# davnords/octic-vits

Measured on AMD Instinct MI355X. Metric: images/sec Hybrid Octic ViT-H/14 224² bf16 train step @1/2/4/8 MI355X, higher is better.
Workload: dtype bf16; 1 GPU; hybrid_deit_huge_patch14 (16 octic + 16 standard blocks, drop_path 0.5) DeiT-III train step: bf16-autocast fwd + bwd + LAMB + EMA, 224x224, batch 64/GPU (BASELINE configs[1]), data parallel over 1 GPU(s); global_batch=64, per_gpu_batch=64, accum_steps=1, parallelism=dp1, library_gemm_table=True, launch=hipGraph replay (whole step)

## Files before the change

include/octic_hip.h:

```cpp
#ifndef OCTIC_HIP_H
#define OCTIC_HIP_H

#include <stdint.h>

#ifdef __cplusplus
extern "C" {
#endif

#define OCTIC_ABI_VERSION 20

enum { OCTIC_F32 = 0, OCTIC_BF16 = 1, OCTIC_U8 = 2  };

enum {
  OCTIC_OK = 0,
  OCTIC_ESHAPE = -1,
  OCTIC_EALIGN = -2,
  OCTIC_EDTYPE = -3,
  OCTIC_ENULL = -4,
  OCTIC_EWORKSPACE = -5
};

typedef struct {
  void* ptr[5];
  int64_t ld[5];
// ... 129 lines not shown
int octic_attn_unpack_heads(void* const heads[3], const octic_view* y, int64_t B, int64_t T, int H, int c, int n_s,
                            int dtype, void* stream);

int octic_attn_fwd(const void* q, const void* k, const void* v, void* o, float* lse, int64_t B, int H, int T, int hd,
                   int64_t sB, int64_t sH, int64_t sT, int64_t oB, int64_t oH, int64_t oT, float scale, void* stream);

int octic_attn_bwd(const void* q, const void* k, const void* v, const void* o, const void* dout, const float* lse,
                   float* delta, void* dq, void* dk, void* dv, int64_t B, int H, int T, int hd, int64_t sB, int64_t sH,
                   int64_t sT, int64_t oB, int64_t oH, int64_t oT, int64_t gB, int64_t gH, int64_t gT, float scale,
                   int phase, void* stream);

int octic_attn_fwd_f32(const void* q, const void* k, const void* v, void* o, float* lse, int64_t B, int H, int T, int hd,
                       int64_t sB, int64_t sH, int64_t sT, int64_t oB, int64_t oH, int64_t oT, float scale, void* stream);
int octic_attn_bwd_f32(const void* q, const void* k, const void* v, const void* o, const void* dout, const float* lse,
                       float* delta, void* dq, void* dk, void* dv, int64_t B, int H, int T, int hd, int64_t sB, int64_t sH,
                       int64_t sT, int64_t oB, int64_t oH, int64_t oT, int64_t gB, int64_t gH, int64_t gT, float scale,
                       int phase, void* stream);

int octic_attn_fwd_packed(const void* qkv, void* o, float* lse, int64_t B, int H, int T, int c, int64_t ld_qkv,
                          int64_t ld_o, float scale, void* stream);
int octic_attn_bwd_packed(const void* qkv, const void* o, const void* dout, const float* lse, float* delta, void* dqkv,
                          int64_t B, int H, int T, int c, int64_t ld_qkv, int64_t ld_o, int64_t ld_g, float scale,
                          int phase, void* stream);

enum {
  OCTIC_ATTN_FWD_PERSIST = 0,
  OCTIC_ATTN_FWD_A80_ONESHOT = 1,
  OCTIC_ATTN_FWD_A80_ONLINE = 2,
  OCTIC_ATTN_FWD_RESIDENT = 3,
  OCTIC_ATTN_FWD_STREAM = 4,
  OCTIC_ATTN_FWD_F32 = 5
};
enum {
  OCTIC_ATTN_BWD_SINGLE = 0,
  OCTIC_ATTN_BWD_PAIR = 1,
  OCTIC_ATTN_BWD_STREAM = 2,
  OCTIC_ATTN_BWD_F32 = 3
};
int octic_attn_plan(int dtype, int T, int hd, int64_t ld_in, int64_t ld_out, int64_t ld_grad, int out[4]);
int octic_attn_skip_plan(int dtype, int T, int hd, int64_t ld_in, int64_t ld_out, int64_t ld_grad, int out[4]);

int octic_attn_fwd_skip(const void* q, const void* k, const void* v, void* o, float* lse, int64_t B, int H, int T, int hd,
                        int64_t sB, int64_t sH, int64_t sT, int64_t oB, int64_t oH, int64_t oT, float scale,
                        const float* sample_scale, void* stream);
int octic_attn_bwd_skip(const void* q, const void* k, const void* v, const void* o, const void* dout, const float* lse,
                        float* delta, void* dq, void* dk, void* dv, int64_t B, int H, int T, int hd, int64_t sB, int64_t sH,
                        int64_t sT, int64_t oB, int64_t oH, int64_t oT, int64_t gB, int64_t gH, int64_t gT, float scale,
                        int phase, const float* sample_scale, void* stream);
int octic_attn_fwd_packed_skip(const void* qkv, void* o, float* lse, int64_t B, int H, int T, int c, int64_t ld_qkv,
                               int64_t ld_o, float scale, const float* sample_scale, void* stream);
int octic_attn_bwd_packed_skip(const void* qkv, const void* o, const void* dout, const float* lse, float* delta, void* dqkv,
                               int64_t B, int H, int T, int c, int64_t ld_qkv, int64_t ld_o, int64_t ld_g, float scale,
                               int phase, const float* sample_scale, void* stream);

int octic_handoff_cat_fwd(const octic_view* x, void* dense, int64_t M, int c, int out_dtype, void* stream);
int octic_handoff_cat_bwd(const float* ddense, const octic_view* dx, int64_t M, int c, void* stream);
int octic_power_spectrum_fwd(const octic_view* x, void* dense, int64_t M, int c, int out_dtype, void* stream);
int octic_power_spectrum_bwd(const float* ddense, const octic_view* x, const octic_view* dx, int64_t M, int c,
                             void* stream);

int octic_im2col_patches(const float* img, void* patches, int64_t B, int Cin, int Himg, int Wimg, int p,
                         int Kpad, int dtype, void* stream);
int octic_lift_gemm(const void* patches, const void* w, const float* bias, const float* pos, float* out,
                    int64_t B, int64_t n_patches, int tok0, int Kpad, int D, int dtype, void* stream);
int64_t octic_lift_wgrad_workspace_bytes(int Kpad, int D, int splits);
int octic_lift_wgrad(const void* patches, const void* dout, float* dw, float* workspace, int splits, int64_t rows,
                     int Kpad, int D, int dtype, void* stream);

int64_t octic_lamb_workspace_floats(int ntensors, int nchunks);
int octic_lamb_step(void* const* p, void* const* g, void* const* m, void* const* v, void* const* ema, const float* wd,
                    const int* chunk_tensor, const int64_t* chunk_off, const int* chunk_len,
                    const int* tensor_chunk_begin, int ntensors, int nchunks, float* workspace, float lr, float beta1,
                    float beta2, float eps, float max_grad_norm, int step, float ema_decay, void* const* bf16_shadow,
                    void* stream);
int octic_adamw_step(void* const* p, void* const* g, void* const* m, void* const* v, void* const* ema, const float* wd,
                     const int* chunk_tensor, const int64_t* chunk_off, const int* chunk_len,
                     const int* tensor_chunk_begin, int ntensors, int nchunks, float* workspace, float lr, float beta1,
                     float beta2, float eps, float max_grad_norm, int step, float ema_decay, void* const* bf16_shadow,
                     void* stream);
int octic_lamb_step_hp(void* const* p, void* const* g, void* const* m, void* const* v, void* const* ema, const float* wd,
                       const int* chunk_tensor, const int64_t* chunk_off, const int* chunk_len,
                       const int* tensor_chunk_begin, int ntensors, int nchunks, float* workspace, const float* lr,
                       float beta1, float beta2, float eps, float max_grad_norm, int step, const float* ema_decay,
                       void* const* bf16_shadow, void* stream);
int octic_adamw_step_hp(void* const* p, void* const* g, void* const* m, void* const* v, void* const* ema, const float* wd,
                        const int* chunk_tensor, const int64_t* chunk_off, const int* chunk_len,
                        const int* tensor_chunk_begin, int ntensors, int nchunks, float* workspace, const float* lr,
                        float beta1, float beta2, float eps, float max_grad_norm, int step, const float* ema_decay,
                        void* const* bf16_shadow, void* stream);

int octic_dense_blocks(int64_t rows);
int octic_dense_resid_layernorm_fwd(const float* x, const void* yb, int yb_dtype, const float* gamma, const float* rs,
                                    int64_t rows_per_scale, float* xout, void* y, int y_dtype, const float* w,
                                    const float* b, float* stats, int64_t rows, int d, float eps, void* stream);
int octic_dense_layernorm_fwd(const float* x, void* y, int y_dtype, const float* w, const float* b, float* stats,
                              int64_t rows, int d, float eps, void* stream);
int octic_dense_layernorm_bwd(const void* gy, int g_dtype, const float* x, const float* w, const float* stats,
                              const float* dres, float* dx, float* partials, int64_t rows, int d, void* stream);
int octic_dense_finish(const float* partials, int nblocks, int d, float* out0, float* out1, const float* scale1,
                       void* stream);
typedef struct octic_finish_job {
  const float* partials;
  float* out0;
  float* out1;
  const float* scale1;
  int nblocks;
  int d;
} octic_finish_job;
int octic_dense_finish_batch(const octic_finish_job* jobs, int njobs, void* stream);
int octic_dense_layernorm_bwd_tail(const void* gy, const float* x, const float* w, const float* stats, const float* dres,
                                   float* dx, float* partials, const void* yb, const float* gamma, const float* rs,
                                   int64_t rows_per_scale, void* gyb, float* partials2, int64_t rows, int d, void* stream);
int octic_dense_gelu_blocks(void);
int octic_dense_gelu_bwd(const void* h, const void* g, void* dh, float* partials, int64_t rows, int d, void* stream);
int octic_dense_colsum(const void* g, int64_t rows, int d, int64_t ld, float* partials, void* stream);
int octic_scale_residual_fwd(const float* x, const void* y, int y_dtype, const float* gamma, const float* rs,
                             int64_t rows_per_scale, float* out, int64_t rows, int d, void* stream);
int octic_scale_residual_bwd(const float* gout, const void* y, int y_dtype, const float* gamma, const float* rs,
                             int64_t rows_per_scale, void* gy, float* partials, int64_t rows, int d, void* stream);

int octic_dense_layernorm_fwd_rows(const float* x, void* y, int y_dtype, const float* w, const float* b, float* stats,
                                   int64_t rows, int d, float eps, const int* rowmap, float* xcopy, void* stream);
int octic_dense_layernorm_bwd_rows(const void* gy, int g_dtype, const float* x, const float* w, const float* stats,
                                   const float* dres, float* dx, float* partials, int64_t rows, int d, const int* rowmap,
                                   void* stream);
int octic_scale_residual_fwd_rows(const float* x, const void* y, int y_dtype, const float* gamma, const float* rs,
                                  int64_t rows_per_scale, float* out, int64_t rows, int d, const int* rowmap, void* stream);
int octic_scale_residual_bwd_rows(const float* gout, const void* y, int y_dtype, const float* gamma, const float* rs,
                                  int64_t rows_per_scale, void* gy, float* partials, int64_t rows, int d, const int* rowmap,
                                  void* stream);

typedef struct octic_dense_prep_item {
  const void* src;
  void* wb;
  void* wt;
  int32_t N, K;
  int32_t block_begin, pad;
} octic_dense_prep_item;
int octic_dense_prep_batch_blocks(int N, int K);
int octic_dense_prep_batch(const octic_dense_prep_item* items_dev, int n_items, int total_blocks, int src_dtype, void* stream);

int64_t octic_dense_gemm_workspace_bytes(int M, int N, int K);
int octic_dense_gemm_colsum_rows(int M, int N, int K);
int octic_dense_gemm_tile(int M, int N, int K, int mode);
int octic_dense_gemm_nt(const void* A, const void* B, int M, int N, int K, int64_t lda, int64_t ldb, int mode, void* C,
                        void* C2, int64_t ldc, const float* bias, const float* gamma, const float* rs,
                        int64_t rows_per_sample, const float* X, float* OUT, const void* H, float* colsum,
                        void* workspace, void* stream);
int octic_dense_gemm_nt_tokens(const void* A, const void* B, int M, int N, int K, int64_t lda, int64_t ldb, int mode, void* C,
                               void* C2, int64_t ldc, const float* bias, const float* gamma, const float* rs,
                               int64_t rows_per_sample, const float* X, float* OUT, const void* H, float* colsum,
                               void* workspace, int tokens, void* stream);
int octic_dense_gemm_plan(int M, int N, int K, int mode, int tokens, int* out4);

int64_t octic_dense_wgrad_workspace_bytes(int M, int N, int K);
int octic_dense_wgrad_tile(int M, int N, int K);
int octic_dense_wgrad_plan(int M, int N0, int N1, int K, int64_t ld_max, int out[4]);
int octic_dense_wgrad_tn(const void* dY, const void* X, int M, int N, int K, int64_t ldy, int64_t ldx, float* dW,
                         void* workspace, void* stream);
int64_t octic_dense_wgrad_pair_workspace_bytes(int M, int N0, int N1, int K);
int octic_dense_wgrad_tn_pair(const void* dY0, const void* X0, int N0, int64_t ldy0, int64_t ldx0, float* dW0,
                              const void* dY1, const void* X1, int N1, int64_t ldy1, int64_t ldx1, float* dW1, int M, int K,
                              void* workspace, void* stream);
int octic_dense_wgrad_tn_skip(const void* dY, const void* X, int M, int N, int K, int64_t ldy, int64_t ldx, float* dW,
                              const float* sample_scale, int rows_per_sample, void* workspace, void* stream);
int octic_dense_wgrad_tn_pair_skip(const void* dY0, const void* X0, int N0, int64_t ldy0, int64_t ldx0, float* dW0,
                                   const void* dY1, const void* X1, int N1, int64_t ldy1, int64_t ldx1, float* dW1, int M, int K,
                                   const float* sample_scale, int rows_per_sample, void* workspace, void* stream);

int octic_softmax_center(const void* t, int t_dtype, int64_t ldt, const float* center, float inv_temp, float* out,
                         int64_t rows, int K, void* stream);
int octic_soft_ce_fwd(const void* s, int s_dtype, int64_t lds, const float* tprob, int64_t t_rows, float inv_temp,
                      float* loss, float* lse, float* tsum, int64_t rows, int K, void* stream);
int octic_soft_ce_bwd(const void* s, int s_dtype, int64_t lds, const float* tprob, int64_t t_rows, float inv_temp,
                      const float* g, const float* lse, const float* tsum, void* ds, int64_t ldd, int64_t rows, int K,
                      void* stream);

typedef struct {
  float* w;
  float* b;
  float* mw;
  float* mb;
  int32_t col0;
  int32_t K;
  int32_t lr_index;
  int32_t tile0;
} octic_probe_head;
int octic_probe_features(const void* const* cls, const int64_t* cls_ld, int n, const void* patch, int64_t patch_ld_b,
                         int64_t patch_ld_t, int dtype, int64_t B, int P, int D, float* F, int64_t ldf, void* stream);
int octic_probe_forward(const octic_probe_head* heads, int nheads, const float* F, int64_t ldf, int B, int C, float* logits,
                        void* stream);
int octic_probe_ce(const float* logits, const int64_t* labels, int nheads, int B, int C, float* dlogits, float* rowloss,
                   int* rowrank, float* loss_mean, float* loss_sum, int* topk, void* stream);
int octic_probe_sgd(const octic_probe_head* heads, int nheads, int total_ktiles, const float* F, int64_t ldf,
                    const float* dlogits, int B, int C, const float* lr, float momentum, void* stream);

int octic_seg_ldd(int C);
int octic_seg_slabs(int64_t N, int D, int C);
int64_t octic_seg_workspace_bytes(int64_t N, int D, int C);
int octic_seg_value_dlogits(const float* X, int64_t ldx, int64_t N, int D, const float* W, const float* b, int C,
                            const int32_t* y, float* dlogits, double* value, void* workspace, void* stream);
int octic_seg_predict(const float* X, int64_t ldx, int64_t N, int D, const float* W, const float* b, int C, int32_t* pred,
                      void* stream);
int octic_seg_wgrad(const float* X, int64_t ldx, int64_t N, int D, const float* dlogits, int C, const float* W, double scale,
                    double lambda, float* dW, float* db, void* workspace, void* stream);
int64_t octic_seg_colstats_workspace_bytes(int64_t N, int D);
int octic_seg_colstats(const float* X, int64_t ldx, int64_t N, int D, double* mean, double* var, void* workspace, void* stream);
int octic_seg_standardize(float* X, int64_t ldx, int64_t N, int D, const double* mean, const double* scale, void* stream);
int octic_seg_patch_mode(const void* labels, int esize, int64_t R, int L, int32_t* mode, void* stream);
int octic_seg_confusion(const void* labels, int esize, int64_t R, int L, const int32_t* pred, const uint8_t* ignore,
                        int64_t* counts, void* stream);

typedef struct {
  int32_t partner;
  float lam;
  int32_t cut;
  int32_t yl, yh;
  int32_t xl, xh;
  int32_t pad;
} octic_mix_row;
int octic_mix_images(const float* src, float* dst, const octic_mix_row* table, int B, int C, int H, int W, void* stream);
int octic_mix_targets(const int64_t* labels, const octic_mix_row* table, int B, int row0, int rows, int num_classes, float on,
                      float off, int binarize, float* targets, void* stream);
int octic_mix_bce(const void* logits, int dtype, int64_t ldl, const int64_t* labels, const octic_mix_row* table, int B, int row0,
                  int rows, int num_classes, float on, float off, int binarize, float* loss, const float* gscale,
                  void* dlogits, int64_t ldd, void* workspace, void* stream);

typedef struct {
  int32_t flip;
  int32_t op;
  int32_t blur_r, blur_ww, blur_fw;
  int32_t order[4];
  float brightness, contrast, saturation;
  int32_t pad[4];
} octic_aug_row;
int64_t octic_augment_workspace_bytes(int B, int H, int W);
int octic_augment_u8(const uint8_t* src, void* dst, int dtype_out, const octic_aug_row* table, float mean0, float mean1,
                     float mean2, float std0, float std1, float std2, int B, int H, int W, void* workspace, void* stream);

#ifdef __cplusplus
}
#endif
#endif
```

octic_vits_amd/_lib.py:

```python
import ctypes
import os
import re

HERE = os.path.dirname(os.path.abspath(__file__))
LIB_PATH = os.environ.get("OCTIC_LIB") or os.path.join(HERE, "liboctic_hip.so")
HEADER_PATH = os.path.join(HERE, "..", "include", "octic_hip.h")

F32, BF16, U8 = 0, 1, 2
ABI_VERSION = 20
(ROUTE_DENSE_TILE, ROUTE_DENSE_SPLIT, ROUTE_WGRAD_SLABS, ROUTE_WGRAD_TILE, ROUTE_LINEAR_RING, ROUTE_RING_EVEN,
 ROUTE_ATTN_LEGACY, ROUTE_ATTN_ONLINE, ROUTE_ATTN_BWD_PAIR, ROUTE_DENSE_IMAGE, ROUTE_DENSE_CLS2, ROUTE_ATTN_STREAM) = range(12)

(ATTN_FWD_PERSIST, ATTN_FWD_A80_ONESHOT, ATTN_FWD_A80_ONLINE, ATTN_FWD_RESIDENT, ATTN_FWD_STREAM, ATTN_FWD_F32) = range(6)
ATTN_BWD_SINGLE, ATTN_BWD_PAIR, ATTN_BWD_STREAM, ATTN_BWD_F32 = range(4)
LINEAR_WREG, LINEAR_RING, LINEAR_CLASSIC = range(3)
WGRAD_RING, WGRAD_TILED = range(2)

c_i64, c_int, c_float, c_void_p = ctypes.c_int64, ctypes.c_int, ctypes.c_float, ctypes.c_void_p
c_double = ctypes.c_double


class OcticView(ctypes.Structure):
    _fields_ = [("ptr", c_void_p * 5), ("ld", c_i64 * 5)]


PtrArray5 = c_void_p * 5
VP = ctypes.POINTER(OcticView)

_PROTOS = {
    "octic_abi_version": (c_int, []),
    "octic_strerror": (ctypes.c_char_p, [c_int]),
    "octic_route_override": (c_int, [c_int, c_int]),
    "octic_gelu_d8_fwd": (c_int, [VP, VP, c_i64, c_int, c_int, c_void_p]),
    "octic_gelu_d8_bwd": (c_int, [VP, VP, VP, c_i64, c_int, c_int, c_void_p]),
    "octic_gelu_d8_fwd_skip": (c_int, [VP, VP, c_i64, c_int, c_int, c_void_p, c_i64, c_void_p]),
    "octic_gelu_d8_bwd_skip": (c_int, [VP, VP, VP, c_i64, c_int, c_int, c_void_p, c_i64, c_void_p]),
    "octic_layernorm_d8_fwd": (c_int, [VP, VP, c_void_p, c_void_p, c_void_p, c_i64, c_int, c_float, c_int, c_void_p]),
    "octic_layernorm_d8_bwd_blocks": (c_int, [c_i64]),
    "octic_layernorm_d8_bwd": (c_int, [VP, VP, c_void_p, c_void_p, VP, VP, c_void_p, c_i64, c_int, c_int, c_void_p]),
    "octic_layernorm_d8_bwd_cast": (c_int, [VP, VP, c_void_p, c_void_p, VP, VP, c_void_p, c_i64, c_int, c_void_p, c_i64,
                                            c_void_p, c_void_p]),
    "octic_layernorm_d8_bwd_finish": (c_int, [c_void_p, c_int, c_int, c_void_p, c_void_p, c_void_p]),
    "octic_layernorm_d8_bwd_finish_batch": (c_int, [c_void_p, c_int, c_void_p]),
    "octic_sample_blocks": (c_int, [c_void_p, c_void_p, c_void_p, c_i64, c_i64, c_int, c_void_p]),
    "octic_linear_d8_fwd": (c_int, [VP, c_void_p, c_void_p, VP, VP, c_void_p, c_i64, c_void_p, c_i64, c_int, c_int,
                                    c_int, c_int, c_void_p]),
    "octic_linear_d8_fwd_skip": (c_int, [VP, c_void_p, c_void_p, VP, VP, c_void_p, c_i64, c_void_p, c_i64, c_int, c_int,
                                         c_int, c_int, c_void_p, c_i64, c_void_p]),
    "octic_linear_d8_fwd_dropped": (c_int, [VP, c_void_p, c_void_p, VP, VP, c_void_p, c_i64, c_void_p, c_i64, c_int, c_int,
                                            c_int, c_int, c_void_p, c_i64, c_void_p]),
    "octic_linear_d8_tile_n": (c_int, [c_i64, c_int, c_int]),
    "octic_linear_d8_plan": (c_int, [c_i64, c_int, c_int, c_int, c_int, c_int, ctypes.POINTER(c_int)]),
    "octic_linear_d8_ring_order": (c_int, [c_void_p, c_void_p, c_void_p, c_int, c_void_p, c_void_p]),
    "octic_linear_d8_ring_order_dropped": (c_int, [c_int, c_void_p, c_void_p, c_int, c_void_p, c_void_p, c_void_p, c_void_p,
                                                   c_void_p, c_void_p]),
    "octic_linear_d8_wgrad_tile": (c_int, [c_i64, c_int, c_int]),
    "octic_linear_d8_wgrad_workspace_bytes": (c_i64, [c_int, c_int, c_int]),
    "octic_linear_d8_wgrad_splits": (c_int, [c_i64, c_int, c_int]),
    "octic_linear_d8_wgrad": (c_int, [VP, VP, c_i64, c_int, c_int, c_int, c_void_p, c_int, c_void_p]),
    "octic_linear_d8_wgrad_finish": (c_int, [c_void_p, c_int, c_int, c_int, c_void_p, c_void_p, c_void_p, c_void_p,
                                             c_void_p, c_void_p, c_void_p, c_void_p]),
    "octic_linear_d8_wgrad_finish_batch": (c_int, [c_void_p, c_int, c_void_p]),
    "octic_linear_d8_wgrad_has_colsum": (c_int, [c_int, c_int, c_int]),
    "octic_linear_d8_wgrad_plan": (c_int, [c_i64, c_int, c_int, c_int, ctypes.POINTER(c_int)]),
    "octic_lamb_workspace_floats": (c_i64, [c_int, c_int]),
    "octic_lamb_step": (c_int, [c_void_p] * 10 + [c_int, c_int, c_void_p, c_float, c_float, c_float, c_float, c_float,
                                                  c_int, c_float, c_void_p, c_void_p]),
    "octic_adamw_step": (c_int, [c_void_p] * 10 + [c_int, c_int, c_void_p, c_float, c_float, c_float, c_float, c_float,
                                                   c_int, c_float, c_void_p, c_void_p]),
    "octic_lamb_step_hp": (c_int, [c_void_p] * 10 + [c_int, c_int, c_void_p, c_void_p, c_float, c_float, c_float, c_float,
                                                     c_int, c_void_p, c_void_p, c_void_p]),
    "octic_adamw_step_hp": (c_int, [c_void_p] * 10 + [c_int, c_int, c_void_p, c_void_p, c_float, c_float, c_float, c_float,
                                                      c_int, c_void_p, c_void_p, c_void_p]),
    "octic_dense_blocks": (c_int, [c_i64]),
    "octic_dense_layernorm_fwd": (c_int, [c_void_p, c_void_p, c_int, c_void_p, c_void_p, c_void_p, c_i64, c_int,
                                          c_float, c_void_p]),
    "octic_dense_resid_layernorm_fwd": (c_int, [c_void_p, c_void_p, c_int, c_void_p, c_void_p, c_i64, c_void_p, c_void_p, c_int,
                                                c_void_p, c_void_p, c_void_p, c_i64, c_int, c_float, c_void_p]),
    "octic_dense_layernorm_bwd": (c_int, [c_void_p, c_int, c_void_p, c_void_p, c_void_p, c_void_p, c_void_p, c_void_p,
                                          c_i64, c_int, c_void_p]),
    "octic_dense_layernorm_bwd_tail": (c_int, [c_void_p] * 10 + [c_i64, c_void_p, c_void_p, c_i64, c_int, c_void_p]),
    "octic_dense_finish": (c_int, [c_void_p, c_int, c_int, c_void_p, c_void_p, c_void_p, c_void_p]),
    "octic_dense_finish_batch": (c_int, [c_void_p, c_int, c_void_p]),
    "octic_dense_gelu_blocks": (c_int, []),
    "octic_dense_gelu_bwd": (c_int, [c_void_p, c_void_p, c_void_p, c_void_p, c_i64, c_int, c_void_p]),
    "octic_dense_layernorm_fwd_rows": (c_int, [c_void_p, c_void_p, c_int, c_void_p, c_void_p, c_void_p, c_i64, c_int, c_float,
                                               c_void_p, c_void_p, c_void_p]),
    "octic_dense_layernorm_bwd_rows": (c_int, [c_void_p, c_int, c_void_p, c_void_p, c_void_p, c_void_p, c_void_p, c_void_p, c_i64,
                                               c_int, c_void_p, c_void_p]),
    "octic_scale_residual_fwd_rows": (c_int, [c_void_p, c_void_p, c_int, c_void_p, c_void_p, c_i64, c_void_p, c_i64, c_int,
                                              c_void_p, c_void_p]),
    "octic_scale_residual_bwd_rows": (c_int, [c_void_p, c_void_p, c_int, c_void_p, c_void_p, c_i64, c_void_p, c_void_p, c_i64,
                                              c_int, c_void_p, c_void_p]),
    "octic_softmax_center": (c_int, [c_void_p, c_int, c_i64, c_void_p, c_float, c_void_p, c_i64, c_int, c_void_p]),
    "octic_soft_ce_fwd": (c_int, [c_void_p, c_int, c_i64, c_void_p, c_i64, c_float, c_void_p, c_void_p, c_void_p, c_i64, c_int,
                                  c_void_p]),
    "octic_soft_ce_bwd": (c_int, [c_void_p, c_int, c_i64, c_void_p, c_i64, c_float, c_void_p, c_void_p, c_void_p, c_void_p, c_i64,
                                  c_i64, c_int, c_void_p]),
    "octic_scale_residual_fwd": (c_int, [c_void_p, c_void_p, c_int, c_void_p, c_void_p, c_i64, c_void_p, c_i64, c_int,
                                         c_void_p]),
    "octic_scale_residual_bwd": (c_int, [c_void_p, c_void_p, c_int, c_void_p, c_void_p, c_i64, c_void_p, c_void_p,
                                         c_i64, c_int, c_void_p]),
    "octic_colsum_blocks": (c_int, [c_i64]),
    "octic_colsum_a1": (c_int, [VP, c_i64, c_int, c_int, c_void_p, c_void_p, c_void_p]),
    "octic_cast_rowscale": (c_int, [VP, VP, c_void_p, c_i64, c_i64, c_int, c_int, c_void_p]),
    "octic_linear_d8_prep": (c_int, [c_void_p, c_void_p, c_int, c_int, c_void_p, c_void_p, c_int, c_void_p]),
    "octic_linear_d8_prep_batch_blocks": (c_int, [c_int, c_int]),
    "octic_linear_d8_prep_batch": (c_int, [c_void_p, c_int, c_int, c_int, c_void_p]),
    "octic_attn_fwd": (c_int, [c_void_p, c_void_p, c_void_p, c_void_p, c_void_p, c_i64, c_int, c_int, c_int,
                               c_i64, c_i64, c_i64, c_i64, c_i64, c_i64, c_float, c_void_p]),
    "octic_attn_fwd_packed": (c_int, [c_void_p] * 3 + [c_i64, c_int, c_int, c_int, c_i64, c_i64, c_float, c_void_p]),
    "octic_attn_bwd_packed": (c_int, [c_void_p] * 6 + [c_i64, c_int, c_int, c_int, c_i64, c_i64, c_i64, c_float, c_int, c_void_p]),
    "octic_attn_bwd": (c_int, [c_void_p] * 10 + [c_i64, c_int, c_int, c_int] + [c_i64] * 9 + [c_float, c_int, c_void_p]),
    "octic_attn_fwd_skip": (c_int, [c_void_p] * 5 + [c_i64, c_int, c_int, c_int] + [c_i64] * 6 + [c_float, c_void_p, c_void_p]),
    "octic_attn_bwd_skip": (c_int, [c_void_p] * 10 + [c_i64, c_int, c_int, c_int] + [c_i64] * 9 + [c_float, c_int, c_void_p, c_void_p]),
    "octic_attn_fwd_packed_skip": (c_int, [c_void_p] * 3 + [c_i64, c_int, c_int, c_int, c_i64, c_i64, c_float, c_void_p, c_void_p]),
    "octic_attn_bwd_packed_skip": (c_int, [c_void_p] * 6 + [c_i64, c_int, c_int, c_int, c_i64, c_i64, c_i64, c_float, c_int, c_void_p, c_void_p]),
    "octic_attn_fwd_f32": (c_int, [c_void_p] * 5 + [c_i64, c_int, c_int, c_int] + [c_i64] * 6 + [c_float, c_void_p]),
    "octic_attn_bwd_f32": (c_int, [c_void_p] * 10 + [c_i64, c_int, c_int, c_int] + [c_i64] * 9 + [c_float, c_int, c_void_p]),
    "octic_attn_plan": (c_int, [c_int, c_int, c_int, c_i64, c_i64, c_i64, ctypes.POINTER(c_int)]),
    "octic_attn_skip_plan": (c_int, [c_int, c_int, c_int, c_i64, c_i64, c_i64, ctypes.POINTER(c_int)]),
    "octic_attn_pack_heads": (c_int, [VP, c_void_p, c_i64, c_i64, c_int, c_int, c_int, c_int, c_void_p]),
    "octic_attn_unpack_heads": (c_int, [c_void_p, VP, c_i64, c_i64, c_int, c_int, c_int, c_int, c_void_p]),
    "octic_handoff_cat_fwd": (c_int, [VP, c_void_p, c_i64, c_int, c_int, c_void_p]),
    "octic_handoff_cat_bwd": (c_int, [c_void_p, VP, c_i64, c_int, c_void_p]),
    "octic_power_spectrum_fwd": (c_int, [VP, c_void_p, c_i64, c_int, c_int, c_void_p]),
    "octic_power_spectrum_bwd": (c_int, [c_void_p, VP, VP, c_i64, c_int, c_void_p]),
    "octic_im2col_patches": (c_int, [c_void_p, c_void_p, c_i64, c_int, c_int, c_int, c_int, c_int, c_int, c_void_p]),
    "octic_lift_gemm": (c_int, [c_void_p, c_void_p, c_void_p, c_void_p, c_void_p, c_i64, c_i64, c_int, c_int, c_int,
                                c_int, c_void_p]),
    "octic_lift_wgrad_workspace_bytes": (c_i64, [c_int, c_int, c_int]),
    "octic_lift_wgrad": (c_int, [c_void_p, c_void_p, c_void_p, c_void_p, c_int, c_i64, c_int, c_int, c_int, c_void_p]),
    "octic_dense_prep_batch_blocks": (c_int, [c_int, c_int]),
    "octic_dense_prep_batch": (c_int, [c_void_p, c_int, c_int, c_int, c_void_p]),
    "octic_dense_gemm_workspace_bytes": (c_i64, [c_int, c_int, c_int]),
    "octic_dense_gemm_colsum_rows": (c_int, [c_int, c_int, c_int]),
    "octic_dense_gemm_tile": (c_int, [c_int, c_int, c_int, c_int]),
    "octic_dense_gemm_nt": (c_int, [c_void_p, c_void_p, c_int, c_int, c_int, c_i64, c_i64, c_int, c_void_p, c_void_p, c_i64,
                                    c_void_p, c_void_p, c_void_p, c_i64, c_void_p, c_void_p, c_void_p, c_void_p, c_void_p,
                                    c_void_p]),
    "octic_dense_gemm_nt_tokens": (c_int, [c_void_p, c_void_p, c_int, c_int, c_int, c_i64, c_i64, c_int, c_void_p, c_void_p,
                                           c_i64, c_void_p, c_void_p, c_void_p, c_i64, c_void_p, c_void_p, c_void_p, c_void_p,
                                           c_void_p, c_int, c_void_p]),
    "octic_dense_gemm_plan": (c_int, [c_int, c_int, c_int, c_int, c_int, ctypes.POINTER(c_int)]),
    "octic_dense_colsum": (c_int, [c_void_p, c_i64, c_int, c_i64, c_void_p, c_void_p]),
    "octic_dense_wgrad_workspace_bytes": (c_i64, [c_int, c_int, c_int]),
    "octic_dense_wgrad_tile": (c_int, [c_int, c_int, c_int]),
    "octic_dense_wgrad_plan": (c_int, [c_int, c_int, c_int, c_int, c_i64, ctypes.POINTER(c_int)]),
    "octic_dense_wgrad_tn": (c_int, [c_void_p, c_void_p, c_int, c_int, c_int, c_i64, c_i64, c_void_p, c_void_p, c_void_p]),
    "octic_dense_wgrad_pair_workspace_bytes": (c_i64, [c_int, c_int, c_int, c_int]),
    "octic_dense_wgrad_tn_pair": (c_int, [c_void_p, c_void_p, c_int, c_i64, c_i64, c_void_p, c_void_p, c_void_p, c_int, c_i64, c_i64,
                                          c_void_p, c_int, c_int, c_void_p, c_void_p]),
    "octic_dense_wgrad_tn_skip": (c_int, [c_void_p, c_void_p, c_int, c_int, c_int, c_i64, c_i64, c_void_p, c_void_p, c_int, c_void_p,
                                          c_void_p]),
    "octic_dense_wgrad_tn_pair_skip": (c_int, [c_void_p, c_void_p, c_int, c_i64, c_i64, c_void_p, c_void_p, c_void_p, c_int, c_i64,
                                               c_i64, c_void_p, c_int, c_int, c_void_p, c_int, c_void_p, c_void_p]),
    "octic_probe_features": (c_int, [c_void_p, c_void_p, c_int, c_void_p, c_i64, c_i64, c_int, c_i64, c_int, c_int, c_void_p,
                                     c_i64, c_void_p]),
    "octic_probe_forward": (c_int, [c_void_p, c_int, c_void_p, c_i64, c_int, c_int, c_void_p, c_void_p]),
    "octic_probe_ce": (c_int, [c_void_p, c_void_p, c_int, c_int, c_int, c_void_p, c_void_p, c_void_p, c_void_p, c_void_p,
                               c_void_p, c_void_p]),
    "octic_probe_sgd": (c_int, [c_void_p, c_int, c_int, c_void_p, c_i64, c_void_p, c_int, c_int, c_void_p, c_float, c_void_p]),
    "octic_seg_ldd": (c_int, [c_int]),
    "octic_seg_slabs": (c_int, [c_i64, c_int, c_int]),
    "octic_seg_workspace_bytes": (c_i64, [c_i64, c_int, c_int]),
    "octic_seg_value_dlogits": (c_int, [c_void_p, c_i64, c_i64, c_int, c_void_p, c_void_p, c_int, c_void_p, c_void_p, c_void_p,
                                        c_void_p, c_void_p]),
    "octic_seg_predict": (c_int, [c_void_p, c_i64, c_i64, c_int, c_void_p, c_void_p, c_int, c_void_p, c_void_p]),
    "octic_seg_wgrad": (c_int, [c_void_p, c_i64, c_i64, c_int, c_void_p, c_int, c_void_p, c_double, c_double, c_void_p, c_void_p,
                                c_void_p, c_void_p]),
    "octic_seg_colstats_workspace_bytes": (c_i64, [c_i64, c_int]),
    "octic_seg_colstats": (c_int, [c_void_p, c_i64, c_i64, c_int, c_void_p, c_void_p, c_void_p, c_void_p]),
    "octic_seg_standardize": (c_int, [c_void_p, c_i64, c_i64, c_int, c_void_p, c_void_p, c_void_p]),
    "octic_seg_patch_mode": (c_int, [c_void_p, c_int, c_i64, c_int, c_void_p, c_void_p]),
    "octic_seg_confusion": (c_int, [c_void_p, c_int, c_i64, c_int, c_void_p, c_void_p, c_void_p, c_void_p]),
    "octic_mix_images": (c_int, [c_void_p, c_void_p, c_void_p, c_int, c_int, c_int, c_int, c_void_p]),
    "octic_mix_targets": (c_int, [c_void_p, c_void_p, c_int, c_int, c_int, c_int, c_float, c_float, c_int, c_void_p, c_void_p]),
    "octic_mix_bce": (c_int, [c_void_p, c_int, c_i64, c_void_p, c_void_p, c_int, c_int, c_int, c_int, c_float, c_float, c_int,
                              c_void_p, c_void_p, c_void_p, c_i64, c_void_p, c_void_p]),
    "octic_augment_workspace_bytes": (c_i64, [c_int, c_int, c_int]),
    "octic_augment_u8": (c_int, [c_void_p, c_void_p, c_int, c_void_p] + [c_float] * 6 + [c_int, c_int, c_int, c_void_p, c_void_p]),
}


def header_symbols():
    with open(HEADER_PATH) as f:
        text = re.sub(r"/\*.*?\*/", "", f.read(), flags=re.S)
    return sorted(set(re.findall(r"\b(octic_[a-z0-9_]+)\s*\(", text)))


_LIB = None


def lib():
    global _LIB
    if _LIB is None:
        if not os.path.exists(LIB_PATH):
            raise RuntimeError(
                f"octic_vits_amd: HIP library {LIB_PATH} is missing. Build it with "
                "`python -m octic_vits_amd.build` (hipcc, --offload-arch=gfx950). There is no CPU fallback.")
        L = ctypes.CDLL(LIB_PATH)
        for name, (res, args) in _PROTOS.items():
            fn = getattr(L, name)
            fn.restype, fn.argtypes = res, args
        if L.octic_abi_version() != ABI_VERSION:
            raise RuntimeError("octic_vits_amd: ABI version mismatch between _lib.py and liboctic_hip.so")
        _LIB = L
    return _LIB


def route_override(knob: int, value: int) -> int:
    old = lib().octic_route_override(knob, value)
    if old < 0:
        raise ValueError(f"octic_route_override: unknown knob {knob}")
    _PLANS.clear()
    for drop in _ON_OVERRIDE:
        drop()
    return old


_ON_OVERRIDE = []


def on_route_override(drop):
    if drop not in _ON_OVERRIDE:
        _ON_OVERRIDE.append(drop)
    return drop


_PLANS = {}


def plan(query, *args):
    key = (query, args)
    answer = _PLANS.get(key, 0)
    if answer == 0:
        out = (c_int * 4)()
        code = getattr(lib(), query)(*args, out)
        if code not in (0, -1):
            check(code)
        _PLANS[key] = answer = tuple(out) if code == 0 else None
    return answer


def attn_plan(T, hd, dtype=BF16, ld_in=0, ld_out=0, ld_grad=0):
    answer = plan("octic_attn_plan", dtype, T, hd, ld_in, ld_out, ld_grad)
    if answer is None:
        check(-1)
    return answer


def check(code: int):
    if code != 0:
        raise RuntimeError(f"octic HIP call failed ({code}): {lib().octic_strerror(code).decode()}")
```

octic_vits_amd/csrc/dense_gemm.hip:

```cpp
#include <cmath>
#include <type_traits>
#include "octic_common.hpp"

namespace octic {

constexpr int DG_BM = 256, DG_BK = 64;
constexpr int DG_UNIT = 128 * 128;
constexpr int DG_SLOTS = 8;
constexpr int DG_D = 6;
static_assert(DG_D >= 4 && DG_D <= DG_SLOTS - 2, "prefetch distance");
template <int NT> struct DgGeom {
  static constexpr int NA = NT - 2;
  static constexpr int BN = 64 * NT;
  static constexpr int WCOLS = 16 * NT;
  static constexpr int U1 = NA * 8192;
  static constexpr int KT = 3 * DG_UNIT + U1;
  static constexpr int RING = 2 * KT;
  static constexpr int SRS = WCOLS * 2 + 16;
  static constexpr int EPI_PASSES = NT == 4 ? 1 : 2;
  static constexpr int EPI_ROWS = 128 / EPI_PASSES;
  static constexpr int EPI = 8 * EPI_ROWS * SRS;
  static constexpr int LDS = RING > EPI ? RING : EPI;
  static constexpr int INFLIGHT = 2 * (DG_D - 2) + (NA - 2);
  static_assert(DG_D == 6 || NT == 4, "unequal units: the steady vmcnt assumes the 4 youngest units are one of each kind");
  __host__ __device__ static constexpr int unit_off(int kind) { return kind == 0 ? 0 : kind == 1 ? DG_UNIT : kind == 2 ? DG_UNIT + U1 : 2 * DG_UNIT + U1; }
  __host__ __device__ static constexpr int unit_instr(int kind) { return kind == 1 ? NA : 2; }
};

struct DgArgs {
  const bf16* A;
  const bf16* B;
  int64_t lda, ldb;
  int M, N, K;
  bf16* C;
  bf16* C2;
  int64_t ldc;
  const float* bias;
  const float* gamma;
  const float* rs;
  int64_t rps;
  const float* X;
  float* OUT;
  const bf16* H;
  float* colsum;
  int m_stride, m_base;
  int tiles_m, tiles_n;
  int full_tiles;
  int split;
  int tail_pad;
  float* slabs;
  int* tickets;
};

enum DgMode { DG_PLAIN = 0, DG_GELU = 1, DG_RESID = 2, DG_DGELU = 3,
              DG_GELUF = 4,
              DG_DFACT = 5,
              DG_GELUO = 6 };

__device__ inline void dg_wait_vmcnt(int n) {
  switch (n) {
    case 2: asm volatile("s_waitcnt vmcnt(2)" ::: "memory"); break;
    case 4: asm volatile("s_waitcnt vmcnt(4)" ::: "memory"); break;
    case 6: asm volatile("s_waitcnt vmcnt(6)" ::: "memory"); break;
    case 8: asm volatile("s_waitcnt vmcnt(8)" ::: "memory"); break;
    case 10: asm volatile("s_waitcnt vmcnt(10)" ::: "memory"); break;
    case 12: asm volatile("s_waitcnt vmcnt(12)" ::: "memory"); break;
    case 14: asm volatile("s_waitcnt vmcnt(14)" ::: "memory"); break;
    case 16: asm volatile("s_waitcnt vmcnt(16)" ::: "memory"); break;
    case 3: asm volatile("s_waitcnt vmcnt(3)" ::: "memory"); break;
    case 5: asm volatile("s_waitcnt vmcnt(5)" ::: "memory"); break;
    case 7: asm volatile("s_waitcnt vmcnt(7)" ::: "memory"); break;
    case 9: asm volatile("s_waitcnt vmcnt(9)" ::: "memory"); break;
    default: asm volatile("s_waitcnt vmcnt(0)" ::: "memory"); break;
  }
}

#ifdef DG_TRACE
__device__ unsigned long long g_dg_trace[8 * 256];
extern "C" void* octic_dbg_dense_trace(void) {
  void* p = nullptr;
  (void)hipGetSymbolAddress(&p, HIP_SYMBOL(g_dg_trace));
  return p;
}
#define DGT()                                                                                        \
  do {                                                                                               \
    if (blockIdx.x == 0 && lane == 0 && dgt_i < 256) g_dg_trace[wid * 256 + dgt_i++] = __builtin_readcyclecounter(); \
    if (blockIdx.x == 0 && lane == 0 && dgt_i == 200) g_dg_trace[wid * 256 + 255] = __builtin_amdgcn_s_memrealtime(); \
  } while (0)
#else
#define DGT() do {} while (0)
#endif
#ifdef DG_TRACE2
__device__ unsigned long long g_dg_trace2[4096 * 8];
extern "C" void* octic_dbg_dense_trace2(void) {
  void* p = nullptr;
  (void)hipGetSymbolAddress(&p, HIP_SYMBOL(g_dg_trace2));
  return p;
}
#define DGT2(slot)                                                                                            \
  do {                                                                                                        \
    if (wid == 0 && lane == 0 && blockIdx.x < 4096) g_dg_trace2[blockIdx.x * 8 + (slot)] = __builtin_amdgcn_s_memrealtime(); \
  } while (0)
#else
#define DGT2(slot) do {} while (0)
#endif

__device__ inline float dg_erf(float x) {
  const float ax = fabsf(x);
  const float t = __builtin_amdgcn_rcpf(1.0f + 0.3275911f * ax);
  const float poly = t * (0.254829592f + t * (-0.284496736f + t * (1.421413741f + t * (-1.453152027f + t * 1.061405429f))));
  const float r = 1.0f - poly * __expf(-ax * ax);
  return copysignf(r, x);
}
__device__ inline float dg_gelu(float x) { return 0.5f * x * (1.0f + dg_erf(x * kSqrt1Over2)); }
__device__ inline float dg_gelu_grad(float x) {
  return 0.5f * (1.0f + dg_erf(x * kSqrt1Over2)) + x * kInvSqrt2Pi * __expf(-0.5f * x * x);
}
__device__ inline void dg_gelu_both(float x, float& g, float& d) {
  const float ax = fabsf(x) * kSqrt1Over2;
  const float t = __builtin_amdgcn_rcpf(1.0f + 0.3275911f * ax);
  const float poly = t * (0.254829592f + t * (-0.284496736f + t * (1.421413741f + t * (-1.453152027f + t * 1.061405429f))));
  const float e = __expf(-ax * ax);
  const float phi = 0.5f * (1.0f + copysignf(1.0f - poly * e, x));
  g = x * phi;
  d = phi + x * kInvSqrt2Pi * e;
}

template <int N>
__device__ inline void dg_wait_imm() {
  if constexpr (N == 8) asm volatile("s_waitcnt vmcnt(8)" ::: "memory");
  else if constexpr (N == 10) asm volatile("s_waitcnt vmcnt(10)" ::: "memory");
  else if constexpr (N == 12) asm volatile("s_waitcnt vmcnt(12)" ::: "memory");
  else if constexpr (N == 14) asm volatile("s_waitcnt vmcnt(14)" ::: "memory");
  else if constexpr (N == 16) asm volatile("s_waitcnt vmcnt(16)" ::: "memory");
  else if constexpr (N == 6) asm volatile("s_waitcnt vmcnt(6)" ::: "memory");
  else if constexpr (N == 9) asm volatile("s_waitcnt vmcnt(9)" ::: "memory");
  else asm volatile("s_waitcnt vmcnt(0)" ::: "memory");
}

template <int MODE, int NT>
__global__ __launch_bounds__(512, 1) void dense_nt_kernel(DgArgs a) {
  extern __shared__ __attribute__((aligned(16))) char lds[];
  using GE = DgGeom<NT>;
  constexpr int NA = GE::NA, DG_BN = GE::BN;
  static_assert(NT == 4 || MODE == DG_PLAIN, "the fused tails exist for the 256-wide tile only");

  const int lane = threadIdx.x & 63;
  const int wid = __builtin_amdgcn_readfirstlane(threadIdx.x >> 6);
  const int wr = wid >> 2, wc = wid & 3;
  const bool hi = wr != 0;
  const int fr = lane & 15, kg = lane >> 4;
#ifdef DG_TRACE
  int dgt_i = 0;
  if (blockIdx.x == 0 && lane == 0) g_dg_trace[wid * 256 + 254] = __builtin_amdgcn_s_memrealtime();
#endif
  DGT();
  DGT2(0);
#ifdef DG_TRACE2
  if (wid == 0 && lane == 0 && blockIdx.x < 4096) {
    unsigned xcc, hwid;
    asm volatile("s_getreg_b32 %0, hwreg(HW_REG_XCC_ID)" : "=s"(xcc));
    asm volatile("s_getreg_b32 %0, hwreg(HW_REG_HW_ID)" : "=s"(hwid));
    g_dg_trace2[blockIdx.x * 8 + 7] = ((unsigned long long)hwid << 32) | xcc;
  }
#endif

  const int bid = blockIdx.x;
  int tile, kt_begin, kt_end, part = 0, rem_idx = -1;
  const int nkt_all = a.K / DG_BK;
  if (bid >= a.tail_pad) {
    const int j = bid - a.tail_pad;
    const int nf = a.full_tiles;
    const int xcd = j & 7, q8 = nf >> 3, r8 = nf & 7;
    tile = (xcd < r8 ? xcd * (q8 + 1) : r8 * (q8 + 1) + (xcd - r8) * q8) + (j >> 3);
    kt_begin = 0;
    kt_end = nkt_all;
  } else {
    const int r = bid;
    if (r >= (a.tiles_m * a.tiles_n - a.full_tiles) * a.split) return;
    rem_idx = r / a.split;
    part = r - rem_idx * a.split;
    tile = a.full_tiles + rem_idx;
    kt_begin = (int)(((int64_t)nkt_all * part) / a.split);
    kt_end = (int)(((int64_t)nkt_all * (part + 1)) / a.split);
  }
  int tm, tn;
  {
    const int G = 8;
    const int per_group = G * a.tiles_n;
    const int gidx = tile / per_group;
    const int first_m = gidx * G;
    const int gsz = (a.tiles_m - first_m) < G ? (a.tiles_m - first_m) : G;
    const int in_g = tile - gidx * per_group;
    tm = first_m + in_g % gsz;
    tn = in_g / gsz;
  }
  const int m0 = tm * a.m_stride + a.m_base, n0 = tn * DG_BN;
  const int nkt = kt_end - kt_begin;
  const int nunits = 4 * nkt;

  const int drow = lane >> 3;
  const int dch = (lane & 7) ^ drow;
  const __amdgpu_buffer_rsrc_t rsA = __builtin_amdgcn_make_buffer_rsrc((void*)a.A, 0, (int)((int64_t)a.M * a.lda * 2), 0x27000);
  const __amdgpu_buffer_rsrc_t rsB = __builtin_amdgcn_make_buffer_rsrc((void*)a.B, 0, (int)((int64_t)a.N * a.ldb * 2), 0x27000);
  const int r0 = 16 * wid + drow;
  const int am0 = m0, an0 = n0;
  const unsigned voA = (unsigned)(((int64_t)(am0 + (r0 >> 6) * 128 + (r0 & 63)) * a.lda + dch * 8) * 2);
  const int rb1 = 8 * NA * wid + drow;
  const unsigned voB1 = (unsigned)(((int64_t)(an0 + (rb1 / (16 * NA)) * GE::WCOLS + (rb1 % (16 * NA))) * a.ldb + dch * 8) * 2);
  const unsigned voB2 = (unsigned)(((int64_t)(an0 + (r0 >> 5) * GE::WCOLS + 16 * NA + (r0 & 31)) * a.ldb + dch * 8) * 2);
  const int rowA8 = (int)(a.lda * 16), rowB8 = (int)(a.ldb * 16);
  const int halfA = (int)(a.lda * 128);
  const int kbase = kt_begin * (DG_BK * 2);

  int u_issue = 0;
  auto issue_unit = [&](auto kind_c) {
    constexpr int KIND = decltype(kind_c)::value;
    constexpr bool isA = KIND == 0 || KIND == 3;
    char* dst = lds + ((u_issue >> 2) & 1) * GE::KT + GE::unit_off(KIND) + wid * (GE::unit_instr(KIND) * 1024);
    const int so = kbase + (u_issue >> 2) * (DG_BK * 2) + (KIND == 3 ? halfA : 0);
    if constexpr (isA) {
      __builtin_amdgcn_raw_ptr_buffer_load_lds(rsA, (__attribute__((address_space(3))) void*)dst, 16, voA, so, 0, 0);
      __builtin_amdgcn_raw_ptr_buffer_load_lds(rsA, (__attribute__((address_space(3))) void*)(dst + 1024), 16, voA, so + rowA8, 0, 0);
    } else if constexpr (KIND == 1) {
      __builtin_amdgcn_raw_ptr_buffer_load_lds(rsB, (__attribute__((address_space(3))) void*)dst, 16, voB1, so, 0, 0);
      __builtin_amdgcn_raw_ptr_buffer_load_lds(rsB, (__attribute__((address_space(3))) void*)(dst + 1024), 16, voB1, so + rowB8, 0, 0);
      if constexpr (NA == 3)
        __builtin_amdgcn_raw_ptr_buffer_load_lds(rsB, (__attribute__((address_space(3))) void*)(dst + 2048), 16, voB1, so + 2 * rowB8, 0, 0);
    } else {
      __builtin_amdgcn_raw_ptr_buffer_load_lds(rsB, (__attribute__((address_space(3))) void*)dst, 16, voB2, so, 0, 0);
      __builtin_amdgcn_raw_ptr_buffer_load_lds(rsB, (__attribute__((address_space(3))) void*)(dst + 1024), 16, voB2, so + rowB8, 0, 0);
    }
    ++u_issue;
  };
  auto young_instr = [&](int n) {
    const int k1 = ((u_issue + 2) >> 2) - ((u_issue - n + 2) >> 2);
    return 2 * n + (NA - 2) * k1;
  };
#define DG_IC(v) std::integral_constant<int, v>()

  const int sw = lane & 7;
  const int rdo0 = fr * 128 + ((kg ^ sw) << 4);
  const int rdo1 = fr * 128 + (((4 + kg) ^ sw) << 4);
  const int a_row0 = wr * 64;

  bf16x8 Af[1][2][4];
  bf16x8 Bf0[2][NA], Bf1[2][2];
  f32x4 acc0[2][4][NA], acc1[2][4][2];
#pragma unroll
  for (int i = 0; i < 2; ++i)
#pragma unroll
    for (int p = 0; p < 4; ++p) {
#pragma unroll
      for (int q = 0; q < NA; ++q) acc0[i][p][q] = f32x4{0, 0, 0, 0};
#pragma unroll
      for (int q = 0; q < 2; ++q) acc1[i][p][q] = f32x4{0, 0, 0, 0};
    }
  int rt_hi = (a.M - m0 - wr * 128 + 15) >> 4;
  rt_hi = rt_hi < 0 ? 0 : (rt_hi > 8 ? 8 : rt_hi);
  const int live_mask = __builtin_amdgcn_readfirstlane((rt_hi > 0 ? 1 : 0) | (rt_hi > 4 ? 2 : 0));

  auto readA = [&](int mh, int unit) {
    const char* base = lds + ((unit >> 2) & 1) * GE::KT + GE::unit_off(mh ? 3 : 0) + a_row0 * 128;
#pragma unroll
    for (int mi = 0; mi < 4; ++mi) {
      Af[0][0][mi] = *(const bf16x8*)(base + mi * 2048 + rdo0);
      Af[0][1][mi] = *(const bf16x8*)(base + mi * 2048 + rdo1);
    }
  };
  auto readB = [&](int nh, int unit) {
    if (nh == 0) {
      const char* base = lds + ((unit >> 2) & 1) * GE::KT + GE::unit_off(1) + wc * (16 * NA) * 128;
#pragma unroll
      for (int ni = 0; ni < NA; ++ni) {
        Bf0[0][ni] = *(const bf16x8*)(base + ni * 2048 + rdo0);
        Bf0[1][ni] = *(const bf16x8*)(base + ni * 2048 + rdo1);
      }
    } else {
      const char* base = lds + ((unit >> 2) & 1) * GE::KT + GE::unit_off(2) + wc * 32 * 128;
#pragma unroll
      for (int ni = 0; ni < 2; ++ni) {
        Bf1[0][ni] = *(const bf16x8*)(base + ni * 2048 + rdo0);
        Bf1[1][ni] = *(const bf16x8*)(base + ni * 2048 + rdo1);
      }
    }
  };
  auto mma = [&](int mh, int nh, auto kind_c) {
    asm volatile("s_waitcnt lgkmcnt(0)" ::: "memory");
    __builtin_amdgcn_sched_barrier(0);
    if (live_mask & (mh ? 2 : 1)) {
#pragma unroll
    for (int ks = 0; ks < 2; ++ks) {
#pragma unroll
      for (int mi = 0; mi < 4; ++mi) {
        if (nh == 0) {
#pragma unroll
          for (int ni = 0; ni < NA; ++ni)
            acc0[mh][mi][ni] = __builtin_amdgcn_mfma_f32_16x16x32_bf16(Bf0[ks][ni], Af[0][ks][mi], acc0[mh][mi][ni], 0, 0, 0);
        } else {
#pragma unroll
          for (int ni = 0; ni < 2; ++ni)
            acc1[mh][mi][ni] = __builtin_amdgcn_mfma_f32_16x16x32_bf16(Bf1[ks][ni], Af[0][ks][mi], acc1[mh][mi][ni], 0, 0, 0);
        }
      }
    }
    }
    __builtin_amdgcn_sched_barrier(0);
  };

  int g = 0;
  auto wait_landed = [&]() {
    int need = g + 2;
    need = need < nunits - 1 ? need : nunits - 1;
    const int ok = (u_issue - 1) - need;
    if (ok == DG_D - 2) dg_wait_imm<GE::INFLIGHT>();
    else dg_wait_vmcnt(ok > 0 ? young_instr(ok) : 0);
  };

#define DG_PRO(i) if constexpr ((i) < DG_D) { if (u_issue < nunits) issue_unit(DG_IC((i) & 3)); }
  DG_PRO(0) DG_PRO(1) DG_PRO(2) DG_PRO(3) DG_PRO(4) DG_PRO(5) DG_PRO(6) DG_PRO(7) DG_PRO(8) DG_PRO(9)
#undef DG_PRO
  {
    const int ok = (u_issue - 1) - 1;
    dg_wait_vmcnt(ok > 0 ? young_instr(ok) : 0);
  }
  if (hi) __builtin_amdgcn_s_barrier();
  DGT2(1);

  auto ktile = [&](int t, auto steady_c) {
    constexpr bool STEADY = decltype(steady_c)::value != 0;
    const int u0 = 4 * t;
    auto dma = [&](auto kind_c) {
      if (STEADY || u_issue < nunits) issue_unit(kind_c);
    };
    auto landed = [&]() {
      if constexpr (STEADY) dg_wait_imm<GE::INFLIGHT>();
      else wait_landed();
    };
#define DG_RP(x) do { __builtin_amdgcn_s_setprio(x); } while (0)
#define DG_R(q, reads) do { DG_RP(2); dma(DG_IC(((q) + DG_D) & 3)); reads; DG_RP(0); } while (0)
    __builtin_amdgcn_s_barrier();
    DGT();
    DG_R(0, readA(0, u0); readB(0, u0 + 1));
    if (hi) landed();
    DGT();
    __builtin_amdgcn_s_barrier();
    DGT();
    mma(0, 0, DG_IC((0 + DG_D) & 3));
    DGT();
    if (!hi) landed();
// ... 397 lines not shown
inline DgPlan dense_plan_nt(int M, int N, int K, int cus, int nt, int force_split = 0, bool front_unsplit = false) {
  DgPlan p;
  const int bn = 64 * nt;
  const double wf = nt / 4.0;
  p.nt = nt;
  p.tiles_m = (M + DG_BM - 1) / DG_BM;
  p.tiles_n = (N + bn - 1) / bn;
  const int tiles = p.tiles_m * p.tiles_n;
  const int rounds = tiles / cus;
  const int nkt = K / DG_BK;
  p.full = rounds * cus;
  p.rem = tiles - p.full;
  p.split = 1;
  double f = 1.0;
  if (p.rem > 0) {
    int s = cus / p.rem;
    const int smax = nkt / 4 > 0 ? nkt / 4 : 1;
    s = s < 1 ? 1 : (s > smax ? smax : s);
    s = s > 8 ? 8 : s;
    if (p.rem * 10 >= cus * 8) s = 1;
    {
      int64_t rows = 0;
      for (int tile = p.full; tile < tiles; ++tile) {
        const int G = 8, per_group = G * p.tiles_n, gidx = tile / per_group, first_m = gidx * G;
        const int gsz = (p.tiles_m - first_m) < G ? (p.tiles_m - first_m) : G;
        const int tm = first_m + (tile - gidx * per_group) % gsz;
        const int left = M - tm * DG_BM;
        rows += left < DG_BM ? left : DG_BM;
      }
      f = (double)rows / ((double)p.rem * DG_BM);
    }
    if (s > 1 && (double)nkt / s + 17.0 * f * wf + 1.0 >= (double)nkt) s = 1;
    if (force_split > 0) s = force_split > smax ? smax : force_split;
    p.split = s;
    if (s == 1 && !(front_unsplit && f < 0.5 && rounds >= 1)) {
      p.full = tiles;
      p.rem = 0;
    }
  }
  p.tail_pad = (p.rem * p.split + 7) & ~7;
  p.grid = p.tail_pad + p.full;
  const double tile_cost = nkt * wf + 3.0;
  p.cost = (double)((p.full + cus - 1) / cus) * tile_cost;
  if (p.rem > 0) {
    const double kt = (f < 0.5 ? 0.5 : 1.0) * wf;
    p.cost += (double)nkt / p.split * kt + 17.0 * f * wf + 3.0;
  }
  return p;
}

constexpr int DG_TICKET_BYTES = 8192;

static inline int dense_force_nt() { const int v = route(OCTIC_ROUTE_DENSE_TILE); return (v == 4 || v == 5) ? v : 0; }
static inline int dense_force_split() { const int v = route(OCTIC_ROUTE_DENSE_SPLIT); return v > 0 ? v : 0; }

inline DgPlan dense_plan(int M, int N, int K, int cus, int mode) {
  const DgPlan p4 = dense_plan_nt(M, N, K, cus, 4, dense_force_split(), dense_force_split() == 1);
  if (mode != DG_PLAIN || (N % 320) != 0 || dense_force_nt() == 4) return p4;
  const DgPlan p5 = dense_plan_nt(M, N, K, cus, 5, dense_force_split(), dense_force_split() == 1);
  if (dense_force_nt() == 5) return p5;
  return p5.cost < p4.cost ? p5 : p4;
}

inline int dense_cls_waves(int K) {
  if (K % 320 == 0 && K / 320 <= 16) return K / 320;
  for (int w = 16; w > 1; --w)
    if (K % (32 * w) == 0) return w;
  return 1;
}

struct DgTokPlan { DgPlan p; bool image; int images; };
#ifndef DG_CLS2_US
#define DG_CLS2_US 15.0
#endif
inline bool dense_cls_two_launches(int mode, int N, int K) {
  const int v = route(OCTIC_ROUTE_DENSE_CLS2);
  const bool legal = mode == DG_PLAIN && (K % CLS_KSLICE) == 0 && (N % 64) == 0;
  return legal && v != 1 && (v == 2 || K >= 3840);
}
inline double dense_cls_cost(int B, int N, int K, int mode) {
  double us = 7.0 * sqrt((double)N / 1280.0) * pow((double)K / 1280.0, 0.8);
  if (dense_cls_two_launches(mode, N, K)) us = DG_CLS2_US;
  return us * (B <= 64 ? 1.0 : (double)B / 64.0) / 1.54;
}
inline DgTokPlan dense_plan_tokens(int M, int N, int K, int cus, int mode, int tokens) {
  DgTokPlan t;
  t.p = dense_plan(M, N, K, cus, mode);
  t.image = false;
  t.images = 0;
  const int force = route(OCTIC_ROUTE_DENSE_IMAGE);
  if (tokens != 257 || M % tokens != 0 || mode == DG_RESID || (K % 128) != 0 || (N % 16) != 0 || force == 2) return t;
  const int B = M / tokens;
  const DgPlan pi = dense_plan(B * DG_BM, N, K, cus, mode);
  const double margin = 1.0;
  const bool pays = mode != DG_DGELU && mode != DG_DFACT && pi.cost + dense_cls_cost(B, N, K, mode) + margin < t.p.cost;
  if (force == 1 || (force == 0 && pays) || (force == 3 && pays && mode == DG_PLAIN)) {
    t.p = pi;
    t.image = true;
    t.images = B;
  }
  return t;
}

}

using namespace octic;

extern "C" {

static int dense_cus() { return device_cus(); }

int64_t octic_dense_gemm_workspace_bytes(int M, int N, int K) {
  int64_t need = 256;
  if ((M % 257) == 0 && (K % CLS_KSLICE) == 0) {
    const int64_t rows_pad = ((int64_t)(M / 257) + 63) / 64 * 64;
    need = DG_TICKET_BYTES + (int64_t)(K / CLS_KSLICE) * rows_pad * N * 4 + 256;
  }
  const int Ms[2] = {M, (M % 257) == 0 ? M / 257 * DG_BM : 0};
  for (int i = 0; i < 2; ++i) {
    if (Ms[i] <= 0) continue;
    for (int nt = 4; nt <= 5; ++nt) {
      if (nt == 5 && (N % 320) != 0) continue;
      DgPlan p = dense_plan_nt(Ms[i], N, K, dense_cus(), nt);
      if (dense_force_split() > 1) p = dense_plan_nt(Ms[i], N, K, dense_cus(), nt, 8);
      if (p.split <= 1) continue;
      const int64_t b = (int64_t)p.rem * p.split * DG_BM * (64 * nt) * 4 + DG_TICKET_BYTES + 256;
      need = b > need ? b : need;
    }
  }
  return need;
}

int octic_dense_gemm_plan(int M, int N, int K, int mode, int tokens, int* out) {
  if (!out) return OCTIC_ENULL;
  if (M <= 0 || N <= 0 || K < 2 * DG_BK) { out[0] = 256; out[1] = 0; out[2] = 0; out[3] = 0; return OCTIC_OK; }
  const DgTokPlan t = dense_plan_tokens(M, N, K, dense_cus(), mode, tokens);
  out[0] = t.p.nt == 5 ? 320 : 256;
  out[1] = t.image ? 2 * t.images + (t.images + 15) / 16 : 2 * ((M + DG_BM - 1) / DG_BM);
  out[2] = t.image ? 1 : 0;
  out[3] = t.p.grid;
  return OCTIC_OK;
}

int octic_dense_gemm_tile(int M, int N, int K, int mode) {
  if (M <= 0 || N <= 0 || K < 2 * DG_BK) return 256;
  return dense_plan(M, N, K, dense_cus(), mode).nt == 5 ? 320 : 256;
}

int octic_dense_gemm_colsum_rows(int M, int N, int K) {
  (void)N; (void)K;
  return 2 * ((M + DG_BM - 1) / DG_BM);
}

int octic_dense_gemm_nt_tokens(const void* A, const void* B, int M, int N, int K, int64_t lda, int64_t ldb, int mode, void* C,
                               void* C2, int64_t ldc, const float* bias, const float* gamma, const float* rs, int64_t rps,
                               const float* X, float* OUT, const void* H, float* colsum, void* workspace, int tokens,
                               void* stream) {
  if (!A || !B || !C) return OCTIC_ENULL;
  if (M <= 0 || N <= 0 || K <= 0 || (K % DG_BK) || K < 2 * DG_BK || (N % 8) || (lda % 8) || (ldb % 8) || (ldc % 8)) return OCTIC_ESHAPE;
  if ((int64_t)M * lda * 2 >= (1ll << 31) || (int64_t)N * ldb * 2 >= (1ll << 31)) return OCTIC_ESHAPE;
  if ((((uintptr_t)A) | ((uintptr_t)B)) & 15) return OCTIC_EALIGN;
  if ((mode == DG_GELU || mode == DG_GELUF) && !C2) return OCTIC_ENULL;
  if (mode == DG_RESID && (!X || !OUT || (rs && rps <= 0))) return OCTIC_ENULL;
  if ((mode == DG_DGELU || mode == DG_DFACT) && !H) return OCTIC_ENULL;
  DgArgs a = {};
  a.A = (const bf16*)A; a.B = (const bf16*)B; a.lda = lda; a.ldb = ldb; a.M = M; a.N = N; a.K = K;
  a.C = (bf16*)C; a.C2 = (bf16*)C2; a.ldc = ldc; a.bias = bias; a.gamma = gamma; a.rs = rs; a.rps = rs ? rps : 1;
  a.X = X; a.OUT = OUT; a.H = (const bf16*)H; a.colsum = (mode == DG_DGELU || mode == DG_DFACT) ? colsum : nullptr;
  const DgTokPlan tp = dense_plan_tokens(M, N, K, dense_cus(), mode, tokens);
  const DgPlan p = tp.p;
  a.tiles_m = p.tiles_m; a.tiles_n = p.tiles_n; a.full_tiles = p.full; a.split = p.split; a.tail_pad = p.tail_pad;
  a.m_stride = tp.image ? tokens : DG_BM;
  a.m_base = tp.image ? 1 : 0;
  hipStream_t s = (hipStream_t)stream;
  if (p.split > 1) {
    if (!workspace) return OCTIC_ENULL;
    if (p.rem * 4 > DG_TICKET_BYTES) return OCTIC_ESHAPE;
    a.tickets = (int*)workspace;
    a.slabs = (float*)((char*)workspace + DG_TICKET_BYTES);
  }
  const int smem = DgGeom<4>::LDS, smem5 = DgGeom<5>::LDS;
  static DeviceOnce once;
  if (once.first()) {
    (void)hipFuncSetAttribute((const void*)dense_nt_kernel<DG_PLAIN, 4>, hipFuncAttributeMaxDynamicSharedMemorySize, smem);
    (void)hipFuncSetAttribute((const void*)dense_nt_kernel<DG_PLAIN, 5>, hipFuncAttributeMaxDynamicSharedMemorySize, smem5);
    (void)hipFuncSetAttribute((const void*)dense_nt_kernel<DG_GELU, 4>, hipFuncAttributeMaxDynamicSharedMemorySize, smem);
    (void)hipFuncSetAttribute((const void*)dense_nt_kernel<DG_RESID, 4>, hipFuncAttributeMaxDynamicSharedMemorySize, smem);
    (void)hipFuncSetAttribute((const void*)dense_nt_kernel<DG_DGELU, 4>, hipFuncAttributeMaxDynamicSharedMemorySize, smem);
    (void)hipFuncSetAttribute((const void*)dense_nt_kernel<DG_GELUF, 4>, hipFuncAttributeMaxDynamicSharedMemorySize, smem);
    (void)hipFuncSetAttribute((const void*)dense_nt_kernel<DG_DFACT, 4>, hipFuncAttributeMaxDynamicSharedMemorySize, smem);
    (void)hipFuncSetAttribute((const void*)dense_nt_kernel<DG_GELUO, 4>, hipFuncAttributeMaxDynamicSharedMemorySize, smem);
    (void)hipGetLastError();
  }
  switch (mode) {
    case DG_PLAIN:
      if (p.nt == 5) dense_nt_kernel<DG_PLAIN, 5><<<p.grid, 512, smem5, s>>>(a);
      else dense_nt_kernel<DG_PLAIN, 4><<<p.grid, 512, smem, s>>>(a);
      break;
    case DG_GELU: dense_nt_kernel<DG_GELU, 4><<<p.grid, 512, smem, s>>>(a); break;
    case DG_RESID: dense_nt_kernel<DG_RESID, 4><<<p.grid, 512, smem, s>>>(a); break;
    case DG_DGELU: dense_nt_kernel<DG_DGELU, 4><<<p.grid, 512, smem, s>>>(a); break;
    case DG_GELUF: dense_nt_kernel<DG_GELUF, 4><<<p.grid, 512, smem, s>>>(a); break;
    case DG_DFACT: dense_nt_kernel<DG_DFACT, 4><<<p.grid, 512, smem, s>>>(a); break;
    case DG_GELUO: dense_nt_kernel<DG_GELUO, 4><<<p.grid, 512, smem, s>>>(a); break;
    default: return OCTIC_ESHAPE;
  }
  if (tp.image && dense_cls_two_launches(mode, N, K) && workspace && p.split <= 1) {
    const int rows_pad = (tp.images + 63) / 64 * 64;
    float* part = (float*)((char*)workspace + DG_TICKET_BYTES);
    const int cus = dense_cus(), per64 = (N / 64) * (K / CLS_KSLICE) * (rows_pad / 64);
    const int nw = (per64 > cus && (N % 80) == 0 && (N / 80) * (K / CLS_KSLICE) * (rows_pad / 64) <= cus) ? 5 : 4;
    dense_cls_part_kernel<<<(N / (16 * nw)) * (K / CLS_KSLICE) * (rows_pad / 64), 64 * nw, 0, s>>>(a, tokens, tp.images, rows_pad, part);
    dense_cls_sum_kernel<<<(tp.images * (N / 4) + 255) / 256, 256, 0, s>>>(a, tokens, tp.images, rows_pad, part);
  } else if (tp.image) {
    const int grid = (N / 16) * ((tp.images + 15) / 16), cr0 = 2 * tp.images, thr = 64 * dense_cls_waves(K);
    switch (mode) {
      case DG_PLAIN: dense_cls_kernel<DG_PLAIN><<<grid, thr, 0, s>>>(a, tokens, tp.images, cr0); break;
      case DG_GELU: dense_cls_kernel<DG_GELU><<<grid, thr, 0, s>>>(a, tokens, tp.images, cr0); break;
      case DG_DGELU: dense_cls_kernel<DG_DGELU><<<grid, thr, 0, s>>>(a, tokens, tp.images, cr0); break;
      case DG_GELUF: dense_cls_kernel<DG_GELUF><<<grid, thr, 0, s>>>(a, tokens, tp.images, cr0); break;
      case DG_DFACT: dense_cls_kernel<DG_DFACT><<<grid, thr, 0, s>>>(a, tokens, tp.images, cr0); break;
      case DG_GELUO: dense_cls_kernel<DG_GELUO><<<grid, thr, 0, s>>>(a, tokens, tp.images, cr0); break;
      default: return OCTIC_ESHAPE;
    }
  }
  return launch_status();
}

int octic_dense_gemm_nt(const void* A, const void* B, int M, int N, int K, int64_t lda, int64_t ldb, int mode, void* C,
                        void* C2, int64_t ldc, const float* bias, const float* gamma, const float* rs, int64_t rps,
                        const float* X, float* OUT, const void* H, float* colsum, void* workspace, void* stream) {
  return octic_dense_gemm_nt_tokens(A, B, M, N, K, lda, ldb, mode, C, C2, ldc, bias, gamma, rs, rps, X, OUT, H, colsum,
                                    workspace, 0, stream);
}

}
```

octic_vits_amd/functional.py:

```python
import os

import torch

from . import ops


class Octic(tuple):

    def __new__(cls, packed: torch.Tensor, c: int):
        self = super().__new__(cls, ops.split_packed(packed, c))
        self.packed, self.c = packed, c
        return self


def as_packed(xs):
    if isinstance(xs, Octic):
        return xs.packed, xs.c
    if len(xs) != 5:
        raise AssertionError("Input should be a 5-tuple")
    c = xs[0].shape[-1]
    if xs[4].shape[-2:] != (2, 2 * c):
        raise ValueError(f"E irrep must be [..., 2, {2 * c}], got {tuple(xs[4].shape)}")
    return torch.cat([xs[0], xs[1], xs[2], xs[3], xs[4].flatten(-2)], dim=-1), c

# ... 244 lines not shown
        w32 = [_c(w.detach().float()) for w in w5] if has_cs else None
        f32_masters = all(w.dtype == torch.float32 for w in w5)
        dw, dcs, dbias = ops.linear_wgrad(xv, gv, M, cin, cout, dtype, x, w32=w32, cs5=cs32, bias=b32, dysum=dysum,
                                          want_bias=has_bias, may_defer=f32_masters, wparams=w5 if f32_masters else None)
        if not f32_masters:
            dw = [d.to(w.dtype) for d, w in zip(dw, w5)]
        dcs = dcs if has_cs else [None] * 5
        return (dx, *dw, dbias, dy if fused else None, None, *dcs, None, None, None, None, None, None, None, None)


class LinearD8NormFn(torch.autograd.Function):

    @staticmethod
    def forward(ctx, x, wA1, wA2, wB1, wB2, wE, bias, resid, rs, sA1, sA2, sB1, sB2, sE, cin, cout, rps, dtype, prep,
                a1, a2, b1, b2, ae, beta, eps, skip_dx=None):
        w5 = (wA1, wA2, wB1, wB2, wE)
        cs5 = None if sA1 is None else (sA1, sA2, sB1, sB2, sE)
        ops._require_cuda(x)
        x_in_dtype = x.dtype
        if x.dtype != dtype:
            x = ops.cast_rowscale(_c(x.float()), None, 1, dtype, cin)
        x = _c(x)
        wb, wt = prep.get(w5, cs5, dtype, cin, cout)
        M = x.numel() // (8 * cin)
        y = torch.empty(x.shape[:-1] + (8 * cout,), dtype=resid.dtype, device=x.device)
        b32 = None if bias is None else _c(bias.detach().float())
        cs32 = None if cs5 is None else [_c(s.detach().float()) for s in cs5]
        rs32 = None if rs is None else _c(rs.float())
        ops.linear_fwd(ops.pview(x, cin), wb, b32, ops.pview(y, cout), M, cin, cout, dtype, resid.dtype, x,
                       resid_v=ops.pview(_c(resid), cout), rs=rs32, rps=rps, cs5=cs32, dropped=ring_skip_scale(rs32, rps, M),
                       dropped_rps=rps)
        alpha = None if a1 is None else [_c(t.float()) for t in (a1, a2, b1, b2, ae)]
        yn, stats = ops.layernorm_fwd(y, alpha, None if beta is None else _c(beta.float()), eps, dtype, cout)
        ctx.save_for_backward(x, rs32, b32, y, stats, linear_skip_scale(skip_dx, rps, M), *w5, *(cs32 or []), *(alpha or []))
        ctx.meta = (cin, cout, rps, dtype, cs5 is not None, bias is not None, x_in_dtype, wt, alpha is not None,
                    beta is not None)
        ctx.set_materialize_grads(False)
        return y, yn

    @staticmethod
    def backward(ctx, dy, dyn):
        cin, cout, rps, dtype, has_cs, has_bias, x_in_dtype, wt, has_affine, has_beta = ctx.meta
        x, rs32, b32, y, stats, ss_dx, *rest = ctx.saved_tensors
        w5 = rest[:5]
        cs32 = rest[5:10] if has_cs else None
        alpha = rest[(10 if has_cs else 5):] if has_affine else None
        M = x.numel() // (8 * cin)
        dal, dbeta, g = [None] * 5, None, None
        if dyn is not None:
            dres = None if dy is None else _c(dy.float())
            gn = _c(dyn)
            if ops.layernorm_bwd_cast_ok(gn, y, cout) and dtype == torch.bfloat16:
                dy, dal_, dbeta, g = ops.layernorm_bwd_cast(gn, y, stats, alpha, dres, cout, rs32, rps,
                                                            want_param_grads=has_affine)
            else:
                dy, dal_, dbeta = ops.layernorm_bwd(gn, y, stats, alpha, dres, cout, want_param_grads=has_affine)
            dal = dal_ if dal_ is not None else dal
        dy = _c(dy)
        if g is None:
            g = ops.cast_rowscale(_c(dy.float()), rs32, rps, dtype, cout)
        gv, xv = ops.pview(g, cout), ops.pview(x, cin)
        dx = None
        if ctx.needs_input_grad[0]:
            dx = torch.empty(x.shape, dtype=dtype, device=x.device)
            ops.linear_fwd(gv, wt, None, ops.pview(dx, cin), M, cout, cin, dtype, dtype, x, sample_scale=ss_dx, skip_rps=rps)
            if dx.dtype != x_in_dtype:
                dx = dx.to(x_in_dtype)
        dysum = ops.colsum_a1(gv, M, cout, dtype, x) if (has_bias and not ops.wgrad_has_colsum(cin, cout, dtype)) else None
        w32 = [_c(w.detach().float()) for w in w5] if has_cs else None
        f32_masters = all(w.dtype == torch.float32 for w in w5)
        dw, dcs, dbias = ops.linear_wgrad(xv, gv, M, cin, cout, dtype, x, w32=w32, cs5=cs32, bias=b32, dysum=dysum,
                                          want_bias=has_bias, may_defer=f32_masters, wparams=w5 if f32_masters else None)
        if not f32_masters:
            dw = [d.to(w.dtype) for d, w in zip(dw, w5)]
        dcs = dcs if has_cs else [None] * 5
        return (dx, *dw, dbias, dy, None, *dcs, None, None, None, None, None, *dal, dbeta if has_beta else None, None, None)


class PackHeadsFn(torch.autograd.Function):

    @staticmethod
    def forward(ctx, qkv, H, c):
        B, T = qkv.shape[0], qkv.shape[1]
        ctx.meta = (B, T, H, c)
        q, k, v = ops.pack_heads(_c(qkv), B, T, H, c, 3)
        return q, k, v

    @staticmethod
    def backward(ctx, gq, gk, gv):
        B, T, H, c = ctx.meta
        return ops.unpack_heads([gq, gk, gv], B, T, H, c), None, None


class UnpackHeadsFn(torch.autograd.Function):
    @staticmethod
    def forward(ctx, o, c):
        B, H, T, _ = o.shape
        ctx.meta = (B, T, H, c)
        return ops.unpack_heads([o], B, T, H, c)

    @staticmethod
    def backward(ctx, g):
        B, T, H, c = ctx.meta
        return ops.pack_heads(_c(g), B, T, H, c, 1)[0], None


class AttnFn(torch.autograd.Function):

    @staticmethod
    def forward(ctx, q, k, v, scale):
        q, k, v = _c(q), _c(k), _c(v)
        o, lse = ops.attn_fwd(q, k, v, scale)
        ctx.save_for_backward(q, k, v, o, lse)
        ctx.scale = scale
        return o

    @staticmethod
    def backward(ctx, do):
        q, k, v, o, lse = ctx.saved_tensors
        do = _c(do)
        dq, dk, dv = torch.empty_like(q), torch.empty_like(k), torch.empty_like(v)
        ops.attn_bwd(q, k, v, o, do, lse, ctx.scale, dq, dk, dv)
        return dq, dk, dv, None


def _attn_skip_from_env():
    return os.environ.get("OCTIC_ATTN_SKIP", "1").strip() != "0"


ATTN_SKIP_DROPPED = _attn_skip_from_env()


def skip_scale(rs, B):
    if (not ATTN_SKIP_DROPPED or rs is None or not rs.is_cuda or rs.dtype != torch.float32 or rs.dim() != 1
            or rs.numel() != B or not rs.is_contiguous()):
        return None
    return rs.detach()


def _wgrad_skip_from_env():
    return os.environ.get("OCTIC_WGRAD_SKIP", "1").strip() != "0"


WGRAD_SKIP_DROPPED = _wgrad_skip_from_env()


def wgrad_skip_scale(rs, rps, M, rows_to=None):
    if (not WGRAD_SKIP_DROPPED or rs is None or rows_to is not None or torch.compiler.is_compiling() or not rs.is_cuda
            or rs.dtype != torch.float32 or rs.dim() != 1 or not rs.is_contiguous() or rps < 2 or rs.numel() * rps != M):
        return None
    return rs.detach()


def _linear_skip_from_env():
    return os.environ.get("OCTIC_LINEAR_SKIP", "1").strip() != "0"


LINEAR_SKIP_DROPPED = _linear_skip_from_env()


def linear_skip_scale(rs, rps, M, rows_to=None):
    if (not LINEAR_SKIP_DROPPED or rs is None or rows_to is not None or torch.compiler.is_compiling() or not rs.is_cuda
            or rs.dtype != torch.float32 or rs.dim() != 1 or not rs.is_contiguous() or rps < 2 or rs.numel() * rps != M):
        return None
    return rs.detach()


def _ring_skip_from_env():
    return os.environ.get("OCTIC_RING_SKIP", "1").strip() != "0"


RING_SKIP_DROPPED = _ring_skip_from_env()


def ring_skip_scale(rs, rps, M):
    return linear_skip_scale(rs, rps, M) if RING_SKIP_DROPPED else None


class AttnPackedFn(torch.autograd.Function):

    @staticmethod
    def forward(ctx, qkv, H, c, scale, sample_scale=None):
        qkv = _c(qkv)
        ss = skip_scale(sample_scale, qkv.shape[0])
        o, lse = ops.attn_fwd_packed(qkv, H, c, scale, sample_scale=ss)
        ctx.save_for_backward(qkv, o, lse, ss)
        ctx.meta = (H, c, scale)
        return o

    @staticmethod
    def backward(ctx, do):
        qkv, o, lse, ss = ctx.saved_tensors
        H, c, scale = ctx.meta
        return ops.attn_bwd_packed(qkv, o, _c(do), lse, H, c, scale, sample_scale=ss), None, None, None, None


class AttnFusedQKVFn(torch.autograd.Function):

    @staticmethod
    def forward(ctx, qkv, scale, sample_scale=None):
        qkv = _c(qkv)
        B, T, _, H, hd = qkv.shape
        ss = skip_scale(sample_scale, B) if qkv.dtype == torch.bfloat16 else None
        q, k, v = (qkv[:, :, i].permute(0, 2, 1, 3) for i in range(3))
        o = torch.empty((B, T, H, hd), dtype=qkv.dtype, device=qkv.device)
        ov = o.permute(0, 2, 1, 3)
        _, lse = ops.attn_fwd(q, k, v, scale, out=ov, sample_scale=ss)
        ctx.save_for_backward(qkv, o, lse, ss)
        ctx.scale = scale
        return o.view(B, T, H * hd)

    @staticmethod
    def backward(ctx, do):
        qkv, o, lse, ss = ctx.saved_tensors
        B, T, _, H, hd = qkv.shape
        do = _c(do).view(B, T, H, hd)
        dqkv = torch.empty_like(qkv)
        q, k, v = (qkv[:, :, i].permute(0, 2, 1, 3) for i in range(3))
        dq, dk, dv = (dqkv[:, :, i].permute(0, 2, 1, 3) for i in range(3))
        ops.attn_bwd(q, k, v, o.permute(0, 2, 1, 3), do.permute(0, 2, 1, 3), lse, ctx.scale, dq, dk, dv, sample_scale=ss)
        return dqkv, None, None


def attention_core(q, k, v, dropout_p=0.0):
    B, H, T, hd = q.shape
    if dropout_p == 0.0 and q.is_cuda and (ops.attn_supported(T, hd, q.dtype) or ops.attn_f32_supported(T, hd, q.dtype)):
        return AttnFn.apply(q, k, v, hd ** -0.5)
    o = torch.nn.functional.scaled_dot_product_attention(q, k, v, dropout_p=dropout_p)
    return o if o.dtype == q.dtype else o.to(q.dtype)


class DenseWeightCache:

    def __init__(self):
        self.key = None
        self.w = self.b = None
        self.wt = self.wt_key = None
        self.static = False
        self.static_wt = False

    def static_nt(self):
        if self.static and self.w is not None and self.w.dtype == torch.bfloat16:
            return self.w, (self.wt if self.static_wt else None)
        return None, None

    @staticmethod
    def _key(w, b, dtype):
        return (dtype, w.data_ptr(), w._version, None if b is None else (b.data_ptr(), b._version))

    def get(self, w, b, dtype):
        key = self._key(w, b, dtype)
        if key != self.key:
            with torch.no_grad():
                self.w = _c(w.detach().to(dtype))
                self.b = None if b is None else _c(b.detach().to(dtype))
            self.key = key
            self.wt, self.wt_key = None, None
            self.static = self.static_wt = False
        return self.w, self.b

    def adopt(self, w, b, w_copy, b_copy, dtype, wt_copy=None):
        self.w, self.b = w_copy, b_copy
        self.key = self._key(w, b, dtype)
        self.static = True
        self.static_wt = wt_copy is not None
        if wt_copy is not None:
            self.wt, self.wt_key = wt_copy, self.key

    def get_nt(self, w, b, need_wt=True):
        wb, _ = self.get(w, b, torch.bfloat16)
        if not need_wt:
            return wb, None
        if self.wt is None or self.wt_key != self.key:
            with torch.no_grad():
                self.wt = wb.t().contiguous()
            self.wt_key = self.key
        return wb, self.wt


class SoftCrossEntropyFn(torch.autograd.Function):

    @staticmethod
    def forward(ctx, s, tprob, temp):
        tprob = _c(tprob.detach().float())
        loss, lse, tsum = ops.soft_ce_fwd(s, tprob, 1.0 / temp)
        ctx.save_for_backward(s, tprob, lse, tsum)
        ctx.temp = temp
        return loss

    @staticmethod
    def backward(ctx, g):
        s, tprob, lse, tsum = ctx.saved_tensors
        return ops.soft_ce_bwd(s, tprob, 1.0 / ctx.temp, g, lse, tsum), None, None


def loss_rows_ok(t):
    return t.is_cuda and t.dtype in (torch.float32, torch.bfloat16) and t.shape[-1] % 8 == 0 and not torch.compiler.is_compiling()


class DenseLayerNormFn(torch.autograd.Function):

    @staticmethod
    def forward(ctx, x, w, b, eps, out_dtype):
        x = _c(x)
        w32 = None if w is None else _c(w.detach().float())
        b32 = None if b is None else _c(b.detach().float())
# ... 125 lines not shown
    def backward(ctx, gout):
        ab, wb, y, g32, rs32 = ctx.saved_tensors
        rps, has_b, has_gamma, a_dtype = ctx.meta
        gout = _c(gout.float())
        gy, dgamma, colsum = ops.scale_residual_bwd(gout, y, g32, rs32, rps, want_gamma=has_gamma, want_colsum=has_b)
        g2, a2 = gy.reshape(-1, wb.shape[0]), ab.reshape(-1, wb.shape[1])
        ga = _mm_lib(g2, wb).view(ab.shape).to(a_dtype) if ctx.needs_input_grad[1] else None
        gw = _wgrad_lib(g2, a2, ctx.wparam)
        return gout, ga, gw, colsum, dgamma, None, None, None, None


def invalidate_weight_caches(model):
    n = 0
    for m in model.modules():
        for attr in ("_prep", "_c1", "_c2"):
            c = getattr(m, attr, None)
            if isinstance(c, (WeightPrep, DenseWeightCache)):
                c.key = None
                if isinstance(c, DenseWeightCache):
                    c.wt, c.wt_key = None, None
                n += 1
    return n


def track_optimizer(model, optimizer):
    return optimizer.register_step_post_hook(lambda *_a, **_k: invalidate_weight_caches(model))


WGRAD_F32_OUT = False
DENSE_HIP = {"qkv", "dqkv", "proj", "dproj", "fc1", "dfc1", "fc2", "dfc2"}
DENSE_RESID_FUSED = False
NEXT_NORM_FUSED = True
OCTIC_NEXT_NORM = True
LN_TAIL_FUSED = True


def dense_hip_ok(x, w, which=None):
    rows = x.numel() // max(1, x.shape[-1])
    return (which is None or which in DENSE_HIP) and x.is_cuda and ops.dense_gemm_ok(rows, w.shape[0], w.shape[1])


def _f32(t):
    return None if t is None else _c(t.detach().float())


def _timed_lib(kind, fn, M, N, K):
    t = ops.KERNEL_TIMER.start()
    out = fn()
    if t is not None:
        ops.KERNEL_TIMER.stop(t, f"library_gemm<{kind} {N}x{K}>", 2 * (M * K + N * K + M * N), 2.0 * M * N * K)
    return out


WGRAD_SLABS = {(5120, 1280): 4, (1280, 5120): 4, (3840, 1280): 2, (1280, 1280): 2}


def wgrad_slabs(M, N, K):
    if WGRAD_SLABS is False:
        return 1
    S = WGRAD_SLABS.get((N, K))
    if S is None:
        tiles = -(-N // 256) * -(-K // 256)
        S = max(1, min(8, 256 // max(1, tiles)))
    while S > 1 and M % S:
        S -= 1
    return S


WGRAD_HIP = True


def _wgrad_lib(g2, x2, wparam=None, sample_scale=None, rps=0):
    M, N, K = g2.shape[0], g2.shape[1], x2.shape[1]
    if (WGRAD_HIP and g2.is_cuda and g2.dtype == torch.bfloat16 and x2.dtype == torch.bfloat16
            and g2.stride(1) == 1 and x2.stride(1) == 1
            and ops.dense_wgrad_ok(M, N, K, max(g2.stride(0), x2.stride(0)))):
        dest = ops.grad_dest(wparam, (N, K))
        dw = ops.dense_wgrad_tn(g2, x2, out=dest, sample_scale=sample_scale, rows_per_sample=rps if sample_scale is not None else 0)
        if dest is not None:
            ops.grad_written(wparam)
        return dw
    S = wgrad_slabs(M, N, K)
    if S > 1 and g2.is_contiguous() and x2.is_contiguous():
        with torch.autocast("cuda", enabled=False):
            return _timed_lib("wgrad", lambda: torch.bmm(g2.view(S, M // S, N).transpose(1, 2), x2.view(S, M // S, K))
                              .sum(0, dtype=torch.float32), M, N, K)
    with torch.autocast("cuda", enabled=False):
        if WGRAD_F32_OUT:
            return _timed_lib("wgrad", lambda: torch.mm(g2.t(), x2, out_dtype=torch.float32), g2.shape[0], g2.shape[1],
                              x2.shape[1])
        w = _timed_lib("wgrad", lambda: g2.t() @ x2, g2.shape[0], g2.shape[1], x2.shape[1])
        return w.float()


def _mm_lib(a2, b):
    with torch.autocast("cuda", enabled=False):
        return _timed_lib("dgrad", lambda: a2 @ b, a2.shape[0], b.shape[1], b.shape[0])


def _linear_lib(x2, wb, bias):
    with torch.autocast("cuda", enabled=False):
        return _timed_lib("fwd", lambda: torch.nn.functional.linear(x2, wb, bias), x2.shape[0], wb.shape[0], wb.shape[1])


WGRAD_PAIRED = True
GELU_FACTOR = True


class WgradPair:
    __slots__ = ("pending",)

    def __init__(self):
        self.pending = None

    def park(self, g2, x2, wparam=None, sample_scale=None, rps=0):
        shape = (g2.shape[1], x2.shape[1])
        dw = ops.grad_dest(wparam, shape)
        landed = wparam if dw is not None else None
        if dw is None:
            dw = torch.empty(shape, dtype=torch.float32, device=g2.device)
        self.pending = (g2, x2, dw.untyped_storage(), dw.data_ptr(), tuple(dw.shape), dw.storage_offset(), landed,
                        sample_scale, rps)
        ops.DEFERRED_FINISHES.add_pair(self)
        return dw

    def take(self):
        p, self.pending = self.pending, None
        if p is None:
            return None
        g2, x2, storage, ptr, shape, offset, landed, ss, rps = p
        dw = torch.empty(0, dtype=torch.float32, device=g2.device).set_(storage, offset, shape)
        assert dw.data_ptr() == ptr
        return g2, x2, dw, landed, ss, rps

    def flush(self):
        p = self.take()
        if p is not None:
            g2, x2, dw, landed, ss, rps = p
            dw.copy_(_wgrad_lib(g2, x2, sample_scale=ss, rps=rps))
            ops.grad_written(landed)


def _pair_ready(pair, g2, x2):
    return (pair is not None and WGRAD_PAIRED and WGRAD_HIP and ops.DEFERRED_FINISHES.enabled
            and ops.DEFERRED_FINISHES.allow_pairs and ops._in_backward()
            and g2.is_cuda and g2.dtype == torch.bfloat16 and x2.dtype == torch.bfloat16 and g2.stride(1) == 1
            and x2.stride(1) == 1)


def _tok(shape):
    return int(shape[-2]) if len(shape) >= 3 else 0


def _gemm_fwd(tag, x2, wb, b, cache, name, tokens):
    if tag in DENSE_HIP:
        return ops.dense_gemm_nt(x2, wb, 0, bias=_f32(b), name=f"dense_nt_kernel<{name}>", tokens=tokens)
    return _linear_lib(x2, wb, None if b is None else cache.b)


def _gemm_dgrad(g2, wt, wb, shape, dtype):
    gx = (ops.dense_gemm_nt(g2, wt, 0, name="dense_nt_kernel<dgrad>", tokens=_tok(shape)) if wt is not None
          else _mm_lib(g2, wb))
    return gx.view(shape).to(dtype)


def _resid_tail_fwd(ctx, x, tag, a2, wb, b, cache, tokens, g32, rs32, rps, nw, nb, neps, rows_to, stream):
    ctx.rows_to, ctx.x_shape = rows_to, x.shape
    ctx.tail = (neps is not None, rps, b is not None, nw is not None, nb is not None)
    x2 = x.view(-1, wb.shape[0])
    if neps is None and rows_to is None and tag in DENSE_HIP and DENSE_RESID_FUSED:
        br, out = ops.dense_gemm_nt(a2, wb, 2, bias=_f32(b), gamma=g32, rs=rs32, rps=rps, x=x2, name="dense_nt_kernel<resid>")
        return out.view(x.shape), (br, g32, rs32)
    br = _gemm_fwd(tag, a2, wb, b, cache, tag, tokens)
    if neps is not None:
        nw32, nb32 = _f32(nw), _f32(nb)
        out, yn, stats = ops.dense_resid_layernorm_fwd(x2, br, g32, rs32, rps, nw32, nb32, neps, torch.bfloat16)
        ctx.set_materialize_grads(False)
        return (out.view(x.shape), yn.view(x.shape)), (br, g32, rs32, out, stats, nw32)
    if rows_to is not None:
        ops.scale_residual_fwd_rows_(stream, rows_to.rowmap, x2, br, g32, rs32, rps)
        ctx.mark_dirty(stream)
        return stream, (br, g32, rs32, rows_to.rowmap)
    return ops.scale_residual_fwd(x2, br, g32, rs32, rps).view(x.shape), (br, g32, rs32)


def _resid_tail_bwd(ctx, tail, gout, gyn, want_norm):
    norm, rps, has_b, has_nw, has_nb = ctx.tail
    br, g32, rs32, *rest = tail
    has_gamma = g32 is not None
    dnw = dnb = gbr = None
    if norm:
        out, stats, nw32 = rest
        if gyn is not None:
            want = has_nw and want_norm
            dres = None if gout is None else _c(gout.float()).view(out.shape)
            g2 = _c(gyn).view(out.shape)
            if LN_TAIL_FUSED and ops.dense_ln_bwd_tail_ok(g2, br, out.shape[-1]):
                gout, dnw, dnb, gbr, dgamma, colsum = ops.dense_layernorm_bwd_tail(
                    g2, out, nw32, stats, dres, br, g32, rs32, rps, want_param_grads=want, want_gamma=has_gamma,
                    want_colsum=has_b)
            else:
                gout, dnw, dnb = ops.dense_layernorm_bwd(g2, out, nw32, stats, dres, want_param_grads=want)
            dnw, dnb = (dnw if has_nw else None), (dnb if has_nb else None)
    elif ctx.rows_to is not None:
        gout = _c(gout.float())
        ctx.rows_to.link.g = gout
        gbr, dgamma, colsum = ops.scale_residual_bwd(gout, br, g32, rs32, rps, want_gamma=has_gamma, want_colsum=has_b,
                                                     rowmap=rest[0])
    if gbr is None:
        gout = _c(gout.float())
        gbr, dgamma, colsum = ops.scale_residual_bwd(gout.view(br.shape), br, g32, rs32, rps, want_gamma=has_gamma,
                                                     want_colsum=has_b)
    gx = None if ctx.rows_to is not None else gout.view(ctx.x_shape)
    return gx, gbr, dgamma, colsum, dnw, dnb


class DenseLinearNTFn(torch.autograd.Function):

    @staticmethod
    def forward(ctx, x, w, b, cache, tag, pair=None, rs=None, rps=0):
        ctx.pair = pair
        ctx.wparam = w
        xb = _c(x if x.dtype == torch.bfloat16 else x.to(torch.bfloat16))
        wb, wt = cache.get_nt(w, b, ("d" + tag) in DENSE_HIP and ctx.needs_input_grad[0])
        x2 = xb.reshape(-1, wb.shape[1])
        y = _gemm_fwd(tag, x2, wb, b, cache, "plain", _tok(x.shape))
        ss = wgrad_skip_scale(rs, rps, x2.shape[0])
        ctx.rps = rps
        ctx.save_for_backward(x2, wb, wt, ss)
        ctx.meta = (b is not None, x.dtype, x.shape, tag)
        return y.view(*x.shape[:-1], wb.shape[0])

    @staticmethod
    def backward(ctx, gy):
        x2, wb, wt, ss = ctx.saved_tensors
        has_b, x_dtype, x_shape, tag = ctx.meta
        g2 = _c(gy).reshape(-1, wb.shape[0])
        gx = _gemm_dgrad(g2, wt, wb, x_shape, x_dtype) if ctx.needs_input_grad[0] else None
        gb = None
        if has_b:
            gb = (ops.dense_colsum(g2) if g2.is_cuda and g2.dtype == torch.bfloat16 and g2.shape[1] % 8 == 0
                  else g2.sum(0, dtype=torch.float32))
        pair = ctx.pair
        if pair is not None and pair.pending is not None:
            pg, px = pair.pending[0], pair.pending[1]
            if (_pair_ready(pair, g2, x2) and pg.shape[0] == g2.shape[0] and px.shape[1] == x2.shape[1]
                    and ops.dense_wgrad_pair_ok(g2.shape[0], g2.shape[1], pg.shape[1], x2.shape[1])):
                pg, px, pdw, landed, pss, prps = pair.take()
                dest = ops.grad_dest(ctx.wparam, (g2.shape[1], x2.shape[1]))
                both = ss if (ss is not None and pss is not None and prps == ctx.rps and pss.data_ptr() == ss.data_ptr()
                              and pss.numel() == ss.numel()) else None
                dw, _ = ops.dense_wgrad_tn_pair(g2, x2, pg, px, dw1=pdw, dw0=dest, sample_scale=both,
                                                rows_per_sample=ctx.rps if both is not None else 0)
                ops.grad_written(landed, ctx.wparam if dest is not None else None)
                return gx, dw, gb, None, None, None, None, None
            pair.flush()
        return gx, _wgrad_lib(g2, x2, ctx.wparam, ss, ctx.rps), gb, None, None, None, None, None


class DenseProjResidFn(torch.autograd.Function):

    @staticmethod
    def forward(ctx, x, a, w, b, gamma, rs, rps, cache, nw=None, nb=None, neps=None, pair=None, rows_to=None, stream=None):
        ctx.pair = pair
        ctx.wparam = w
        x = _c(x)
        ab = _c(a if a.dtype == torch.bfloat16 else a.to(torch.bfloat16))
        wb, wt = cache.get_nt(w, b, "dproj" in DENSE_HIP and ctx.needs_input_grad[1])
        a2 = ab.reshape(-1, wb.shape[1])
        outs, tail = _resid_tail_fwd(ctx, x, "proj", a2, wb, b, cache, _tok(a.shape), _f32(gamma), _f32(rs), rps,
                                     nw, nb, neps, rows_to, stream)
        ctx.save_for_backward(a2, wb, wt, *tail)
        ctx.meta = (a.dtype, a.shape)
        return outs

    @staticmethod
    def backward(ctx, gout, gyn=None):
        a2, wb, wt, *tail = ctx.saved_tensors
        a_dtype, a_shape = ctx.meta
        gx, gy, dgamma, colsum, dnw, dnb = _resid_tail_bwd(ctx, tail, gout, gyn,
                                                           ctx.needs_input_grad[8] or ctx.needs_input_grad[9])
        ga = _gemm_dgrad(gy, wt, wb, a_shape, a_dtype) if ctx.needs_input_grad[1] else None
        rps = ctx.tail[1]
        ss = wgrad_skip_scale(tail[2], rps, gy.shape[0], ctx.rows_to)
        if _pair_ready(ctx.pair, gy, a2) and ops.dense_wgrad_ok(gy.shape[0], gy.shape[1], a2.shape[1]):
            dw = ctx.pair.park(gy, a2, ctx.wparam, ss, rps)
        else:
            dw = _wgrad_lib(gy, a2, ctx.wparam, ss, rps)
        return gx, ga, dw, colsum, dgamma, None, None, None, dnw, dnb, None, None, None, None


class DenseMlpFn(torch.autograd.Function):

    @staticmethod
    def forward(ctx, y, x, w1, b1, w2, b2, gamma, rs, rps, c1, c2, nw=None, nb=None, neps=None, rows_to=None, stream=None):
        ctx.wparams = (w1, w2)
        x = _c(x)
        yb = _c(y if y.dtype == torch.bfloat16 else y.to(torch.bfloat16))
        need_t = any(ctx.needs_input_grad[:2])
        w1b, w1t = c1.get_nt(w1, b1, "dfc1" in DENSE_HIP and need_t)
        w2b, w2t = c2.get_nt(w2, b2, "dfc2" in DENSE_HIP and need_t)
        y2 = yb.reshape(-1, w1b.shape[1])
        g32, rs32 = _f32(gamma), _f32(rs)
        factor = GELU_FACTOR and "fc1" in DENSE_HIP and w2t is not None
        ctx.factor = factor
        if "fc1" in DENSE_HIP and not any(ctx.needs_input_grad):
            a = ops.dense_gemm_nt(y2, w1b, 6, bias=_f32(b1), name="dense_nt_kernel<gelu-only>", tokens=_tok(y.shape))
            h = a
        elif "fc1" in DENSE_HIP:
            h, a = ops.dense_gemm_nt(y2, w1b, 4 if factor else 1, bias=_f32(b1), name="dense_nt_kernel<gelu>",
                                     tokens=_tok(y.shape))
        else:
            h = _linear_lib(y2, w1b, None if b1 is None else c1.b)
            a = torch.nn.functional.gelu(h)
        outs, tail = _resid_tail_fwd(ctx, x, "fc2", a, w2b, b2, c2, _tok(y.shape), g32, rs32, rps,
                                     nw, nb, neps, rows_to, stream)
        ctx.save_for_backward(y2, h, a, w1b, w1t, w2b, w2t, *tail)
        ctx.meta = (b1 is not None, y.dtype, y.shape)
        return outs

    @staticmethod
    def backward(ctx, gout, gyn=None):
        y2, h, a, w1b, w1t, w2b, w2t, *tail = ctx.saved_tensors
        has_b1, y_dtype, y_shape = ctx.meta
        gx, gbr, dgamma, db2, dnw, dnb = _resid_tail_bwd(ctx, tail, gout, gyn,
                                                         ctx.needs_input_grad[11] or ctx.needs_input_grad[12])
        if w2t is not None:
            md = 5 if ctx.factor else 3
            if has_b1:
                dh, db1 = ops.dense_gemm_nt(gbr, w2t, md, h=h, name="dense_nt_kernel<dgelu>", want_colsum=True,
                                            tokens=_tok(y_shape))
            else:
                dh, db1 = ops.dense_gemm_nt(gbr, w2t, md, h=h, name="dense_nt_kernel<dgelu>", tokens=_tok(y_shape)), None
        else:
            dh, db1 = ops.dense_gelu_bwd(h, _mm_lib(gbr, w2b), want_colsum=has_b1)
        rps = ctx.tail[1]
        ss = wgrad_skip_scale(tail[2], rps, gbr.shape[0], ctx.rows_to)
        gw2 = _wgrad_lib(gbr, a, ctx.wparams[1], ss, rps)
        gw1 = _wgrad_lib(dh, y2, ctx.wparams[0], ss, rps)
        gy = _gemm_dgrad(dh, w1t, w1b, y_shape, y_dtype) if ctx.needs_input_grad[0] else None
        return gy, gx, gw1, db1, gw2, db2, dgamma, None, None, None, None, dnw, dnb, None, None, None


class HandoffCatFn(torch.autograd.Function):
    @staticmethod
    def forward(ctx, x, c, out_dtype):
        ctx.c, ctx.in_dtype = c, x.dtype
        return ops.handoff_cat_fwd(_c(x.float()), c, out_dtype)

    @staticmethod
    def backward(ctx, g):
        return ops.handoff_cat_bwd(g, ctx.c).to(ctx.in_dtype), None, None


class PowerSpectrumFn(torch.autograd.Function):
    @staticmethod
    def forward(ctx, x, c, out_dtype):
        x = _c(x.float())
        ctx.save_for_backward(x)
        ctx.c = c
        return ops.power_spectrum_fwd(x, c, out_dtype)

    @staticmethod
    def backward(ctx, g):
        (x,) = ctx.saved_tensors
        return ops.power_spectrum_bwd(g, x, ctx.c), None, None


class LiftFn(torch.autograd.Function):

    @staticmethod
    def forward(ctx, img, wfull, bias_full, pos, cls_row, p, dtype):
        B, Cin, Hh, Ww = img.shape
        D, K = wfull.shape
        Kpad = (K + 7) // 8 * 8
        n_p = (Hh // p) * (Ww // p)
        tok0 = 0 if cls_row is None else 1
        patches = ops.im2col(img, p, Kpad, dtype)
        wpad = torch.zeros((D, Kpad), dtype=dtype, device=img.device)
        wpad[:, :K] = wfull.detach()
        out = torch.empty((B, tok0 + n_p, D), dtype=torch.float32, device=img.device)
        ops.lift_gemm(patches, wpad, None if bias_full is None else _c(bias_full.detach().float()),
                      None if pos is None else _c(pos.detach().float()), out, B, n_p, tok0, Kpad, D)
        if tok0:
            out[:, 0] = cls_row.detach().float()
        ctx.save_for_backward(patches)
        ctx.meta = (B, n_p, tok0, K, Kpad, D, dtype, bias_full is not None, pos is not None)
        return out

    @staticmethod
    def backward(ctx, dout):
        (patches,) = ctx.saved_tensors
        B, n_p, tok0, K, Kpad, D, dtype, has_bias, has_pos = ctx.meta
        dtok = dout[:, tok0:]
        dcompact = _c(dtok.to(dtype)).reshape(B * n_p, D)
        dw = ops.lift_wgrad(patches, dcompact, Kpad, D)[:, :K]
        dpos = dtok.sum(0) if (has_pos or has_bias) else None
        dbias = dpos.sum(0) if has_bias else None
        dcls = dout[:, 0].sum(0) if tok0 else None
        return None, dw, dbias, dpos if has_pos else None, dcls, None, None
```

octic_vits_amd/ops.py:

```python
import ctypes
import operator

import torch

from . import _lib
from ._lib import BF16, F32, OcticView, PtrArray5, check, lib

_DT = {torch.float32: F32, torch.bfloat16: BF16}
_DTN = {torch.float32: "f32", torch.bfloat16: "bf16"}


class KernelTimer:

    def __init__(self):
        self.on = False
        self.records = []
        self.overhead_us = 0.0

    def enable(self):
        self.on, self.records = True, []
        pairs = []
        for _ in range(64):
            e0, e1 = torch.cuda.Event(enable_timing=True), torch.cuda.Event(enable_timing=True)
            e0.record()
# ... 905 lines not shown
        dw = torch.empty(d, dtype=torch.float32, device=x.device)
        db = torch.empty(d, dtype=torch.float32, device=x.device)
        _finish(p1, nblk, d, dw, db, None, _stream(x))
    if want2:
        dgamma = torch.empty(d, dtype=torch.float32, device=x.device) if want_gamma else None
        colsum = torch.empty(d, dtype=torch.float32, device=x.device) if want_colsum else None
        _finish(p2, nblk, d, dgamma, colsum, gamma, _stream(x))
    return dx, dw, db, gyb, dgamma, colsum


def _rows2d(t):
    K = t.shape[-1]
    t2 = t.reshape(-1, K)
    if t2.stride(1) != 1 or (t2.shape[0] > 1 and t2.stride(0) % 8):
        t2 = t2.contiguous()
    return t2, t2.shape[0], K, (t2.stride(0) if t2.shape[0] > 1 else K)


def softmax_center(t, center, inv_temp):
    _require_cuda(t)
    t2, rows, K, ld = _rows2d(t)
    out = torch.empty(t.shape, dtype=torch.float32, device=t.device)
    c = None if center is None else center.reshape(-1).float().contiguous()
    tk = KERNEL_TIMER.start()
    check(lib().octic_softmax_center(_p(t2), dt_code(t2.dtype), ld, _p(c), float(inv_temp), _p(out), rows, K, _stream(t)))
    KERNEL_TIMER.stop(tk, f"softmax_center_kernel<{_DTN[t2.dtype]}>", rows * K * (2 * t2.element_size() + 4))
    return out


def soft_ce_fwd(s, tprob, inv_temp):
    _require_cuda(s)
    s2, rows, K, ld = _rows2d(s)
    if tprob.dtype != torch.float32 or not tprob.is_contiguous() or tprob.shape[-1] != K:
        raise ValueError("soft_ce_fwd: tprob must be a contiguous f32 [Nt, K] tensor")
    nt = tprob.numel() // K
    loss, lse, tsum = (torch.empty(rows, dtype=torch.float32, device=s.device) for _ in range(3))
    tk = KERNEL_TIMER.start()
    check(lib().octic_soft_ce_fwd(_p(s2), dt_code(s2.dtype), ld, _p(tprob), nt, float(inv_temp), _p(loss), _p(lse), _p(tsum),
                                  rows, K, _stream(s)))
    KERNEL_TIMER.stop(tk, f"soft_ce_fwd_kernel<{_DTN[s2.dtype]}>", rows * K * (s2.element_size() + 4))
    return loss, lse, tsum


def soft_ce_bwd(s, tprob, inv_temp, g, lse, tsum):
    s2, rows, K, ld = _rows2d(s)
    nt = tprob.numel() // K
    ds = torch.empty((rows, K), dtype=s2.dtype, device=s.device)
    g = g.reshape(-1).float().contiguous()
    tk = KERNEL_TIMER.start()
    check(lib().octic_soft_ce_bwd(_p(s2), dt_code(s2.dtype), ld, _p(tprob), nt, float(inv_temp), _p(g), _p(lse), _p(tsum),
                                  _p(ds), K, rows, K, _stream(s)))
    KERNEL_TIMER.stop(tk, f"soft_ce_bwd_kernel<{_DTN[s2.dtype]}>", rows * K * (2 * s2.element_size() + 4))
    return ds.view(s.shape)


def scale_residual_fwd(x, y, gamma, rs, rps):
    _require_cuda(x)
    d = x.shape[-1]
    rows = x.numel() // d
    out = torch.empty_like(x)
    t = KERNEL_TIMER.start()
    check(lib().octic_scale_residual_fwd(_p(x), _p(y), dt_code(y.dtype), _p(gamma), _p(rs), int(rps), _p(out), rows, d,
                                         _stream(x)))
    KERNEL_TIMER.stop(t, f"scale_residual_fwd_kernel<{_DTN[y.dtype]}>", rows * d * (8 + y.element_size()))
    return out


def scale_residual_fwd_rows_(stream, rowmap, x, y, gamma, rs, rps):
    _require_cuda(x)
    d = x.shape[-1]
    rows = rowmap.numel()
    _check_rowmap(rowmap, rows)
    t = KERNEL_TIMER.start()
    check(lib().octic_scale_residual_fwd_rows(_p(x), _p(y), dt_code(y.dtype), _p(gamma), _p(rs), int(rps), _p(stream), rows, d,
                                              _p(rowmap), _stream(x)))
    KERNEL_TIMER.stop(t, f"scale_residual_fwd_kernel<{_DTN[y.dtype]},rows>", rows * d * (8 + y.element_size()))
    return stream


def scale_residual_bwd(gout, y, gamma, rs, rps, want_gamma=True, want_colsum=True, rowmap=None):
    d = gout.shape[-1]
    rows = gout.numel() // d if rowmap is None else rowmap.numel()
    if rowmap is not None:
        _check_rowmap(rowmap, rows)
    gy = torch.empty(gout.shape if rowmap is None else y.shape, dtype=y.dtype, device=gout.device)
    nblk = lib().octic_dense_blocks(rows)
    want = want_gamma or want_colsum
    partials = torch.empty((nblk, 2, d), dtype=torch.float32, device=gout.device) if want else None
    t = KERNEL_TIMER.start()
    check(lib().octic_scale_residual_bwd_rows(_p(gout), _p(y), dt_code(y.dtype), _p(gamma), _p(rs), int(rps), _p(gy),
                                              _p(partials), rows, d, _p(rowmap), _stream(gout)))
    KERNEL_TIMER.stop(t, f"scale_residual_bwd_kernel<{_DTN[y.dtype]}>", rows * d * (4 + 2 * y.element_size()))
    if not want:
        return gy, None, None
    dgamma = torch.empty(d, dtype=torch.float32, device=gout.device) if want_gamma else None
    colsum = torch.empty(d, dtype=torch.float32, device=gout.device) if want_colsum else None
    _finish(partials, nblk, d, dgamma, colsum, gamma, _stream(gout))
    return gy, dgamma, colsum


def dense_gelu_bwd(h, g, want_colsum=True):
    _require_cuda(h)
    d = h.shape[-1]
    rows = h.numel() // d
    dh = torch.empty_like(h)
    nblk = lib().octic_dense_gelu_blocks()
    partials = torch.empty((nblk, d), dtype=torch.float32, device=h.device) if want_colsum else None
    t = KERNEL_TIMER.start()
    check(lib().octic_dense_gelu_bwd(_p(h), _p(g), _p(dh), _p(partials), rows, d, _stream(h)))
    KERNEL_TIMER.stop(t, "dense_gelu_bwd_kernel", rows * d * 6)
    if not want_colsum:
        return dh, None
    out = torch.empty(d, dtype=torch.float32, device=h.device)
    half = d // 2
    _finish(partials, nblk, half, out, None, None, _stream(h), out1_ptr=out.data_ptr() + 4 * half)
    return dh, out


_DG_WS = {}
_lib.on_route_override(_DG_WS.clear)


def _dense_ws(M, N, K, dev):
    key = (M, N, K, dev)
    ws = _DG_WS.get(key)
    if ws is None:
        ws = _DG_WS[key] = torch.zeros(int(lib().octic_dense_gemm_workspace_bytes(M, N, K)), dtype=torch.uint8, device=dev)
    return ws


def dense_colsum(g):
    _require_cuda(g)
    rows, d = g.shape
    if g.stride(1) != 1:
        raise ValueError("dense_colsum: rows must be contiguous along d")
    nblk = lib().octic_dense_gelu_blocks()
    partials = torch.empty((nblk, d), dtype=torch.float32, device=g.device)
    t = KERNEL_TIMER.start()
    check(lib().octic_dense_colsum(_p(g), rows, d, g.stride(0), _p(partials), _stream(g)))
    KERNEL_TIMER.stop(t, "dense_colsum_kernel", rows * d * 2)
    out = torch.empty(d, dtype=torch.float32, device=g.device)
    half = d // 2
    _finish(partials, nblk, half, out, None, None, _stream(g), out1_ptr=out.data_ptr() + 4 * half)
    return out


def dense_plan(M, N, K, mode, tokens):
    out = _lib.plan("octic_dense_gemm_plan", M, N, K, mode, int(tokens))
    if out is None:
        check(-1)
    return out[0], out[1], bool(out[2]), out[3]


def dense_gemm_nt(a, b, mode=0, bias=None, gamma=None, rs=None, rps=1, x=None, h=None, name=None, want_colsum=False,
                  tokens=0):
    _require_cuda(a)
    M, K = a.shape
    N = b.shape[0]
    if a.stride(1) != 1 or b.stride(1) != 1 or b.shape[1] != K:
        raise ValueError("dense_gemm_nt: operands must be [M,K] / [N,K] with contiguous K")
    c = torch.empty((M, N), dtype=torch.bfloat16, device=a.device)
    c2 = torch.empty_like(c) if mode in (1, 4) else None
    out = torch.empty((M, N), dtype=torch.float32, device=a.device) if mode == 2 else None
    ws = _dense_ws(M, N, K, a.device)
    tokens = int(tokens) if (tokens and M % int(tokens) == 0) else 0
    cs_rows = dense_plan(M, N, K, mode, tokens)[1] if (mode in (3, 5) and want_colsum) else 0
    cs = torch.empty((cs_rows, N), dtype=torch.float32, device=a.device) if cs_rows else None
    t = KERNEL_TIMER.start()
    check(lib().octic_dense_gemm_nt_tokens(_p(a), _p(b), M, N, K, a.stride(0), b.stride(0), mode, _p(c), _p(c2), N, _p(bias),
                                           _p(gamma), _p(rs), int(rps), _p(x), _p(out), _p(h), _p(cs), _p(ws), tokens,
                                           _stream(a)))
    if t is not None:
        nb = 2 * (M * K + N * K + M * N * (2 if mode in (1, 3, 4, 5) else 1)) + (8 * M * N if mode == 2 else 0)
        wide = "@320" if dense_plan(M, N, K, mode, tokens)[0] == 320 else ""
        KERNEL_TIMER.stop(t, (name or f"dense_nt_kernel<{mode}>") + wide, nb, 2.0 * M * N * K)
    if mode in (1, 4):
        return c, c2
    if mode == 2:
        return c, out
    if cs is not None:
        colsum = torch.empty(N, dtype=torch.float32, device=a.device)
        _finish(cs, cs_rows, N // 2, colsum, None, None, _stream(a), out1_ptr=colsum.data_ptr() + 2 * N)
        return c, colsum
    return c


def probe_features(pairs, F):
    n = len(pairs)
    patch, cls0 = pairs[-1][0], pairs[0][1]
    _require_cuda(patch)
    B, P, D = patch.shape
    dtype = patch.dtype
    for p, c in pairs:
        if c.dtype != dtype or p.dtype != dtype or tuple(c.shape) != (B, D) or c.stride(1) != 1:
            raise ValueError("probe_features: class tokens must be [B, D] rows of one dtype")
    if patch.stride(2) != 1 or F.dtype != torch.float32 or F.stride(1) != 1 or F.shape[0] < B:
        raise ValueError("probe_features: patch tokens / F must have contiguous channels")
    cls = (ctypes.c_void_p * n)(*[c.data_ptr() for _, c in pairs])
    cls_ld = (ctypes.c_int64 * n)(*[c.stride(0) for _, c in pairs])
    t = KERNEL_TIMER.start()
    check(lib().octic_probe_features(cls, cls_ld, n, _p(patch), patch.stride(0), patch.stride(1), dt_code(dtype), B, P, D,
                                     _p(F), F.stride(0), _stream(patch)))
    KERNEL_TIMER.stop(t, f"probe_features_kernel<{_DTN[dtype]}>", B * D * (P + n) * patch.element_size() + 4 * B * (n + 1) * D)
    return F


def probe_forward(table, nheads, F, B, C, logits, sumK):
    t = KERNEL_TIMER.start()
    check(lib().octic_probe_forward(_p(table), nheads, _p(F), F.stride(0), B, C, _p(logits), _stream(F)))
    KERNEL_TIMER.stop(t, "probe_forward_kernel", 4 * (C * sumK + nheads * B * C), 2.0 * B * C * sumK)


def probe_ce(logits, labels, nheads, B, C, dlogits, rowloss, rowrank, loss_mean=None, loss_sum=None, topk=None):
    if labels.dtype != torch.int64 or not labels.is_contiguous() or labels.numel() != B:
        raise ValueError("probe_ce: labels must be a contiguous int64 tensor of B class indices")
    t = KERNEL_TIMER.start()
    check(lib().octic_probe_ce(_p(logits), _p(labels), nheads, B, C, _p(dlogits), _p(rowloss), _p(rowrank), _p(loss_mean),
                               _p(loss_sum), _p(topk), _stream(logits)))
    KERNEL_TIMER.stop(t, "probe_ce_kernel", 4 * nheads * B * C * (3 if dlogits is not None else 2))


def probe_sgd(table, nheads, total_ktiles, F, dlogits, B, C, lr, momentum, sumK):
    t = KERNEL_TIMER.start()
    check(lib().octic_probe_sgd(_p(table), nheads, total_ktiles, _p(F), F.stride(0), _p(dlogits), B, C, _p(lr),
                                float(momentum), _stream(F)))
    KERNEL_TIMER.stop(t, "probe_sgd_kernel", 16 * C * sumK, 2.0 * B * C * sumK)


def _seg_rows(X):
    _require_cuda(X)
    if X.dim() != 2 or X.dtype != torch.float32 or X.stride(1) != 1:
        raise ValueError("segmentation ops take an f32 [N, D] matrix with contiguous channels")
    return X.shape[0], X.shape[1], X.stride(0)


def seg_ldd(C):
    ldd = lib().octic_seg_ldd(int(C))
    check(min(ldd, 0))
    return ldd


def seg_workspace(N, D, C, device):
    nbytes = lib().octic_seg_workspace_bytes(N, D, C)
    check(min(nbytes, 0))
    return torch.empty(nbytes, dtype=torch.uint8, device=device)


def seg_value_dlogits(X, W, b, y, dlogits, value, workspace):
    N, D, ldx = _seg_rows(X)
    C = W.shape[0]
    if (W.dtype != torch.float32 or not W.is_contiguous() or W.shape[1] != D or b.dtype != torch.float32 or b.numel() != C
            or not b.is_contiguous()):
        raise ValueError("seg_value_dlogits: W must be a contiguous f32 [C, D], b a contiguous f32 [C]")
    if y.dtype != torch.int32 or not y.is_contiguous() or y.numel() != N:
        raise ValueError("seg_value_dlogits: y must be a contiguous int32 tensor of N class indices")
    if (dlogits.dtype != torch.float32 or not dlogits.is_contiguous() or dlogits.numel() < N * max(seg_ldd(C), 0)
            or value.dtype != torch.float64):
        raise ValueError("seg_value_dlogits: dlogits must be a contiguous f32 [N, seg_ldd(C)], value an f64 scalar")
    t = KERNEL_TIMER.start()
    check(lib().octic_seg_value_dlogits(_p(X), ldx, N, D, _p(W), _p(b), C, _p(y), _p(dlogits), _p(value), _p(workspace),
                                        _stream(X)))
    KERNEL_TIMER.stop(t, "seg_forward_kernel", 4 * N * (D + seg_ldd(C)), 2.0 * N * C * D)


def seg_predict(X, W, b, pred):
    N, D, ldx = _seg_rows(X)
    C = W.shape[0]
    if W.dtype != torch.float32 or not W.is_contiguous() or W.shape[1] != D or b.dtype != torch.float32 or b.numel() != C:
        raise ValueError("seg_predict: W must be a contiguous f32 [C, D], b an f32 [C]")
    if pred.dtype != torch.int32 or not pred.is_contiguous() or pred.numel() != N:
        raise ValueError("seg_predict: pred must be a contiguous int32 [N]")
    t = KERNEL_TIMER.start()
    check(lib().octic_seg_predict(_p(X), ldx, N, D, _p(W), _p(b), C, _p(pred), _stream(X)))
    KERNEL_TIMER.stop(t, "seg_forward_kernel<predict>", 4 * N * (D + 1), 2.0 * N * C * D)


def seg_wgrad(X, dlogits, W, scale, lam, dW, db, workspace):
    N, D, ldx = _seg_rows(X)
    C = W.shape[0]
    if (dW.dtype != torch.float32 or not dW.is_contiguous() or tuple(dW.shape) != (C, D) or db.dtype != torch.float32
            or db.numel() != C or not W.is_contiguous() or W.dtype != torch.float32):
        raise ValueError("seg_wgrad: W / dW must be contiguous f32 [C, D], db an f32 [C]")
    t = KERNEL_TIMER.start()
    check(lib().octic_seg_wgrad(_p(X), ldx, N, D, _p(dlogits), C, _p(W), float(scale), float(lam), _p(dW), _p(db),
                                _p(workspace), _stream(X)))
    KERNEL_TIMER.stop(t, "seg_wgrad_kernel", 4 * N * D, 2.0 * N * C * D)


def seg_colstats(X):
    N, D, ldx = _seg_rows(X)
    nbytes = lib().octic_seg_colstats_workspace_bytes(N, D)
    check(min(nbytes, 0))
    ws = torch.empty(nbytes // 8, dtype=torch.float64, device=X.device)
    mean = torch.empty(D, dtype=torch.float64, device=X.device)
    var = torch.empty(D, dtype=torch.float64, device=X.device)
    t = KERNEL_TIMER.start()
    check(lib().octic_seg_colstats(_p(X), ldx, N, D, _p(mean), _p(var), _p(ws), _stream(X)))
    KERNEL_TIMER.stop(t, "seg_colstats_kernel", 4 * N * D)
    return mean, var


def seg_standardize_(X, mean, scale):
    N, D, ldx = _seg_rows(X)
    for v in (mean, scale):
        if v.dtype != torch.float64 or v.numel() != D or not v.is_contiguous() or v.device != X.device:
            raise ValueError("seg_standardize_: mean and scale must be contiguous f64 [D] on X's device")
    t = KERNEL_TIMER.start()
    check(lib().octic_seg_standardize(_p(X), ldx, N, D, _p(mean), _p(scale), _stream(X)))
    KERNEL_TIMER.stop(t, "seg_standardize_kernel", 8 * N * D)
    return X


_SEG_LABEL_DTYPES = (torch.uint8, torch.int16, torch.int32, torch.int64)


def _seg_labels(labels):
    _require_cuda(labels)
    if labels.dim() != 2 or labels.dtype not in _SEG_LABEL_DTYPES or not labels.is_contiguous():
        raise ValueError("segmentation labels must be a contiguous [R, L] tensor of uint8 / int16 / int32 / int64 values 0 .. 255")
    return labels.shape[0], labels.shape[1], labels.element_size()


def seg_patch_mode(labels):
    R, L, es = _seg_labels(labels)
    mode = torch.empty(R, dtype=torch.int32, device=labels.device)
    if R:
        t = KERNEL_TIMER.start()
# ... 114 lines not shown
```

octic_vits_amd/probe.py:

```python
from collections import OrderedDict

import numpy as np
import torch

DEFAULT_LEARNING_RATES = (1e-5, 2e-5, 5e-5, 1e-4, 2e-4, 5e-4, 1e-3, 2e-3, 5e-3, 1e-2, 2e-2, 5e-2, 0.1)
STATE_PREFIX = "classifiers_dict."


def create_linear_input(x_tokens_list, use_n_blocks, use_avgpool):
    last = x_tokens_list[-use_n_blocks:]
    parts = [cls for _, cls in last]
    if use_avgpool:
        parts.append(last[-1][0].mean(dim=1))
    out = torch.cat(parts, dim=-1)
    return out.reshape(out.shape[0], -1).float()


def scale_lr(learning_rate, batch_size, world_size=1):
    return learning_rate * (batch_size * world_size) / 256.0


def classifier_name(n_blocks, avgpool, lr):
    return f"classifier_{n_blocks}_blocks_avgpool_{avgpool}_lr_{lr:.5f}".replace(".", "_")


def classifier_grid(embed_dim, n_last_blocks_list=(1, 4), learning_rates=DEFAULT_LEARNING_RATES, batch_size=128, world_size=1):
    heads, n_groups = OrderedDict(), 0
    for n in n_last_blocks_list:
        for avgpool in (False, True):
            for base in learning_rates:
                lr = scale_lr(base, batch_size, world_size)
                heads[classifier_name(n, avgpool, lr)] = dict(n_blocks=n, avgpool=avgpool, lr=lr,
                                                              out_dim=(n + int(avgpool)) * embed_dim)
                n_groups += 1
    return heads, n_groups


_HEAD_DTYPE = np.dtype([("w", "<u8"), ("b", "<u8"), ("mw", "<u8"), ("mb", "<u8"), ("col0", "<i4"), ("K", "<i4"),
                        ("lr_index", "<i4"), ("tile0", "<i4")])


class LinearProbe:

    def __init__(self, model, n_last_blocks_list=(1, 4), learning_rates=DEFAULT_LEARNING_RATES, batch_size=128, num_classes=1000,
                 autocast_dtype=torch.bfloat16, world_size=1, device=None, generator=None, embed_dim=None):
        self.model = model
        self.autocast_dtype = autocast_dtype
        self.batch_size, self.num_classes = int(batch_size), int(num_classes)
        D = self.embed_dim = int(model.embed_dim if model is not None else embed_dim)
        if D % 64:
            raise ValueError(f"LinearProbe: embed_dim {D} must be a multiple of 64")
        self.n_blocks = max(n_last_blocks_list)
        if not 1 <= self.n_blocks <= 4 or min(n_last_blocks_list) < 1:
            raise ValueError("LinearProbe: n_last_blocks within 1 .. 4")
        self.heads, self.n_reference_groups = classifier_grid(D, n_last_blocks_list, learning_rates, batch_size, world_size)
        self.names = list(self.heads)
        if device is None:
            device = next(self.model.parameters()).device if self.model is not None else torch.device("cpu")
        self.device = torch.device(device)
        C, nh = self.num_classes, len(self.names)
        self.width = (self.n_blocks + 1) * D
        self.sum_k = sum(h["out_dim"] for h in self.heads.values())
        self.total_ktiles = self.sum_k // 64
        n_w = C * self.sum_k
        self.flat = torch.zeros(n_w + nh * C, dtype=torch.float32, device=self.device)
        self.momentum = torch.zeros_like(self.flat)
        self.weights, self.biases, self.momentum_w, self.momentum_b = OrderedDict(), OrderedDict(), OrderedDict(), OrderedDict()
        off = 0
        for i, (name, h) in enumerate(self.heads.items()):
            K = h["out_dim"]
            h["col0"] = (self.n_blocks - h["n_blocks"]) * D
            self.weights[name] = self.flat[off:off + C * K].view(C, K)
            self.momentum_w[name] = self.momentum[off:off + C * K].view(C, K)
            self.biases[name] = self.flat[n_w + i * C:n_w + (i + 1) * C]
            self.momentum_b[name] = self.momentum[n_w + i * C:n_w + (i + 1) * C]
            off += C * K
            self.weights[name].normal_(mean=0.0, std=0.01, generator=generator)
        self.lr = torch.zeros(nh, dtype=torch.float32, device=self.device)
        self.optimizer = None
        self._cap = 0
        self._table = None
        self._have_grad, self._last_F = False, None
        if self.device.type == "cuda":
            tab = np.zeros(nh, dtype=_HEAD_DTYPE)
            tile0 = 0
            for i, (name, h) in enumerate(self.heads.items()):
                tab[i] = (self.weights[name].data_ptr(), self.biases[name].data_ptr(), self.momentum_w[name].data_ptr(),
                          self.momentum_b[name].data_ptr(), h["col0"], h["out_dim"], i, tile0)
                tile0 += h["out_dim"] // 64
            self._table = torch.from_numpy(tab.view(np.uint8).copy()).to(self.device)
            self.loss = torch.zeros(nh, dtype=torch.float32, device=self.device)
            self.loss_sum = torch.zeros(nh, dtype=torch.float32, device=self.device)
            self.topk = torch.zeros(nh, 2, dtype=torch.int32, device=self.device)
            self._reserve(self.batch_size)

    def __len__(self):
        return len(self.names)

    def _reserve(self, B):
        if B <= self._cap:
            return
        if torch.cuda.is_current_stream_capturing():
            raise RuntimeError("LinearProbe: a batch larger than the reserved buffers during graph capture")
        nh, C = len(self.names), self.num_classes
        self.features = torch.zeros(B, self.width, dtype=torch.float32, device=self.device)
        self._logits = torch.empty(nh * B * C, dtype=torch.float32, device=self.device)
        self._dlogits = torch.empty(nh * B * C, dtype=torch.float32, device=self.device)
        self._rowloss = torch.empty(nh * B, dtype=torch.float32, device=self.device)
        self._rowrank = torch.empty(nh * B, dtype=torch.int32, device=self.device)
        self._cap = B

    def _need_gpu(self):
        if self._table is None:
            raise RuntimeError("LinearProbe: the probe kernels run on the GPU only (no CPU fallback)")

    def logits(self, B):
        nh, C = len(self.names), self.num_classes
        return self._logits[:nh * B * C].view(nh, B, C)

    def dlogits(self, B):
        nh, C = len(self.names), self.num_classes
        return self._dlogits[:nh * B * C].view(nh, B, C)

    def extract(self, images):
        self._need_gpu()
        if self.model is None:
            raise RuntimeError("LinearProbe: built without a backbone (feature rows only)")
        self.model.eval()
        B = images.shape[0]
        self._reserve(B)
        with torch.no_grad():
            if self.autocast_dtype is None:
                pairs = self.model.get_intermediate_layers(images, self.n_blocks, return_class_token=True)
            else:
                with torch.autocast("cuda", dtype=self.autocast_dtype):
                    pairs = self.model.get_intermediate_layers(images, self.n_blocks, return_class_token=True)
            return self.features_from_tokens(pairs)

    def features_from_tokens(self, pairs):
        from . import ops
        self._need_gpu()
        B = pairs[-1][0].shape[0]
        self._reserve(B)
        if len(pairs) != self.n_blocks or pairs[-1][0].shape[-1] != self.embed_dim:
            raise ValueError(f"LinearProbe: expected {self.n_blocks} (patch tokens, class token) pairs of width {self.embed_dim}")
        F = self.features[:B]
        ops.probe_features(pairs, F)
        return F

    def _check_features(self, F):
        if (not F.is_cuda or F.dtype != torch.float32 or F.dim() != 2 or F.shape[1] != self.width or F.stride(1) != 1
                or F.stride(0) % 4 or F.data_ptr() % 16):
# ... 5 lines not shown
        self._check_features(F)
        B = F.shape[0]
        self._reserve(B)
        ops.probe_forward(self._table, len(self.names), F, B, self.num_classes, self._logits, self.sum_k)
        self._last_F = F
        return self.logits(B)

    def loss_and_grad(self, labels, B, train=True):
        from . import ops
        nh = len(self.names)
        if train:
            ops.probe_ce(self._logits, labels, nh, B, self.num_classes, self._dlogits, self._rowloss, self._rowrank,
                         loss_mean=self.loss)
            self._grad_F, self._grad_B, self._have_grad = self._last_F, B, True
        else:
            ops.probe_ce(self._logits, labels, nh, B, self.num_classes, None, self._rowloss, self._rowrank,
                         loss_sum=self.loss_sum, topk=self.topk)

    def step_features(self, F, labels):
        if self.optimizer is None:
            raise RuntimeError("LinearProbe.step: build a ProbeSGD(probe) first")
        self.forward_features(F)
        self.loss_and_grad(labels, F.shape[0], train=True)
        self.optimizer.step()
        return self.loss

    def step(self, images, labels):
        return self.step_features(self.extract(images), labels)

    def capture(self, example_images, example_labels, warmup=2):
        return CapturedProbeStep(self, example_images, example_labels, warmup)

    def evaluate(self, batches, metric_type="mean_accuracy", class_mapping=None, on_features=False):
        if str(getattr(metric_type, "value", metric_type)) != "mean_accuracy":
            raise NotImplementedError(f"LinearProbe.evaluate: metric type {metric_type!r} (only mean_accuracy)")
        if class_mapping is not None:
            raise NotImplementedError("LinearProbe.evaluate: class mappings")
        self._need_gpu()
        self.loss_sum.zero_()
        self.topk.zero_()
        n = 0
        for x, labels in batches:
            F = x if on_features else self.extract(x)
            self.forward_features(F)
            self.loss_and_grad(labels, F.shape[0], train=False)
            n += F.shape[0]
        topk = self.topk.cpu()
        loss = self.loss_sum.cpu()
        results, best, best_acc = OrderedDict(), "", 0
        for i, name in enumerate(self.names):
            top1 = topk[i, 0].item() / max(n, 1)
            results[name] = {"top-1": top1, "top-5": topk[i, 1].item() / max(n, 1), "loss": loss[i].item() / max(n, 1)}
            if top1 > best_acc:
                best, best_acc = name, top1
        return {"best_classifier": {"name": best, "accuracy": best_acc}, "classifiers": results, "samples": n}

    def state_dict(self):
        sd = OrderedDict()
        for name in self.names:
            sd[f"{STATE_PREFIX}{name}.linear.weight"] = self.weights[name].detach().clone()
            sd[f"{STATE_PREFIX}{name}.linear.bias"] = self.biases[name].detach().clone()
        return sd

    def load_state_dict(self, sd):
        sd = {(k[len("module."):] if k.startswith("module.") else k): v for k, v in sd.items()}
        want = set(self.state_dict_keys())
        if set(sd) != want:
            raise KeyError(f"LinearProbe.load_state_dict: missing {sorted(want - set(sd))[:3]}, unexpected {sorted(set(sd) - want)[:3]}")
        for name in self.names:
            self.weights[name].copy_(sd[f"{STATE_PREFIX}{name}.linear.weight"])
            self.biases[name].copy_(sd[f"{STATE_PREFIX}{name}.linear.bias"])

    def state_dict_keys(self):
        return [f"{STATE_PREFIX}{name}.linear.{p}" for name in self.names for p in ("weight", "bias")]


class ProbeSGD(torch.optim.Optimizer):

    def __init__(self, probe, momentum=0.9):
        self.probe = probe
        groups = [{"params": [probe.weights[n], probe.biases[n]], "lr": probe.heads[n]["lr"], "name": n} for n in probe.names]
        super().__init__(groups, dict(lr=0.0, momentum=momentum))
        self._key, self._ring, self._ring_i = None, None, 0
        probe.optimizer = self

    def push_lr(self):
        key = tuple(float(g["lr"]) for g in self.param_groups)
        if key == self._key or torch.cuda.is_current_stream_capturing():
            return False
        if self._ring is None:
            self._ring = [[torch.empty(len(key), dtype=torch.float32).pin_memory(), None] for _ in range(4)]
        slot = self._ring[self._ring_i]
        self._ring_i = (self._ring_i + 1) % len(self._ring)
        if slot[1] is not None:
            slot[1].synchronize()
        slot[0].copy_(torch.tensor(key, dtype=torch.float64))
        self.probe.lr.copy_(slot[0], non_blocking=True)
        slot[1] = torch.cuda.Event()
        slot[1].record()
        self._key = key
        return True

    @torch.no_grad()
    def step(self, closure=None):
        from . import ops
        p = self.probe
        p._need_gpu()
        if closure is not None:
            raise NotImplementedError("ProbeSGD.step: closures")
        if not p._have_grad:
            raise RuntimeError("ProbeSGD.step: no gradient - run LinearProbe.step / loss_and_grad first")
        momenta = {float(g["momentum"]) for g in self.param_groups}
        if len(momenta) != 1:
            raise ValueError("ProbeSGD: one momentum for all classifiers")
        self.push_lr()
        ops.probe_sgd(p._table, len(p.names), p.total_ktiles, p._grad_F, p._dlogits, p._grad_B, p.num_classes, p.lr,
                      momenta.pop(), p.sum_k)
        if not torch.cuda.is_current_stream_capturing():
            p._have_grad = False

    def zero_grad(self, set_to_none=True):
        self.probe._have_grad = False

    def state_dict(self):
        return {"momentum_buffer": self.probe.momentum.detach().clone(),
                "param_groups": [{k: v for k, v in g.items() if k != "params"} for g in self.param_groups]}

    def load_state_dict(self, sd):
        if [g["name"] for g in sd["param_groups"]] != self.probe.names:
            raise KeyError("ProbeSGD.load_state_dict: the classifier names differ")
        self.probe.momentum.copy_(sd["momentum_buffer"])
        for g, s in zip(self.param_groups, sd["param_groups"]):
            g.update(s)
        self._key = None


class CapturedProbeStep:

    def __init__(self, probe, images, labels, warmup=2):
        if not images.is_cuda or probe.optimizer is None:
            raise RuntimeError("CapturedProbeStep: CUDA example inputs and a ProbeSGD are required")
        self.probe = probe
        self.images = images.detach().clone()
        self.labels = labels.detach().clone()
        dev = images.device
        side = torch.cuda.Stream(dev)
        side.wait_stream(torch.cuda.current_stream(dev))
        with torch.cuda.stream(side):
            for _ in range(max(1, warmup)):
                probe.extract(self.images)
        torch.cuda.current_stream(dev).wait_stream(side)
        torch.cuda.synchronize(dev)
        probe.optimizer.push_lr()
        self.graph = torch.cuda.CUDAGraph()
        with torch.cuda.graph(self.graph):
            self.loss = probe.step(self.images, self.labels)
        probe._have_grad = False
        self._stamp = self._param_stamp()

    def _param_stamp(self):
        return tuple((p.data_ptr(), p._version) for p in self.probe.model.parameters())

    def __call__(self, images, labels):
        if images.shape != self.images.shape or images.dtype != self.images.dtype or labels.shape != self.labels.shape:
            raise ValueError(f"CapturedProbeStep: input {tuple(images.shape)} {images.dtype} / labels {tuple(labels.shape)} differ "
                             f"from the captured {tuple(self.images.shape)} {self.images.dtype} / {tuple(self.labels.shape)}")
        if self._param_stamp() != self._stamp:
            raise RuntimeError("CapturedProbeStep: the backbone's parameters changed since the capture - capture again")
        if self.probe.model.training:
            raise RuntimeError("CapturedProbeStep: the backbone was switched to training mode")
        self.images.copy_(images, non_blocking=True)
        self.labels.copy_(labels, non_blocking=True)
        self.probe.optimizer.push_lr()
        self.graph.replay()
        return self.loss

    replay = __call__
```

octic_vits_amd/serve.py:

```python
import torch


class GraphedForward:
    def __init__(self, model, example, autocast_dtype=torch.bfloat16, warmup=2):
        if not example.is_cuda:
            raise RuntimeError("GraphedForward: a CUDA example input (its shape and dtype become the graph's)")
        self.model = model.eval()
        self.autocast_dtype = autocast_dtype
        self.static_in = example.detach().clone()
        side = torch.cuda.Stream(example.device)
        side.wait_stream(torch.cuda.current_stream(example.device))
        with torch.cuda.stream(side), torch.no_grad():
            for _ in range(max(1, warmup)):
                self._run()
        torch.cuda.current_stream(example.device).wait_stream(side)
        torch.cuda.synchronize(example.device)
        self.graph = torch.cuda.CUDAGraph()
        with torch.no_grad(), torch.cuda.graph(self.graph):
            self.static_out = self._run()
        self._stamp = self._param_stamp()

    def _run(self):
        if self.autocast_dtype is None:
            return self.model(self.static_in)
        with torch.autocast("cuda", dtype=self.autocast_dtype):
            return self.model(self.static_in)

    def _param_stamp(self):
        return tuple((p.data_ptr(), p._version) for p in self.model.parameters())

    def __call__(self, x, copy_out=True):
        if x.shape != self.static_in.shape or x.dtype != self.static_in.dtype:
            raise ValueError(f"GraphedForward: input {tuple(x.shape)} {x.dtype} differs from the captured "
                             f"{tuple(self.static_in.shape)} {self.static_in.dtype}")
        if self._param_stamp() != self._stamp:
            raise RuntimeError("GraphedForward: the model's parameters changed since the capture (the graph reads frozen "
                               "compute-dtype copies of them) - build a new GraphedForward")
        if self.model.training:
            raise RuntimeError("GraphedForward: the model was switched to training mode")
        self.static_in.copy_(x, non_blocking=True)
        self.graph.replay()
        out = self.static_out
        if not copy_out:
            return out
        return out.clone() if torch.is_tensor(out) else out
```

octic_vits_amd/train.py:

```python
import math
import os

import torch
import torch.distributed as dist
import torch.nn as nn


DDP_BUCKET_MB = 48
DDP_FLAT_SMALL_NUMEL = 100_000
GRAD_BUCKET_MB = 96
DDP_GRADS_IN_BUCKETS = True


class Lamb(torch.optim.Optimizer):

    def __init__(self, params, lr=3e-3, betas=(0.9, 0.999), eps=1e-8, weight_decay=0.02, max_grad_norm=1.0):
        super().__init__(params, dict(lr=lr, betas=betas, eps=eps, weight_decay=weight_decay, max_grad_norm=max_grad_norm))
        self.last_grad_norm = None

    @torch.no_grad()
    def step(self):
        grads_all = [p.grad for g in self.param_groups for p in g["params"] if p.grad is not None]
        norms = torch._foreach_norm(grads_all)
        gnorm = torch.linalg.vector_norm(torch.stack(norms))
        self.last_grad_norm = gnorm
        if not bool(torch.isfinite(gnorm)):
            self.skipped_steps = getattr(self, "skipped_steps", 0) + 1
            return
        mg = self.param_groups[0]["max_grad_norm"]
        clip = torch.clamp(gnorm / mg, min=1.0) if mg is not None else None
        for group in self.param_groups:
            params = [p for p in group["params"] if p.grad is not None]
            if not params:
                continue
            grads = [p.grad for p in params]
            if clip is not None:
                grads = torch._foreach_div(grads, clip)
            b1, b2 = group["betas"]
            for p in params:
                st = self.state[p]
                if not st:
                    st["step"] = 0
                    st["exp_avg"] = torch.zeros_like(p)
                    st["exp_avg_sq"] = torch.zeros_like(p)
            group["step"] = group.get("step", 0) + 1
            t = group["step"]
            m = [self.state[p]["exp_avg"] for p in params]
            v = [self.state[p]["exp_avg_sq"] for p in params]
            torch._foreach_lerp_(m, grads, 1 - b1)
            torch._foreach_mul_(v, b2)
            torch._foreach_addcmul_(v, grads, grads, 1 - b2)
            bc1, bc2 = 1 - b1 ** t, 1 - b2 ** t
            denom = torch._foreach_sqrt(v)
            torch._foreach_div_(denom, math.sqrt(bc2))
            torch._foreach_add_(denom, group["eps"])
            upd = torch._foreach_div(m, denom)
            torch._foreach_div_(upd, bc1)
            wd = group["weight_decay"]
            if wd != 0:
                torch._foreach_add_(upd, params, alpha=wd)
                wn = torch._foreach_norm(params)
                un = torch._foreach_norm(upd)
                wn_t, un_t = torch.stack(wn), torch.stack(un)
                ratio = torch.where((wn_t > 0) & (un_t > 0), wn_t / un_t, torch.ones_like(wn_t))
                torch._foreach_mul_(upd, list(ratio.unbind(0)))
            torch._foreach_add_(params, upd, alpha=-group["lr"])


class FusedLamb:

    CHUNK = 65536

    def __init__(self, param_groups, lr=3e-3, betas=(0.9, 0.999), eps=1e-8, max_grad_norm=1.0, ema_decay=None,
                 shadow_layers=(), prep_source=None, adam=False, ema_tensors=None):
        from . import _lib
        self._lib = _lib
        self.adam = bool(adam)
        self._lr, self.betas, self.eps, self.max_grad_norm, self.ema_decay = lr, betas, eps, max_grad_norm, ema_decay
        self.params, self.param_groups, self._group_sizes = [], [], []
        for g in param_groups:
            ps = [p for p in g["params"] if p.requires_grad]
            group = {k: v for k, v in g.items() if k != "params"}
            group["params"] = ps
            group.setdefault("lr", lr)
            group.setdefault("weight_decay", 0.0)
            self.param_groups.append(group)
            self._group_sizes.append(len(ps))
            self.params += ps
        dev = self.params[0].device
        if dev.type != "cuda":
            raise RuntimeError("FusedLamb runs on the GPU only")
        offs, total = [], 0
        for p in self.params:
            offs.append(total)
            total += (p.numel() + 3) // 4 * 4
        self.m = torch.zeros(total, dtype=torch.float32, device=dev)
        self.v = torch.zeros(total, dtype=torch.float32, device=dev)
        self.ema = None
        self._ema_ext = None
        if ema_tensors is not None:
            self._ema_ext = [ema_tensors[id(p)] for p in self.params]
            for p, e in zip(self.params, self._ema_ext):
                if e.shape != p.shape or e.dtype != torch.float32 or not e.is_contiguous() or e.device != p.device:
                    raise ValueError("FusedLamb: an external EMA tensor must be a contiguous f32 twin of its parameter")
        elif ema_decay:
            self.ema = torch.zeros(total, dtype=torch.float32, device=dev)
            for p, o in zip(self.params, offs):
                self.ema[o:o + p.numel()].copy_(p.detach().flatten())
        self._offs = offs
        ct, co, cl, tb = [], [], [], [0]
        for i, p in enumerate(self.params):
            n = p.numel()
            for o in range(0, n, self.CHUNK):
                ct.append(i); co.append(o); cl.append(min(self.CHUNK, n - o))
            tb.append(len(ct))
        i32, i64 = torch.int32, torch.int64
        self.chunk_tensor = torch.tensor(ct, dtype=i32, device=dev)
        self.chunk_off = torch.tensor(co, dtype=i64, device=dev)
        self.chunk_len = torch.tensor(cl, dtype=i32, device=dev)
        self.tensor_chunk_begin = torch.tensor(tb, dtype=i32, device=dev)
        n = len(self.params)
        key = self._hyper_key()
        self.hyper = torch.from_numpy(self._hyper_values(key)).to(dev)
        self.lr_t, self.wd, self.ema_decay_t = self.hyper[:n], self.hyper[n:2 * n], self.hyper[2 * n:]
        self._hp_key, self._hp_ring, self._hp_i = key, None, 0
        base = lambda t: [t.data_ptr() + 4 * o for o in offs]
        self.p_ptrs = torch.tensor([p.data_ptr() for p in self.params], dtype=i64, device=dev)
        self.m_ptrs = torch.tensor(base(self.m), dtype=i64, device=dev)
        self.v_ptrs = torch.tensor(base(self.v), dtype=i64, device=dev)
        self.e_ptrs = torch.tensor(base(self.ema), dtype=i64, device=dev) if self.ema is not None else None
        if self._ema_ext is not None:
            self.e_ptrs = torch.tensor([e.data_ptr() for e in self._ema_ext], dtype=i64, device=dev)
        self.g_ptrs = torch.zeros(len(self.params), dtype=i64, device=dev)
        index = {id(p): i for i, p in enumerate(self.params)}
        sh_ptrs, self._shadows = [0] * len(self.params), []
        from . import functional as _OF
        for item in shadow_layers:
            lin, cache = item[0], item[1]
            need_wt = len(item) < 3 or ("d" + item[2]) in _OF.DENSE_HIP
            w, b = lin.weight, lin.bias
            if id(w) not in index or (b is not None and id(b) not in index):
                continue
            wb = torch.empty_like(w, dtype=torch.bfloat16)
            bb = None if b is None else torch.empty_like(b, dtype=torch.bfloat16)
            sh_ptrs[index[id(w)]] = wb.data_ptr()
            if b is not None:
                sh_ptrs[index[id(b)]] = bb.data_ptr()
            self._shadows.append((lin, cache, wb, bb, need_wt))
        self.s_ptrs = torch.tensor(sh_ptrs, dtype=i64, device=dev) if self._shadows else None
        self._wt, self._wt_items, self._wt_blocks = [], None, 0
        wt_layers = [sh for sh in self._shadows if sh[4]]
        self._wt = [None] * len(self._shadows)
# ... 819 lines not shown
    def _aug_batch(self, samples):
        return self.augment.launch(samples, self._aug_table(samples.shape[0], samples.device).table)

    def _mix_draw(self, samples):
        if self.augment is not None and samples.dtype == torch.uint8:
            B, H, W, _ = samples.shape
        else:
            B, _, H, W = samples.shape
        return self._mix_table(B, samples.device).upload(self.mixup.draw(B, H, W))

    def _mix_batch(self, samples, labels):
        from . import mixup as M
        table = self._mix_table(samples.shape[0], samples.device).table
        mixed = M.mix_images(samples, table)
        on, off = self.mixup.on_off()
        if self.fused_loss:
            return mixed, _MixedTargets(labels, table, on, off)
        return mixed, M.mix_targets(labels, table, self.mixup.num_classes, on=on, off=off, binarize=True)

    def _batched_finishes(self, first_of_many=False):
        from . import ops
        safe = (BATCHED_FINISHES and self.device_type == "cuda" and self.model is self.raw_model
                and (self.accum_steps == 1 or first_of_many))
        return _FinishScope(ops.DEFERRED_FINISHES, safe)

    def _reduced_backward(self, loss, hold=False):
        r = self._reducer
        r.begin(hold=hold)
        try:
            with self._batched_finishes(first_of_many=hold):
                loss.backward()
        except BaseException:
            r.abort()
            raise
        if hold:
            r.settle()
        else:
            r.finish()

    def _accumulate(self, samples, targets):
        k = self.accum_steps
        xs, ys = samples.chunk(k), targets.chunk(k)
        loss = None
        for i, (x, y) in enumerate(zip(xs, ys)):
            last = i == len(xs) - 1
            ctx = self.model.no_sync() if (hasattr(self.model, "no_sync") and not last) else _null()
            with ctx:
                li = self._forward_loss(x, y) / len(xs)
                if self._reducer is not None and i == 0:
                    self._reduced_backward(li, hold=True)
                elif i == 0:
                    with self._batched_finishes(first_of_many=True):
                        li.backward()
                else:
                    li.backward()
            loss = li.detach() if loss is None else loss + li.detach()
        if self._reducer is not None:
            self._reducer.reduce_all()
        return loss

    def step(self, samples, targets):
        if self._ddp_args is not None and self.model is self.segmented:
            raise RuntimeError("Trainer(distributed=True, segment_graphs=n): call capture_segments(micro_batch) before the "
                               "first step (the slices are captured, then wrapped in DistributedDataParallel)")
        if self.augment is not None:
            self.augment.check_batch(samples, "Trainer(augment=...)")
        if self.mixup is not None:
            self._mix_check(samples, targets)
        self.model.train()
        self._steps += 1
        if self._steps % self.check_every == 0:
            self._watch.check()
        if self.augment is not None:
            self._aug_draw(samples)
            samples = self._aug_batch(samples)
        if self.mixup is not None:
            self._mix_draw(samples)
            samples, targets = self._mix_batch(samples, targets)
        k = self.accum_steps
        if k > 1 and self.segmented is not None and self.segmented.graphed:
            params = [p for p in self.raw_model.parameters() if p.requires_grad]
            for p in params:
                if p.grad is None:
                    p.grad = torch.zeros_like(p)
            torch._foreach_zero_([p.grad for p in params])
        else:
            self.optimizer.zero_grad(set_to_none=True)
        if k == 1:
            loss = self._forward_loss(samples, targets)
            dest = getattr(self, "_grad_dest", None)
            if dest is not None:
                from . import ops as _ops
                _ops.GRAD_DEST = dest
                try:
                    with _FinishScope(_ops.DEFERRED_FINISHES, BATCHED_FINISHES and self._vectors_outside_ddp, vectors_only=True):
                        loss.backward()
                finally:
                    _ops.GRAD_DEST = None
                for p in self._ddp_params:
                    if p.grad is not None:
                        dest[p.data_ptr()] = p.grad
            elif self._reducer is not None:
                self._reduced_backward(loss)
            else:
                with self._batched_finishes():
                    loss.backward()
        else:
            loss = self._accumulate(samples, targets)
        self._reduce_small_grads()
        if self._proxy is not None:
            self._proxy.join()
        self.optimizer.step()
        if self.ema is not None:
            self.ema.update(self.raw_model)
        self._watch.push(loss)
        return loss.detach()

    def capture(self, samples, targets, warmup=3):
        if self.device_type != "cuda" or not isinstance(self.optimizer, FusedLamb):
            raise RuntimeError("Trainer.capture needs the GPU and the fused optimizer")
        if self.model is not self.raw_model:
            raise RuntimeError("Trainer.capture: DistributedDataParallel / segmented steps are not captured as one graph "
                               "(own_reducer=True, or segment_graphs=n + capture_segments)")
        from . import d8_layers as _L
        if _L.COMPACT_DROP_PATH:
            raise RuntimeError("Trainer.capture: d8_layers.COMPACT_DROP_PATH launches every branch on the samples its mask "
                               "keeps - the shapes change from step to step and cannot be one captured graph; run eagerly")
        from . import ops
        if ops.KERNEL_TIMER.on:
            raise RuntimeError("Trainer.capture: disable the kernel timer first")
        if self.mixup is not None:
            self._mix_check(samples, targets)
        if self.augment is not None:
            self.augment.check_batch(samples, "Trainer(augment=...)")
        sx, sy = samples.clone(), targets.clone()
        for _ in range(max(1, warmup)):
            self.step(sx, sy)
        torch.cuda.synchronize()
        self.model.train()
        graph = torch.cuda.CUDAGraph()
        self.optimizer.prepare_capture()
        self.optimizer.zero_grad(set_to_none=True)
        mode = {"capture_error_mode": "thread_local"} if self._reducer is not None else {}
        if self._reducer is not None:
            self._reducer.capturing = True
        try:
            loss = self._capture_body(graph, mode, sx, sy)
        finally:
            if self._reducer is not None:
                self._reducer.capturing = False
        return GraphedStep(self, graph, sx, sy, loss.detach())

    def _capture_body(self, graph, mode, sx, sy):
        with torch.cuda.graph(graph, **mode):
            if self.augment is not None:
                sx = self._aug_batch(sx)
            if self.mixup is not None:
                sx, sy = self._mix_batch(sx, sy)
            if self.accum_steps > 1:
                loss = self._accumulate(sx, sy)
            else:
                loss = self._forward_loss(sx, sy)
                if self._reducer is not None:
                    self._reduced_backward(loss)
                else:
                    with self._batched_finishes():
                        loss.backward()
            self.optimizer.step()
        return loss


BATCHED_FINISHES = True


class _FinishScope:
    def __init__(self, deferred, on, vectors_only=False):
        self.deferred, self.on, self.vectors_only = deferred, on, vectors_only

    def __enter__(self):
        from . import d8_layers as _L
        self.prev = (self.deferred.enabled, self.deferred.allow_pairs)
        self.deferred.enabled = self.on
        self.deferred.slabs_too = not _L.COMPACT_DROP_PATH and not self.vectors_only
        self.deferred.allow_pairs = not self.vectors_only
        return self

    def __exit__(self, *exc):
        self.deferred.enabled, self.deferred.allow_pairs = self.prev
        self.deferred.flush()
        return False


class _MixedTargets:

    def __init__(self, labels, table, on, off, row0=0, rows=None):
        self.labels, self.table, self.on, self.off, self.row0 = labels, table, on, off, row0
        self.rows = labels.shape[0] - row0 if rows is None else rows

    def chunk(self, k):
        size = -(-self.rows // k)
        return [_MixedTargets(self.labels, self.table, self.on, self.off, self.row0 + o, min(size, self.rows - o))
                for o in range(0, self.rows, size)]

    def loss(self, logits):
        from .mixup import mix_bce_loss
        if logits.shape[0] != self.rows:
            raise ValueError("Trainer: the logits do not match the mixed targets' rows")
        return mix_bce_loss(logits, self.labels, self.table, on=self.on, off=self.off, binarize=True, row0=self.row0)


class GraphedStep:

    def __init__(self, trainer, graph, samples, targets, loss):
        self.trainer, self.graph, self.samples, self.targets, self.loss = trainer, graph, samples, targets, loss

    def replay(self, samples=None, targets=None):
        t = self.trainer
        t._steps += 1
        if t._steps % t.check_every == 0:
            t._watch.check()
        if samples is not None and samples.data_ptr() != self.samples.data_ptr():
            if t.augment is not None:
                t.augment.check_batch(samples, "Trainer(augment=...)")
            self.samples.copy_(samples, non_blocking=True)
        if targets is not None and targets.data_ptr() != self.targets.data_ptr():
            if t.mixup is not None:
                t._mix_check(self.samples, targets)
            self.targets.copy_(targets, non_blocking=True)
        if t.augment is not None:
            t._aug_draw(self.samples)
        if t.mixup is not None:
            t._mix_draw(self.samples)
        t.optimizer.push_hyper()
        self.graph.replay()
        t.optimizer.step_count += 1
        t._watch.push(self.loss)
        return self.loss


class _null:
    def __enter__(self):
        return self

    def __exit__(self, *a):
        return False


@torch.no_grad()
def evaluate(model, batches, graphed=True):
    from . import ops
    model.eval()
    gf = None
    loss_sum = topk = None
    n = 0
    for images, labels in batches:
        ops._require_cuda(images)
        ops._require_cuda(labels)
        if labels.dtype != torch.int64 or labels.dim() != 1 or labels.shape[0] != images.shape[0]:
            raise ValueError("evaluate: labels must be int64 class indices [B]")
        if images.dtype == torch.uint8:
            from .augment import to_tensor
            images = to_tensor(images)
        if loss_sum is None:
            loss_sum = torch.zeros(1, dtype=torch.float32, device=images.device)
            topk = torch.zeros(2, dtype=torch.int32, device=images.device)
        if graphed and gf is None:
            from .serve import GraphedForward
            gf = GraphedForward(model, images)
        if gf is not None and images.shape == gf.static_in.shape and images.dtype == gf.static_in.dtype:
            logits = gf(images, copy_out=False)
        else:
            with torch.autocast("cuda", dtype=torch.bfloat16):
                logits = model(images)
        logits = logits.float().contiguous()
        B, C = logits.shape
        rowloss = torch.empty(B, dtype=torch.float32, device=logits.device)
        rowrank = torch.empty(B, dtype=torch.int32, device=logits.device)
        ops.probe_ce(logits, labels.contiguous(), 1, B, C, None, rowloss, rowrank, loss_sum=loss_sum, topk=topk)
        n += B
    if n == 0:
        raise ValueError("evaluate: no batch")
    total = torch.cat([loss_sum.double(), topk.double()]).cpu()
    return {"loss": float(total[0]) / n, "acc1": 100.0 * float(total[1]) / n, "acc5": 100.0 * float(total[2]) / n}


def init_distributed(force=False):
    world = int(os.environ.get("WORLD_SIZE", "1"))
    rank = int(os.environ.get("RANK", "0"))
    local_rank = int(os.environ.get("LOCAL_RANK", "0"))
    if world > 1 or force:
        os.environ.setdefault("MASTER_ADDR", "127.0.0.1")
        os.environ.setdefault("HSA_ENABLE_IPC_MODE_LEGACY", "0")
        os.environ.setdefault("TORCH_NCCL_CUDA_EVENT_CACHE", "0")
        backend = "nccl" if torch.cuda.is_available() else "gloo"
        if torch.cuda.is_available():
            torch.cuda.set_device(local_rank)
        dist.init_process_group(backend=backend, rank=rank, world_size=world)
    return world, rank, local_rank
```

Before: 1149 images/s.

## Skip dense GEMM tiles for drop-path-dropped samples via per-sample mask

Adds a SKIP variant of the dense NT GEMM kernel. It builds a bitmask of live M-panels from the per-sample drop-path scale in LDS. Tiles whose rows belong only to dropped samples are zero-filled instead of computed, and live tiles are reordered so they are spread across CUs. The fc1 forward, the dgelu backward and the dgrad GEMMs in the MLP and residual blocks now pass this scale, so with drop_path 0.5 roughly half the panel work can be skipped. It also adds gc.collect() before graph capture. The cost is extra mask and scheduling logic per block and possible load imbalance, since the schedule is decided on device at replay time.

```diff
diff --git a/include/octic_hip.h b/include/octic_hip.h
--- a/include/octic_hip.h
+++ b/include/octic_hip.h
@@ -305,6 +305,14 @@
                                int64_t rows_per_sample, const float* X, float* OUT, const void* H, float* colsum,
                                void* workspace, int tokens, void* stream);
 int octic_dense_gemm_plan(int M, int N, int K, int mode, int tokens, int* out4);
+int octic_dense_gemm_nt_tokens_skip(const void* A, const void* B, int M, int N, int K, int64_t lda, int64_t ldb, int mode, void* C,
+                                    void* C2, int64_t ldc, const float* bias, const float* gamma, const float* rs,
+                                    int64_t rows_per_sample_rs, const float* X, float* OUT, const void* H, float* colsum,
+                                    const float* sample_scale, int rows_per_sample, void* workspace, int tokens,
+                                    void* stream);
+int octic_dense_gemm_plan_dropped(int M, int N, int K, int mode, int tokens, int rows_per_sample, int* out4);
+int octic_dense_gemm_order_dropped(int M, int N, int K, int mode, int tokens, const float* sample_scale, int rows_per_sample,
+                                   int cap, int* out_tm, int* out_tn, int* out_part, int* out_split, int* out_dead);
 
 int64_t octic_dense_wgrad_workspace_bytes(int M, int N, int K);
 int octic_dense_wgrad_tile(int M, int N, int K);
diff --git a/octic_vits_amd/_lib.py b/octic_vits_amd/_lib.py
--- a/octic_vits_amd/_lib.py
+++ b/octic_vits_amd/_lib.py
@@ -143,6 +143,12 @@
                                            c_i64, c_void_p, c_void_p, c_void_p, c_i64, c_void_p, c_void_p, c_void_p, c_void_p,
                                            c_void_p, c_int, c_void_p]),
     "octic_dense_gemm_plan": (c_int, [c_int, c_int, c_int, c_int, c_int, ctypes.POINTER(c_int)]),
+    "octic_dense_gemm_nt_tokens_skip": (c_int, [c_void_p, c_void_p, c_int, c_int, c_int, c_i64, c_i64, c_int, c_void_p, c_void_p,
+                                                c_i64, c_void_p, c_void_p, c_void_p, c_i64, c_void_p, c_void_p, c_void_p, c_void_p,
+                                                c_void_p, c_int, c_void_p, c_int, c_void_p]),
+    "octic_dense_gemm_plan_dropped": (c_int, [c_int, c_int, c_int, c_int, c_int, c_int, ctypes.POINTER(c_int)]),
+    "octic_dense_gemm_order_dropped": (c_int, [c_int, c_int, c_int, c_int, c_int, c_void_p, c_int, c_int, c_void_p, c_void_p,
+                                               c_void_p, c_void_p, c_void_p]),
     "octic_dense_colsum": (c_int, [c_void_p, c_i64, c_int, c_i64, c_void_p, c_void_p]),
     "octic_dense_wgrad_workspace_bytes": (c_i64, [c_int, c_int, c_int]),
     "octic_dense_wgrad_tile": (c_int, [c_int, c_int, c_int]),
diff --git a/octic_vits_amd/csrc/dense_gemm.hip b/octic_vits_amd/csrc/dense_gemm.hip
--- a/octic_vits_amd/csrc/dense_gemm.hip
+++ b/octic_vits_amd/csrc/dense_gemm.hip
@@ -50,12 +50,102 @@
   int tail_pad;
   float* slabs;
   int* tickets;
+  const float* sample_scale;
+  int rows_per_sample;
 };
 
 enum DgMode { DG_PLAIN = 0, DG_GELU = 1, DG_RESID = 2, DG_DGELU = 3,
               DG_GELUF = 4,
               DG_DFACT = 5,
               DG_GELUO = 6 };
+
+constexpr int kDgMaskCap = 1024;
+constexpr int kDgMaskWords = kDgMaskCap / 64;
+
+__host__ __device__ inline bool dg_panel_live(const float* scale, int rps, int M, int m_stride, int m_base, int tm) {
+  const int m0 = tm * m_stride + m_base;
+  if (m0 >= M) return false;
+  const int m1 = (m0 + DG_BM < M ? m0 + DG_BM : M) - 1;
+  const int b1 = m1 / rps;
+  for (int b = m0 / rps; b <= b1; ++b)
+    if (scale[b] != 0.0f) return true;
+  return false;
+}
+__host__ __device__ inline int dg_group_bits(const unsigned long long* bm, int g, int gsz, bool live) {
+  int b = (int)((bm[g >> 3] >> ((g & 7) * 8)) & 0xffull);
+  if (!live) b = ~b;
+  return b & ((1 << gsz) - 1);
+}
+__host__ __device__ inline int dg_group_count(int bits, int gsz, int tiles_n, int cut) {
+  if (cut == gsz * tiles_n) return tiles_n * __builtin_popcount(bits);
+  const int cols = cut / gsz, rest = cut - cols * gsz;
+  return cols * __builtin_popcount(bits) + __builtin_popcount(bits & ((1 << rest) - 1));
+}
+__host__ __device__ inline int dg_live_full(const unsigned long long* bm, int tiles_m, int tiles_n, int full) {
+  const int per_group = 8 * tiles_n;
+  int L = 0;
+  for (int g = 0; g * per_group < full; ++g) {
+    const int gsz = tiles_m - 8 * g < 8 ? tiles_m - 8 * g : 8;
+    const int left = full - g * per_group, cut = left < gsz * tiles_n ? left : gsz * tiles_n;
+    L += dg_group_count(dg_group_bits(bm, g, gsz, true), gsz, tiles_n, cut);
+  }
+  return L;
+}
+__host__ __device__ inline int dg_select_full(const unsigned long long* bm, int tiles_m, int tiles_n, int full, int k, bool live) {
+  const int per_group = 8 * tiles_n;
+  for (int g = 0; g * per_group < full; ++g) {
+    const int gsz = tiles_m - 8 * g < 8 ? tiles_m - 8 * g : 8;
+    const int left = full - g * per_group, cut = left < gsz * tiles_n ? left : gsz * tiles_n;
+    int bits = dg_group_bits(bm, g, gsz, live);
+    const int cnt = dg_group_count(bits, gsz, tiles_n, cut);
+    if (k < cnt) {
+      const int lg = __builtin_popcount(bits);
+      const int col = k / lg;
+      int idx = k - col * lg, pos = 0;
+      for (; pos < 8; ++pos) {
+        if (bits & 1) {
+          if (idx == 0) break;
+          --idx;
+        }
+        bits >>= 1;
+      }
+      return g * per_group + col * gsz + pos;
+    }
+    k -= cnt;
+  }
+  return 0;
+}
+__host__ __device__ inline void dg_tile_panel(int tiles_m, int tiles_n, int tile, int& tm, int& tn) {
+  const int per_group = 8 * tiles_n, gidx = tile / per_group, first_m = gidx * 8;
+  const int gsz = (tiles_m - first_m) < 8 ? (tiles_m - first_m) : 8;
+  const int in_g = tile - gidx * per_group;
+  tm = first_m + in_g % gsz;
+  tn = in_g / gsz;
+}
+__host__ __device__ inline void dense_item_masked(int tiles_m, int tiles_n, int full, int split, int tail_pad, int bid,
+                                                  const unsigned long long* bm, int& tile, int& rem_idx, int& part, bool& dead) {
+  tile = -1; rem_idx = -1; part = 0; dead = false;
+  if (bid < tail_pad) {
+    if (bid >= (tiles_m * tiles_n - full) * split) return;
+    rem_idx = bid / split;
+    part = bid - rem_idx * split;
+    tile = full + rem_idx;
+    int tm, tn;
+    dg_tile_panel(tiles_m, tiles_n, tile, tm, tn);
+    dead = ((bm[tm >> 6] >> (tm & 63)) & 1ull) == 0;
+    return;
+  }
+  const int j = bid - tail_pad;
+  const int L = dg_live_full(bm, tiles_m, tiles_n, full), D = full - L;
+  if (j < D) {
+    tile = dg_select_full(bm, tiles_m, tiles_n, full, j, false);
+    dead = true;
+    return;
+  }
+  const int i = j - D, x = i & 7, q8 = L >> 3, r8 = L & 7;
+  const int rank = (x < r8 ? x * (q8 + 1) : r8 * (q8 + 1) + (x - r8) * q8) + (i >> 3);
+  tile = dg_select_full(bm, tiles_m, tiles_n, full, rank, true);
+}
 
 __device__ inline void dg_wait_vmcnt(int n) {
   switch (n) {
@@ -138,12 +228,13 @@
   else asm volatile("s_waitcnt vmcnt(0)" ::: "memory");
 }
 
-template <int MODE, int NT>
+template <int MODE, int NT, bool SKIP = false>
 __global__ __launch_bounds__(512, 1) void dense_nt_kernel(DgArgs a) {
   extern __shared__ __attribute__((aligned(16))) char lds[];
   using GE = DgGeom<NT>;
   constexpr int NA = GE::NA, DG_BN = GE::BN;
   static_assert(NT == 4 || MODE == DG_PLAIN, "the fused tails exist for the 256-wide tile only");
+  static_assert(!SKIP || MODE != DG_RESID, "the fused residual tail never takes a mask");
 
   const int lane = threadIdx.x & 63;
   const int wid = __builtin_amdgcn_readfirstlane(threadIdx.x >> 6);
@@ -168,6 +259,26 @@
   const int bid = blockIdx.x;
   int tile, kt_begin, kt_end, part = 0, rem_idx = -1;
   const int nkt_all = a.K / DG_BK;
+  bool dead_item = false;
+  if constexpr (SKIP) {
+    unsigned long long* const live_bm = (unsigned long long*)(lds + GE::LDS);
+    const int words = (a.tiles_m + 63) >> 6;
+    for (int w = wid; w < words; w += 8) {
+      const int p = w * 64 + lane;
+      const bool live = p < a.tiles_m && dg_panel_live(a.sample_scale, a.rows_per_sample, a.M, a.m_stride, a.m_base, p);
+      const unsigned long long m = __ballot(live);
+      if (lane == 0) live_bm[w] = m;
+    }
+    __syncthreads();
+    dense_item_masked(a.tiles_m, a.tiles_n, a.full_tiles, a.split, a.tail_pad, bid, live_bm, tile, rem_idx, part, dead_item);
+    tile = __builtin_amdgcn_readfirstlane(tile);
+    rem_idx = __builtin_amdgcn_readfirstlane(rem_idx);
+    part = __builtin_amdgcn_readfirstlane(part);
+    dead_item = __builtin_amdgcn_readfirstlane((int)dead_item) != 0;
+    if (tile < 0) return;
+    kt_begin = rem_idx >= 0 ? (int)(((int64_t)nkt_all * part) / a.split) : 0;
+    kt_end = rem_idx >= 0 ? (int)(((int64_t)nkt_all * (part + 1)) / a.split) : nkt_all;
+  } else
   if (bid >= a.tail_pad) {
     const int j = bid - a.tail_pad;
     const int nf = a.full_tiles;
@@ -196,6 +307,28 @@
     tn = in_g / gsz;
   }
   const int m0 = tm * a.m_stride + a.m_base, n0 = tn * DG_BN;
+  if constexpr (SKIP) {
+    if (dead_item) {
+      if (part != 0) return;
+      constexpr int CPR = DG_BN / 8;
+      const u32x4 z = {0, 0, 0, 0};
+#pragma unroll 4
+      for (int p = threadIdx.x; p < DG_BM * CPR; p += 512) {
+        const int r = p / CPR, c = p - r * CPR;
+        const int m = m0 + r, n = n0 + c * 8;
+        if (m < a.M && n < a.N) {
+          *(u32x4*)(a.C + (int64_t)m * a.ldc + n) = z;
+          if (MODE == DG_GELU || MODE == DG_GELUF) *(u32x4*)(a.C2 + (int64_t)m * a.ldc + n) = z;
+        }
+      }
+      if ((MODE == DG_DGELU || MODE == DG_DFACT) && a.colsum != nullptr) {
+        const int t = threadIdx.x;
+        const int row = t / (DG_BN / 4), n = n0 + (t - row * (DG_BN / 4)) * 4;
+        if (row < 2 && n < a.N) *(f32x4*)(a.colsum + (int64_t)(tm * 2 + row) * a.N + n) = f32x4{0, 0, 0, 0};
+      }
+      return;
+    }
+  }
   const int nkt = kt_end - kt_begin;
   const int nunits = 4 * nkt;
 
@@ -899,11 +1032,13 @@
   return 2 * ((M + DG_BM - 1) / DG_BM);
 }
 
-int octic_dense_gemm_nt_tokens(const void* A, const void* B, int M, int N, int K, int64_t lda, int64_t ldb, int mode, void* C,
-                               void* C2, int64_t ldc, const float* bias, const float* gamma, const float* rs, int64_t rps,
-                               const float* X, float* OUT, const void* H, float* colsum, void* workspace, int tokens,
-                               void* stream) {
+int octic_dense_gemm_nt_tokens_skip(const void* A, const void* B, int M, int N, int K, int64_t lda, int64_t ldb, int mode, void* C,
+                                    void* C2, int64_t ldc, const float* bias, const float* gamma, const float* rs, int64_t rps,
+                                    const float* X, float* OUT, const void* H, float* colsum, const float* sample_scale,
+                                    int rows_per_sample, void* workspace, int tokens, void* stream) {
   if (!A || !B || !C) return OCTIC_ENULL;
+  if (sample_scale && (rows_per_sample <= 0 || M <= 0 || (M % rows_per_sample) != 0)) return OCTIC_ESHAPE;
+  if (sample_scale && (((uintptr_t)sample_scale) & 3)) return OCTIC_EALIGN;
   if (M <= 0 || N <= 0 || K <= 0 || (K % DG_BK) || K < 2 * DG_BK || (N % 8) || (lda % 8) || (ldb % 8) || (ldc % 8)) return OCTIC_ESHAPE;
   if ((int64_t)M * lda * 2 >= (1ll << 31) || (int64_t)N * ldb * 2 >= (1ll << 31)) return OCTIC_ESHAPE;
   if ((((uintptr_t)A) | ((uintptr_t)B)) & 15) return OCTIC_EALIGN;
@@ -919,6 +1054,9 @@
   a.tiles_m = p.tiles_m; a.tiles_n = p.tiles_n; a.full_tiles = p.full; a.split = p.split; a.tail_pad = p.tail_pad;
   a.m_stride = tp.image ? tokens : DG_BM;
   a.m_base = tp.image ? 1 : 0;
+  const bool skip = sample_scale != nullptr && mode != DG_RESID && p.tiles_m <= kDgMaskCap;
+  a.sample_scale = skip ? sample_scale : nullptr;
+  a.rows_per_sample = skip ? rows_per_sample : 0;
   hipStream_t s = (hipStream_t)stream;
   if (p.split > 1) {
     if (!workspace) return OCTIC_ENULL;
@@ -926,7 +1064,7 @@
     a.tickets = (int*)workspace;
     a.slabs = (float*)((char*)workspace + DG_TICKET_BYTES);
   }
-  const int smem = DgGeom<4>::LDS, smem5 = DgGeom<5>::LDS;
+  const int smem = DgGeom<4>::LDS, smem5 = DgGeom<5>::LDS, bmb = kDgMaskWords * 8;
   static DeviceOnce once;
   if (once.first()) {
     (void)hipFuncSetAttribute((const void*)dense_nt_kernel<DG_PLAIN, 4>, hipFuncAttributeMaxDynamicSharedMemorySize, smem);
@@ -937,8 +1075,29 @@
     (void)hipFuncSetAttribute((const void*)dense_nt_kernel<DG_GELUF, 4>, hipFuncAttributeMaxDynamicSharedMemorySize, smem);
     (void)hipFuncSetAttribute((const void*)dense_nt_kernel<DG_DFACT, 4>, hipFuncAttributeMaxDynamicSharedMemorySize, smem);
     (void)hipFuncSetAttribute((const void*)dense_nt_kernel<DG_GELUO, 4>, hipFuncAttributeMaxDynamicSharedMemorySize, smem);
+    (void)hipFuncSetAttribute((const void*)dense_nt_kernel<DG_PLAIN, 4, true>, hipFuncAttributeMaxDynamicSharedMemorySize, smem + bmb);
+    (void)hipFuncSetAttribute((const void*)dense_nt_kernel<DG_PLAIN, 5, true>, hipFuncAttributeMaxDynamicSharedMemorySize, smem5 + bmb);
+    (void)hipFuncSetAttribute((const void*)dense_nt_kernel<DG_GELU, 4, true>, hipFuncAttributeMaxDynamicSharedMemorySize, smem + bmb);
+    (void)hipFuncSetAttribute((const void*)dense_nt_kernel<DG_DGELU, 4, true>, hipFuncAttributeMaxDynamicSharedMemorySize, smem + bmb);
+    (void)hipFuncSetAttribute((const void*)dense_nt_kernel<DG_GELUF, 4, true>, hipFuncAttributeMaxDynamicSharedMemorySize, smem + bmb);
+    (void)hipFuncSetAttribute((const void*)dense_nt_kernel<DG_DFACT, 4, true>, hipFuncAttributeMaxDynamicSharedMemorySize, smem + bmb);
+    (void)hipFuncSetAttribute((const void*)dense_nt_kernel<DG_GELUO, 4, true>, hipFuncAttributeMaxDynamicSharedMemorySize, smem + bmb);
     (void)hipGetLastError();
   }
+  if (skip) {
+    switch (mode) {
+      case DG_PLAIN:
+        if (p.nt == 5) dense_nt_kernel<DG_PLAIN, 5, true><<<p.grid, 512, smem5 + bmb, s>>>(a);
+        else dense_nt_kernel<DG_PLAIN, 4, true><<<p.grid, 512, smem + bmb, s>>>(a);
+        break;
+      case DG_GELU: dense_nt_kernel<DG_GELU, 4, true><<<p.grid, 512, smem + bmb, s>>>(a); break;
+      case DG_DGELU: dense_nt_kernel<DG_DGELU, 4, true><<<p.grid, 512, smem + bmb, s>>>(a); break;
+      case DG_GELUF: dense_nt_kernel<DG_GELUF, 4, true><<<p.grid, 512, smem + bmb, s>>>(a); break;
+      case DG_DFACT: dense_nt_kernel<DG_DFACT, 4, true><<<p.grid, 512, smem + bmb, s>>>(a); break;
+      case DG_GELUO: dense_nt_kernel<DG_GELUO, 4, true><<<p.grid, 512, smem + bmb, s>>>(a); break;
+      default: return OCTIC_ESHAPE;
+    }
+  } else
   switch (mode) {
     case DG_PLAIN:
       if (p.nt == 5) dense_nt_kernel<DG_PLAIN, 5><<<p.grid, 512, smem5, s>>>(a);
@@ -974,6 +1133,44 @@
   return launch_status();
 }
 
+int octic_dense_gemm_nt_tokens(const void* A, const void* B, int M, int N, int K, int64_t lda, int64_t ldb, int mode, void* C,
+                               void* C2, int64_t ldc, const float* bias, const float* gamma, const float* rs, int64_t rps,
+                               const float* X, float* OUT, const void* H, float* colsum, void* workspace, int tokens,
+                               void* stream) {
+  return octic_dense_gemm_nt_tokens_skip(A, B, M, N, K, lda, ldb, mode, C, C2, ldc, bias, gamma, rs, rps, X, OUT, H, colsum,
+                                         nullptr, 0, workspace, tokens, stream);
+}
+
+int octic_dense_gemm_plan_dropped(int M, int N, int K, int mode, int tokens, int rows_per_sample, int* out) {
+  if (!out) return OCTIC_ENULL;
+  if (rows_per_sample <= 0 || M <= 0 || (M % rows_per_sample) != 0) return OCTIC_ESHAPE;
+  return octic_dense_gemm_plan(M, N, K, mode, tokens, out);
+}
+
+int octic_dense_gemm_order_dropped(int M, int N, int K, int mode, int tokens, const float* sample_scale, int rows_per_sample,
+                                   int cap, int* out_tm, int* out_tn, int* out_part, int* out_split, int* out_dead) {
+  if (!sample_scale) return OCTIC_ENULL;
+  if (M <= 0 || N <= 0 || K < 2 * DG_BK || rows_per_sample <= 0 || (M % rows_per_sample) != 0 || mode == DG_RESID) return OCTIC_ESHAPE;
+  const DgTokPlan tp = dense_plan_tokens(M, N, K, dense_cus(), mode, tokens);
+  const DgPlan p = tp.p;
+  if (p.tiles_m > kDgMaskCap || cap < p.grid) return OCTIC_ESHAPE;
+  unsigned long long bm[kDgMaskWords] = {};
+  for (int tm = 0; tm < p.tiles_m; ++tm)
+    if (dg_panel_live(sample_scale, rows_per_sample, M, tp.image ? tokens : DG_BM, tp.image ? 1 : 0, tm)) bm[tm >> 6] |= 1ull << (tm & 63);
+  for (int bid = 0; bid < p.grid; ++bid) {
+    int tile, rem_idx, part, tm = -1, tn = -1;
+    bool dead;
+    dense_item_masked(p.tiles_m, p.tiles_n, p.full, p.split, p.tail_pad, bid, bm, tile, rem_idx, part, dead);
+    if (tile >= 0) dg_tile_panel(p.tiles_m, p.tiles_n, tile, tm, tn);
+    if (out_tm) out_tm[bid] = tm;
+    if (out_tn) out_tn[bid] = tn;
+    if (out_part) out_part[bid] = part;
+    if (out_split) out_split[bid] = rem_idx >= 0 ? 1 : 0;
+    if (out_dead) out_dead[bid] = dead ? 1 : 0;
+  }
+  return p.grid;
+}
+
 int octic_dense_gemm_nt(const void* A, const void* B, int M, int N, int K, int64_t lda, int64_t ldb, int mode, void* C,
                         void* C2, int64_t ldc, const float* bias, const float* gamma, const float* rs, int64_t rps,
                         const float* X, float* OUT, const void* H, float* colsum, void* workspace, void* stream) {
diff --git a/octic_vits_amd/functional.py b/octic_vits_amd/functional.py
--- a/octic_vits_amd/functional.py
+++ b/octic_vits_amd/functional.py
@@ -420,6 +420,20 @@
     return rs.detach()
 
 
+def _dense_skip_from_env():
+    return os.environ.get("OCTIC_DENSE_SKIP", "1").strip() != "0"
+
+
+DENSE_NT_SKIP_DROPPED = _dense_skip_from_env()
+
+
+def dense_skip_scale(rs, rps, M, rows_to=None):
+    if (not DENSE_NT_SKIP_DROPPED or rs is None or rows_to is not None or torch.compiler.is_compiling() or not rs.is_cuda
+            or rs.dtype != torch.float32 or rs.dim() != 1 or not rs.is_contiguous() or rps < 2 or rs.numel() * rps != M):
+        return None
+    return rs.detach()
+
+
 def _linear_skip_from_env():
     return os.environ.get("OCTIC_LINEAR_SKIP", "1").strip() != "0"
 
@@ -851,14 +865,16 @@
     return int(shape[-2]) if len(shape) >= 3 else 0
 
 
-def _gemm_fwd(tag, x2, wb, b, cache, name, tokens):
+def _gemm_fwd(tag, x2, wb, b, cache, name, tokens, ss=None, rps=0):
     if tag in DENSE_HIP:
-        return ops.dense_gemm_nt(x2, wb, 0, bias=_f32(b), name=f"dense_nt_kernel<{name}>", tokens=tokens)
+        return ops.dense_gemm_nt(x2, wb, 0, bias=_f32(b), name=f"dense_nt_kernel<{name}>", tokens=tokens, sample_scale=ss,
+                                 rows_per_sample=rps if ss is not None else 0)
     return _linear_lib(x2, wb, None if b is None else cache.b)
 
 
-def _gemm_dgrad(g2, wt, wb, shape, dtype):
-    gx = (ops.dense_gemm_nt(g2, wt, 0, name="dense_nt_kernel<dgrad>", tokens=_tok(shape)) if wt is not None
+def _gemm_dgrad(g2, wt, wb, shape, dtype, ss=None, rps=0):
+    gx = (ops.dense_gemm_nt(g2, wt, 0, name="dense_nt_kernel<dgrad>", tokens=_tok(shape), sample_scale=ss,
+                            rows_per_sample=rps if ss is not None else 0) if wt is not None
           else _mm_lib(g2, wb))
     return gx.view(shape).to(dtype)
 
@@ -870,7 +886,7 @@
     if neps is None and rows_to is None and tag in DENSE_HIP and DENSE_RESID_FUSED:
         br, out = ops.dense_gemm_nt(a2, wb, 2, bias=_f32(b), gamma=g32, rs=rs32, rps=rps, x=x2, name="dense_nt_kernel<resid>")
         return out.view(x.shape), (br, g32, rs32)
-    br = _gemm_fwd(tag, a2, wb, b, cache, tag, tokens)
+    br = _gemm_fwd(tag, a2, wb, b, cache, tag, tokens, dense_skip_scale(rs32, rps, a2.shape[0], rows_to), rps)
     if neps is not None:
         nw32, nb32 = _f32(nw), _f32(nb)
         out, yn, stats = ops.dense_resid_layernorm_fwd(x2, br, g32, rs32, rps, nw32, nb32, neps, torch.bfloat16)
@@ -923,19 +939,20 @@
         xb = _c(x if x.dtype == torch.bfloat16 else x.to(torch.bfloat16))
         wb, wt = cache.get_nt(w, b, ("d" + tag) in DENSE_HIP and ctx.needs_input_grad[0])
         x2 = xb.reshape(-1, wb.shape[1])
-        y = _gemm_fwd(tag, x2, wb, b, cache, "plain", _tok(x.shape))
+        ds = dense_skip_scale(rs, rps, x2.shape[0])
+        y = _gemm_fwd(tag, x2, wb, b, cache, "plain", _tok(x.shape), ds, rps)
         ss = wgrad_skip_scale(rs, rps, x2.shape[0])
         ctx.rps = rps
-        ctx.save_for_backward(x2, wb, wt, ss)
+        ctx.save_for_backward(x2, wb, wt, ss, ds)
         ctx.meta = (b is not None, x.dtype, x.shape, tag)
         return y.view(*x.shape[:-1], wb.shape[0])
 
     @staticmethod
     def backward(ctx, gy):
-        x2, wb, wt, ss = ctx.saved_tensors
+        x2, wb, wt, ss, ds = ctx.saved_tensors
         has_b, x_dtype, x_shape, tag = ctx.meta
         g2 = _c(gy).reshape(-1, wb.shape[0])
-        gx = _gemm_dgrad(g2, wt, wb, x_shape, x_dtype) if ctx.needs_input_grad[0] else None
+        gx = _gemm_dgrad(g2, wt, wb, x_shape, x_dtype, ds, ctx.rps) if ctx.needs_input_grad[0] else None
         gb = None
         if has_b:
             gb = (ops.dense_colsum(g2) if g2.is_cuda and g2.dtype == torch.bfloat16 and g2.shape[1] % 8 == 0
@@ -979,8 +996,9 @@
         a_dtype, a_shape = ctx.meta
         gx, gy, dgamma, colsum, dnw, dnb = _resid_tail_bwd(ctx, tail, gout, gyn,
                                                            ctx.needs_input_grad[8] or ctx.needs_input_grad[9])
-        ga = _gemm_dgrad(gy, wt, wb, a_shape, a_dtype) if ctx.needs_input_grad[1] else None
         rps = ctx.tail[1]
+        ds = dense_skip_scale(tail[2], rps, gy.shape[0], ctx.rows_to)
+        ga = _gemm_dgrad(gy, wt, wb, a_shape, a_dtype, ds, rps) if ctx.needs_input_grad[1] else None
         ss = wgrad_skip_scale(tail[2], rps, gy.shape[0], ctx.rows_to)
         if _pair_ready(ctx.pair, gy, a2) and ops.dense_wgrad_ok(gy.shape[0], gy.shape[1], a2.shape[1]):
             dw = ctx.pair.park(gy, a2, ctx.wparam, ss, rps)
@@ -1003,12 +1021,15 @@
         g32, rs32 = _f32(gamma), _f32(rs)
         factor = GELU_FACTOR and "fc1" in DENSE_HIP and w2t is not None
         ctx.factor = factor
+        ds = dense_skip_scale(rs32, rps, y2.shape[0], rows_to)
+        drps = rps if ds is not None else 0
         if "fc1" in DENSE_HIP and not any(ctx.needs_input_grad):
-            a = ops.dense_gemm_nt(y2, w1b, 6, bias=_f32(b1), name="dense_nt_kernel<gelu-only>", tokens=_tok(y.shape))
+            a = ops.dense_gemm_nt(y2, w1b, 6, bias=_f32(b1), name="dense_nt_kernel<gelu-only>", tokens=_tok(y.shape),
+                                  sample_scale=ds, rows_per_sample=drps)
             h = a
         elif "fc1" in DENSE_HIP:
             h, a = ops.dense_gemm_nt(y2, w1b, 4 if factor else 1, bias=_f32(b1), name="dense_nt_kernel<gelu>",
-                                     tokens=_tok(y.shape))
+                                     tokens=_tok(y.shape), sample_scale=ds, rows_per_sample=drps)
         else:
             h = _linear_lib(y2, w1b, None if b1 is None else c1.b)
             a = torch.nn.functional.gelu(h)
@@ -1024,20 +1045,23 @@
         has_b1, y_dtype, y_shape = ctx.meta
         gx, gbr, dgamma, db2, dnw, dnb = _resid_tail_bwd(ctx, tail, gout, gyn,
                                                          ctx.needs_input_grad[11] or ctx.needs_input_grad[12])
+        rps = ctx.tail[1]
+        ds = dense_skip_scale(tail[2], rps, gbr.shape[0], ctx.rows_to)
+        drps = rps if ds is not None else 0
         if w2t is not None:
             md = 5 if ctx.factor else 3
             if has_b1:
                 dh, db1 = ops.dense_gemm_nt(gbr, w2t, md, h=h, name="dense_nt_kernel<dgelu>", want_colsum=True,
-                                            tokens=_tok(y_shape))
+                                            tokens=_tok(y_shape), sample_scale=ds, rows_per_sample=drps)
             else:
-                dh, db1 = ops.dense_gemm_nt(gbr, w2t, md, h=h, name="dense_nt_kernel<dgelu>", tokens=_tok(y_shape)), None
+                dh, db1 = ops.dense_gemm_nt(gbr, w2t, md, h=h, name="dense_nt_kernel<dgelu>", tokens=_tok(y_shape),
+                                            sample_scale=ds, rows_per_sample=drps), None
         else:
             dh, db1 = ops.dense_gelu_bwd(h, _mm_lib(gbr, w2b), want_colsum=has_b1)
-        rps = ctx.tail[1]
         ss = wgrad_skip_scale(tail[2], rps, gbr.shape[0], ctx.rows_to)
         gw2 = _wgrad_lib(gbr, a, ctx.wparams[1], ss, rps)
         gw1 = _wgrad_lib(dh, y2, ctx.wparams[0], ss, rps)
-        gy = _gemm_dgrad(dh, w1t, w1b, y_shape, y_dtype) if ctx.needs_input_grad[0] else None
+        gy = _gemm_dgrad(dh, w1t, w1b, y_shape, y_dtype, ds, rps) if ctx.needs_input_grad[0] else None
         return gy, gx, gw1, db1, gw2, db2, dgamma, None, None, None, None, dnw, dnb, None, None, None
 
 
diff --git a/octic_vits_amd/ops.py b/octic_vits_amd/ops.py
--- a/octic_vits_amd/ops.py
+++ b/octic_vits_amd/ops.py
@@ -1081,8 +1081,15 @@
     return out[0], out[1], bool(out[2]), out[3]
 
 
+def dense_plan_dropped(M, N, K, mode, tokens, rows_per_sample):
+    out = _lib.plan("octic_dense_gemm_plan_dropped", M, N, K, mode, int(tokens), int(rows_per_sample))
+    if out is None:
+        check(-1)
+    return out[0], out[1], bool(out[2]), out[3]
+
+
 def dense_gemm_nt(a, b, mode=0, bias=None, gamma=None, rs=None, rps=1, x=None, h=None, name=None, want_colsum=False,
-                  tokens=0):
+                  tokens=0, sample_scale=None, rows_per_sample=0):
     _require_cuda(a)
     M, K = a.shape
     N = b.shape[0]
@@ -1093,15 +1100,25 @@
     out = torch.empty((M, N), dtype=torch.float32, device=a.device) if mode == 2 else None
     ws = _dense_ws(M, N, K, a.device)
     tokens = int(tokens) if (tokens and M % int(tokens) == 0) else 0
-    cs_rows = dense_plan(M, N, K, mode, tokens)[1] if (mode in (3, 5) and want_colsum) else 0
+    if sample_scale is not None and mode == 2:
+        raise ValueError("dense_gemm_nt: the fused residual tail (mode 2) takes no sample_scale")
+    plan = ((lambda: dense_plan(M, N, K, mode, tokens)) if sample_scale is None else
+            (lambda: dense_plan_dropped(M, N, K, mode, tokens, rows_per_sample)))
+    cs_rows = plan()[1] if (mode in (3, 5) and want_colsum) else 0
     cs = torch.empty((cs_rows, N), dtype=torch.float32, device=a.device) if cs_rows else None
     t = KERNEL_TIMER.start()
-    check(lib().octic_dense_gemm_nt_tokens(_p(a), _p(b), M, N, K, a.stride(0), b.stride(0), mode, _p(c), _p(c2), N, _p(bias),
-                                           _p(gamma), _p(rs), int(rps), _p(x), _p(out), _p(h), _p(cs), _p(ws), tokens,
-                                           _stream(a)))
+    if sample_scale is None:
+        check(lib().octic_dense_gemm_nt_tokens(_p(a), _p(b), M, N, K, a.stride(0), b.stride(0), mode, _p(c), _p(c2), N, _p(bias),
+                                               _p(gamma), _p(rs), int(rps), _p(x), _p(out), _p(h), _p(cs), _p(ws), tokens,
+                                               _stream(a)))
+    else:
+        check(lib().octic_dense_gemm_nt_tokens_skip(_p(a), _p(b), M, N, K, a.stride(0), b.stride(0), mode, _p(c), _p(c2), N,
+                                                    _p(bias), _p(gamma), _p(rs), int(rps), _p(x), _p(out), _p(h), _p(cs),
+                                                    _p(sample_scale), int(rows_per_sample), _p(ws), tokens,
+                                                    _stream(a)))
     if t is not None:
         nb = 2 * (M * K + N * K + M * N * (2 if mode in (1, 3, 4, 5) else 1)) + (8 * M * N if mode == 2 else 0)
-        wide = "@320" if dense_plan(M, N, K, mode, tokens)[0] == 320 else ""
+        wide = "@320" if plan()[0] == 320 else ""
         KERNEL_TIMER.stop(t, (name or f"dense_nt_kernel<{mode}>") + wide, nb, 2.0 * M * N * K)
     if mode in (1, 4):
         return c, c2
diff --git a/octic_vits_amd/probe.py b/octic_vits_amd/probe.py
--- a/octic_vits_amd/probe.py
+++ b/octic_vits_amd/probe.py
@@ -1,3 +1,4 @@
+import gc
 from collections import OrderedDict
 
 import numpy as np
@@ -309,6 +310,7 @@
         torch.cuda.current_stream(dev).wait_stream(side)
         torch.cuda.synchronize(dev)
         probe.optimizer.push_lr()
+        gc.collect()
         self.graph = torch.cuda.CUDAGraph()
         with torch.cuda.graph(self.graph):
             self.loss = probe.step(self.images, self.labels)
diff --git a/octic_vits_amd/serve.py b/octic_vits_amd/serve.py
--- a/octic_vits_amd/serve.py
+++ b/octic_vits_amd/serve.py
@@ -1,3 +1,5 @@
+import gc
+
 import torch
 
 
@@ -15,6 +17,7 @@
                 self._run()
         torch.cuda.current_stream(example.device).wait_stream(side)
         torch.cuda.synchronize(example.device)
+        gc.collect()
         self.graph = torch.cuda.CUDAGraph()
         with torch.no_grad(), torch.cuda.graph(self.graph):
             self.static_out = self._run()
diff --git a/octic_vits_amd/train.py b/octic_vits_amd/train.py
--- a/octic_vits_amd/train.py
+++ b/octic_vits_amd/train.py
@@ -1,3 +1,4 @@
+import gc
 import math
 import os
 
@@ -1123,6 +1124,7 @@
         return GraphedStep(self, graph, sx, sy, loss.detach())
 
     def _capture_body(self, graph, mode, sx, sy):
+        gc.collect()
         with torch.cuda.graph(graph, **mode):
             if self.augment is not None:
                 sx = self._aug_batch(sx)
```

Result: faster. 1185 images/s, median of 6 (+3.2%).
